# jwliao1209/DiffMusic

Measured on AMD Instinct MI355X. Metric: denoising steps/sec (10 s clip, 200-step DPS), higher is better.
Workload: dtype f16; 1 GPU; MusicLDM + DPS music_inpainting, 10 s @16 kHz, 200-step schedule, batch 8 per GPU (BASELINE.json configs[1]); global_batch=8, clips_per_gpu=8, lanes=1, parallelism=clip-sharded x1 (RCCL world size 1, no per-step collective), finite=True, nan_steps=0, settle_steps=10, cached_reference_transform=True, launched_by=single process

## Files before the change

### diffmusic_amd/_ctypes_ops.py

```python
import ctypes as C

import torch

from . import _lib


def _stream():
    return C.c_void_p(torch.cuda.current_stream().cuda_stream)


def _p(t):
    return C.c_void_p(t.data_ptr()) if t is not None else C.c_void_p(0)


def abi_version():
    return _lib.lib().dmx_abi_version()


def sched_pred_x0(x, eps, alpha_t, *, ptype=0, clip_r=0.0):
    x0 = torch.empty_like(x)
    if ptype == 0 and clip_r == 0.0:
        _lib.check(_lib.lib().dmx_sched_pred_x0(_p(x), _p(eps), _p(x0), x.numel(), alpha_t, _stream()), "pred_x0")
    else:
        _lib.check(_lib.lib().dmx_sched_pred_x0_ex(_p(x), _p(eps), _p(x0), x.numel(), alpha_t, ptype, clip_r, _stream()), "pred_x0_ex")
# ... 244 lines not shown


def vae_dec_fwd(model, z, z_scale, keep_state, want_f32, scale_factor, ws):
    B, _, h, w = z.shape
    s = scale_factor
    mel = torch.empty(B, h * s, w * s, dtype=_lib.act_dtype(), device=z.device)
    mel32 = torch.empty(B, h * s, w * s, dtype=torch.float32, device=z.device) if want_f32 else None
    _lib.check(_lib.lib().dmx_vae_decode_fwd(model, _p(z), z_scale, _p(mel), _p(mel32), B, h, w, int(keep_state), _p(ws), ws.numel(),
                                             _stream()), "vae_decode_fwd")
    return mel, mel32


def vae_dec_bwd(model, dmel, z_scale, latent_channels, scale_factor):
    B, H, W = dmel.shape
    dz = torch.empty(B, latent_channels, H // scale_factor, W // scale_factor, dtype=torch.float32, device=dmel.device)
    _lib.check(_lib.lib().dmx_vae_decode_bwd(model, _p(dmel), z_scale, _p(dz), _stream()), "vae_decode_bwd")
    return dz


def vae_enc_fwd(model, mel, log_floor, latent_channels, scale_factor, ws):
    B, T, F = mel.shape
    s = scale_factor
    mom = torch.empty(B, (T // s) * (F // s), 2 * latent_channels, dtype=torch.float32, device=mel.device)
    _lib.check(_lib.lib().dmx_vae_encode_fwd(model, _p(mel), log_floor, _p(mom), B, T, F, _p(ws), ws.numel(), _stream()), "vae_encode_fwd")
    return mom


def latent_init(moments, h, w, eps, noise, sqrt_abar, scaling_factor, sqrt_1m_abar, want_x):
    B, P, L2 = moments.shape
    assert P == h * w and L2 % 2 == 0, (moments.shape, h, w)
    L = L2 // 2
    mean = torch.empty(B, L, h, w, dtype=torch.float32, device=moments.device)
    logvar = torch.empty_like(mean)
    x = torch.empty_like(mean) if want_x else None
    _lib.check(_lib.lib().dmx_latent_init(_p(moments), _p(mean), _p(logvar), _p(x), _p(eps), _p(noise), B, L, P, sqrt_abar,
                                          scaling_factor, sqrt_1m_abar, _stream()), "latent_init")
    return mean, logvar, x


def grad_normalize_(dwav, target):
    inv_scale = torch.empty(dwav.shape[0], dtype=torch.float32, device=dwav.device)
    _lib.check(_lib.lib().dmx_grad_normalize(_p(dwav), _p(inv_scale), dwav.shape[0], dwav.shape[1], target, _stream()), "grad_normalize")
    return inv_scale


def hifigan_fwd(model, mel, ws):
    lib = _lib.lib()
    B, T, _ = mel.shape
    wav = torch.empty(B, lib.dmx_hifigan_out_len(model, T), dtype=torch.float32, device=mel.device)
    _lib.check(lib.dmx_hifigan_fwd(model, _p(mel), _p(wav), B, T, _p(ws), ws.numel(), _stream()), "hifigan_fwd")
    return wav


def hifigan_bwd(model, dwav, frames, model_in_dim):
    dmel = torch.empty(dwav.shape[0], frames, model_in_dim, dtype=_lib.act_dtype(), device=dwav.device)
    _lib.check(_lib.lib().dmx_hifigan_bwd(model, _p(dwav), _p(dmel), _stream()), "hifigan_bwd")
    return dmel


def htsat_fwd(model, mel, keep_state, ws):
    lib = _lib.lib()
    B, frames, _ = mel.shape
    tokens, channels = C.c_int(), C.c_int()
    _lib.check(lib.dmx_htsat_feature_dims(model, C.byref(tokens), C.byref(channels)), "htsat dims")
    feat = torch.empty(B, tokens.value, channels.value, dtype=torch.float32, device=mel.device)
    _lib.check(lib.dmx_htsat_fwd(model, _p(mel), B, frames, _p(feat), int(keep_state), _p(ws), ws.numel(), _stream()), "htsat_fwd")
    return feat


def htsat_bwd(model, dfeat, scale, frames, bins):
    dmel = torch.empty(dfeat.shape[0], frames, bins, dtype=torch.float32, device=dfeat.device)
    _lib.check(_lib.lib().dmx_htsat_bwd(model, _p(dfeat), _p(scale), _p(dmel), _stream()), "htsat_bwd")
    return dmel


def gram_fwd(feat):
    B, T, Cc = feat.shape
    g = torch.empty(B, Cc, Cc, dtype=torch.float32, device=feat.device)
    _lib.check(_lib.lib().dmx_gram_fwd(_p(feat), _p(g), B, T, Cc, _stream()), "gram_fwd")
    return g


def gram_bwd(feat, dgram):
    B, T, Cc = feat.shape
    d = torch.empty_like(feat)
    _lib.check(_lib.lib().dmx_gram_bwd(_p(feat), _p(dgram), _p(d), B, T, Cc, _stream()), "gram_bwd")
    return d
```

### diffmusic_amd/_lib.py

```python
import ctypes as C
import os

_HERE = os.path.dirname(os.path.abspath(__file__))
LIB_PATH = os.environ.get("DMX_LIB_PATH") or os.path.join(_HERE, "lib", "libdiffmusic_hip.so")
MAX_STAGES = 8


class HifiGanConfig(C.Structure):
    _fields_ = [("model_in_dim", C.c_int), ("upsample_initial_channel", C.c_int), ("num_upsamples", C.c_int),
                ("upsample_rates", C.c_int * MAX_STAGES), ("upsample_kernel_sizes", C.c_int * MAX_STAGES),
                ("num_kernels", C.c_int), ("resblock_kernel_sizes", C.c_int * MAX_STAGES),
                ("num_dilations", C.c_int), ("resblock_dilation_sizes", C.c_int * (MAX_STAGES * MAX_STAGES)),
                ("leaky_relu_slope", C.c_float)]


class VaeConfig(C.Structure):
    _fields_ = [("latent_channels", C.c_int), ("out_channels", C.c_int), ("num_blocks", C.c_int),
                ("block_out_channels", C.c_int * MAX_STAGES), ("layers_per_block", C.c_int),
                ("norm_num_groups", C.c_int), ("eps", C.c_float)]


class UNetConfig(C.Structure):
    _fields_ = [("in_channels", C.c_int), ("out_channels", C.c_int), ("num_blocks", C.c_int),
                ("block_out_channels", C.c_int * MAX_STAGES), ("layers_per_block", C.c_int),
# ... 2 lines not shown
                ("class_embed_dim", C.c_int), ("num_attn_per_layer", C.c_int), ("attn_cross_dims", C.c_int * 4)]


class HtsatConfig(C.Structure):
    _fields_ = [("spec_size", C.c_int), ("num_mel_bins", C.c_int), ("patch_size", C.c_int), ("embed_dim", C.c_int), ("window_size", C.c_int),
                ("num_stages", C.c_int), ("depths", C.c_int * 4), ("num_heads", C.c_int * 4), ("ln_eps", C.c_float), ("bn_eps", C.c_float)]


class GemmDesc(C.Structure):
    _fields_ = [("A", C.c_void_p), ("W", C.c_void_p), ("C", C.c_void_p), ("C2", C.c_void_p),
                ("bias", C.c_void_p), ("rowbias", C.c_void_p), ("R", C.c_void_p), ("X", C.c_void_p),
                ("M", C.c_int), ("N", C.c_int), ("K", C.c_int), ("ldw", C.c_int),
                ("Hi", C.c_int), ("Wi", C.c_int), ("Ci", C.c_int), ("lda", C.c_int),
                ("Hq", C.c_int), ("Wq", C.c_int), ("sy", C.c_int), ("sx", C.c_int),
                ("ntaps", C.c_int),
                ("Ho", C.c_int), ("Wo", C.c_int), ("ldc", C.c_int), ("osy", C.c_int), ("ooy", C.c_int),
                ("osx", C.c_int), ("oox", C.c_int),
                ("ldr", C.c_int), ("ldx", C.c_int), ("ldc2", C.c_int),
                ("Z", C.c_int), ("Zi", C.c_int),
                ("sAo", C.c_longlong), ("sAi", C.c_longlong), ("sWo", C.c_longlong), ("sWi", C.c_longlong),
                ("sCo", C.c_longlong), ("sCi", C.c_longlong),
                ("alpha", C.c_float), ("act_slope", C.c_float), ("mask_slope", C.c_float),
                ("flags", C.c_int),
                ("tdy", C.c_byte * 16), ("tdx", C.c_byte * 16), ("resid_inv_slope", C.c_float), ("tile_cfg", C.c_int), ("ldrb", C.c_int), ("ksplit", C.c_int),
                ("XB", C.c_void_p), ("B2", C.c_void_p), ("ldxb", C.c_int), ("ldb2", C.c_int),
                ("colsum", C.c_void_p), ("ln_eps", C.c_float), ("rowstats_in", C.c_void_p), ("rowstats_out", C.c_void_p), ("nslots", C.c_int),
                ("gn_part", C.c_void_p), ("gnb_x", C.c_void_p), ("gnb_scale", C.c_void_p), ("gnb_shift", C.c_void_p),
                ("gnb_ldx", C.c_int), ("gnb_silu", C.c_int), ("gnb_stats", C.c_void_p), ("gnb_cpg", C.c_int)]


EPI_BIAS, EPI_ROWBIAS, EPI_RESID, EPI_ACCUM, EPI_MASK, EPI_LRELU2, EPI_TANH, EPI_F32OUT, EPI_NO_C, EPI_RESID_INV, EPI_MASKBITS, EPI_BITS2, EPI_SOFTBWD = \
    1, 2, 4, 8, 16, 32, 64, 128, 256, 512, 1024, 2048, 4096
EPI_GEGLU, EPI_LNFOLD, EPI_ROWSTATS, EPI_GNSTATS, EPI_GNBWD = 8192, 16384, 32768, 65536, 131072

_SIGS = {
    "dmx_abi_version": (C.c_int, []),
    "dmx_act_dtype": (C.c_int, []),
    "dmx_last_error": (C.c_char_p, []),
    "dmx_hifigan_create": (C.c_void_p, [C.POINTER(HifiGanConfig)]),
    "dmx_vae_decoder_create": (C.c_void_p, [C.POINTER(VaeConfig)]),
    "dmx_unet_create": (C.c_void_p, [C.POINTER(UNetConfig)]),
    "dmx_model_destroy": (None, [C.c_void_p]),
    "dmx_model_num_params": (C.c_int, [C.c_void_p]),
    "dmx_model_param_name": (C.c_char_p, [C.c_void_p, C.c_int]),
    "dmx_model_param_numel": (C.c_size_t, [C.c_void_p, C.c_int]),
    "dmx_model_param_ndim": (C.c_int, [C.c_void_p, C.c_int]),
    "dmx_model_param_dim": (C.c_int, [C.c_void_p, C.c_int, C.c_int]),
    "dmx_model_load_param": (C.c_int, [C.c_void_p, C.c_char_p, C.c_void_p, C.c_size_t]),
    "dmx_model_finalize": (C.c_int, [C.c_void_p, C.c_void_p]),
    "dmx_hifigan_out_len": (C.c_int, [C.c_void_p, C.c_int]),
    "dmx_hifigan_workspace_bytes": (C.c_size_t, [C.c_void_p, C.c_int, C.c_int]),
    "dmx_hifigan_fwd": (C.c_int, [C.c_void_p, C.c_void_p, C.c_void_p, C.c_int, C.c_int, C.c_void_p, C.c_size_t, C.c_void_p]),
    "dmx_hifigan_bwd": (C.c_int, [C.c_void_p, C.c_void_p, C.c_void_p, C.c_void_p]),
    "dmx_vae_workspace_bytes": (C.c_size_t, [C.c_void_p, C.c_int, C.c_int, C.c_int]),
    "dmx_vae_decode_fwd": (C.c_int, [C.c_void_p, C.c_void_p, C.c_float, C.c_void_p, C.c_void_p, C.c_int, C.c_int, C.c_int,
                                     C.c_int, C.c_void_p, C.c_size_t, C.c_void_p]),
    "dmx_vae_decode_bwd": (C.c_int, [C.c_void_p, C.c_void_p, C.c_float, C.c_void_p, C.c_void_p]),
    "dmx_vae_encoder_create": (C.c_void_p, [C.POINTER(VaeConfig)]),
    "dmx_vae_encoder_workspace_bytes": (C.c_size_t, [C.c_void_p, C.c_int, C.c_int, C.c_int]),
    "dmx_vae_encode_fwd": (C.c_int, [C.c_void_p, C.c_void_p, C.c_float, C.c_void_p, C.c_int, C.c_int, C.c_int, C.c_void_p, C.c_size_t,
                                     C.c_void_p]),
    "dmx_latent_init": (C.c_int, [C.c_void_p] * 6 + [C.c_int] * 3 + [C.c_float] * 3 + [C.c_void_p]),
    "dmx_conv2d_raw": (C.c_int, [C.c_void_p] * 4 + [C.c_int] * 9 + [C.c_void_p]),
    "dmx_unet_workspace_bytes": (C.c_size_t, [C.c_void_p, C.c_int, C.c_int, C.c_int]),
    "dmx_unet_fwd": (C.c_int, [C.c_void_p, C.c_void_p, C.c_void_p, C.c_void_p, C.c_void_p, C.c_int, C.c_int, C.c_int,
                               C.c_void_p, C.c_size_t, C.c_void_p]),
    "dmx_unet_fwd_ctx": (C.c_int, [C.c_void_p] * 5 + [C.c_int, C.c_void_p, C.c_int, C.c_void_p, C.c_void_p, C.c_int, C.c_int, C.c_int,
                                   C.c_void_p, C.c_size_t, C.c_void_p]),
    "dmx_unet_workspace_bytes_ctx": (C.c_size_t, [C.c_void_p, C.c_int, C.c_int, C.c_int, C.c_int, C.c_int]),
    "dmx_htsat_create": (C.c_void_p, [C.POINTER(HtsatConfig)]),
    "dmx_htsat_feature_dims": (C.c_int, [C.c_void_p, C.POINTER(C.c_int), C.POINTER(C.c_int)]),
    "dmx_htsat_workspace_bytes": (C.c_size_t, [C.c_void_p, C.c_int, C.c_int]),
    "dmx_htsat_fwd": (C.c_int, [C.c_void_p, C.c_void_p, C.c_int, C.c_int, C.c_void_p, C.c_int, C.c_void_p, C.c_size_t, C.c_void_p]),
    "dmx_htsat_bwd": (C.c_int, [C.c_void_p, C.c_void_p, C.c_void_p, C.c_void_p, C.c_void_p]),
    "dmx_htsat_tape_raw": (C.c_size_t, [C.c_void_p, C.c_int, C.c_int, C.c_int, C.c_void_p, C.c_size_t, C.c_void_p]),
    "dmx_gram_fwd": (C.c_int, [C.c_void_p, C.c_void_p, C.c_int, C.c_int, C.c_int, C.c_void_p]),
    "dmx_gram_bwd": (C.c_int, [C.c_void_p, C.c_void_p, C.c_void_p, C.c_int, C.c_int, C.c_int, C.c_void_p]),
    "dmx_gemm_raw": (C.c_int, [C.c_void_p, C.c_size_t, C.c_void_p]),
    "dmx_prof_begin": (None, []),
    "dmx_prof_end": (C.c_int, [C.POINTER(C.c_double), C.POINTER(C.c_double)]),
    "dmx_flash_attn_raw": (C.c_int, [C.c_void_p, C.c_void_p, C.c_void_p, C.c_void_p, C.c_void_p] + [C.c_int] * 6 + [C.c_float, C.c_void_p]),
    "dmx_gemm_splitk_workspace": (C.c_int, [C.c_void_p, C.c_size_t]),
    "dmx_conv_pair_raw": (C.c_int, [C.c_void_p, C.c_void_p, C.c_size_t, C.c_void_p]),
    "dmx_conv_pair_group_raw": (C.c_int, [C.c_int, C.c_void_p, C.c_void_p, C.c_size_t, C.c_void_p]),
    "dmx_groupnorm_scratch_floats": (C.c_size_t, [C.c_int, C.c_int, C.c_int]),
    "dmx_groupnorm_raw": (C.c_int, [C.c_void_p] * 8 + [C.c_int] * 4 + [C.c_float, C.c_int, C.c_void_p]),
    "dmx_groupnorm_part_floats": (C.c_size_t, [C.c_int, C.c_int, C.c_int]),
    "dmx_groupnorm_parts_raw": (C.c_int, [C.c_void_p] * 7 + [C.c_int] * 4 + [C.c_float, C.c_int, C.c_int, C.c_void_p, C.c_void_p, C.c_void_p]),
    "dmx_gemm_last_tile_rows_raw": (C.c_int, []),
    "dmx_groupnorm_bwd_raw": (C.c_int, [C.c_void_p] * 10 + [C.c_int] * 6 + [C.c_void_p, C.c_void_p, C.c_void_p]),
    "dmx_prof_dominant": (C.c_int, [C.POINTER(C.c_double)] * 3),
    "dmx_audio_create": (C.c_void_p, [C.c_int, C.c_int, C.c_int, C.c_int, C.c_void_p]),
    "dmx_audio_destroy": (None, [C.c_void_p]),
    "dmx_audio_num_frames": (C.c_int, [C.c_void_p, C.c_int]),
    "dmx_audio_num_bins": (C.c_int, [C.c_void_p]),
    "dmx_audio_state_bytes": (C.c_size_t, [C.c_void_p, C.c_int, C.c_int]),
    "dmx_audio_transform_fwd": (C.c_int, [C.c_void_p, C.c_void_p, C.c_longlong, C.c_void_p, C.c_void_p, C.c_int, C.c_int, C.c_int,
                                          C.c_int, C.c_float, C.c_float, C.c_void_p]),
    "dmx_audio_transform_bwd": (C.c_int, [C.c_void_p, C.c_void_p, C.c_void_p, C.c_longlong, C.c_void_p, C.c_int, C.c_int, C.c_int,
                                          C.c_int, C.c_float, C.c_float, C.c_int, C.c_void_p]),
    "dmx_audio_is_fused": (C.c_int, [C.c_void_p, C.c_int]),
    "dmx_audio_guidance_fwd": (C.c_int, [C.c_void_p, C.c_void_p, C.c_longlong, C.c_void_p, C.c_void_p, C.c_longlong, C.c_void_p, C.c_void_p,
                                         C.c_int, C.c_int, C.c_int, C.c_int, C.c_float, C.c_float, C.c_void_p]),
    "dmx_audio_guidance_bwd": (C.c_int, [C.c_void_p, C.c_void_p, C.c_longlong, C.c_void_p, C.c_void_p, C.c_longlong, C.c_float, C.c_void_p,
                                         C.c_void_p, C.c_longlong, C.c_int, C.c_void_p, C.c_int, C.c_int, C.c_int, C.c_int, C.c_float, C.c_float,
                                         C.c_void_p]),
    "dmx_audio_guidance_fwd_ex": (C.c_int, [C.c_void_p, C.c_void_p, C.c_longlong, C.c_void_p, C.c_void_p, C.c_longlong, C.c_void_p, C.c_void_p,
                                            C.c_int, C.c_int, C.c_int, C.c_int, C.c_float, C.c_float, C.c_void_p, C.c_longlong, C.c_void_p,
                                            C.c_float, C.c_void_p]),
    "dmx_audio_guidance_bwd_ex": (C.c_int, [C.c_void_p, C.c_void_p, C.c_longlong, C.c_void_p, C.c_void_p, C.c_longlong, C.c_float, C.c_void_p,
                                            C.c_void_p, C.c_longlong, C.c_int, C.c_void_p, C.c_int, C.c_int, C.c_int, C.c_int, C.c_float, C.c_float,
                                            C.c_void_p, C.c_longlong, C.c_void_p, C.c_float, C.c_void_p]),
    "dmx_audio_guidance_fwd_shaped": (C.c_int, [C.c_void_p, C.c_void_p, C.c_longlong, C.c_void_p, C.c_void_p, C.c_longlong, C.c_void_p, C.c_void_p,
                                                C.c_int, C.c_int, C.c_int, C.c_int, C.c_float, C.c_float, C.c_void_p, C.c_longlong, C.c_void_p,
                                                C.c_float, C.c_void_p, C.c_void_p]),
    "dmx_audio_guidance_bwd_shaped": (C.c_int, [C.c_void_p, C.c_void_p, C.c_longlong, C.c_void_p, C.c_void_p, C.c_longlong, C.c_float, C.c_void_p,
                                                C.c_void_p, C.c_longlong, C.c_int, C.c_void_p, C.c_int, C.c_int, C.c_int, C.c_int, C.c_float, C.c_float,
                                                C.c_void_p, C.c_longlong, C.c_void_p, C.c_float, C.c_void_p, C.c_void_p]),
    "dmx_clip_fwd": (C.c_int, [C.c_void_p, C.c_longlong, C.c_void_p, C.c_void_p, C.c_longlong, C.c_int, C.c_int, C.c_void_p]),
    "dmx_clip_bwd": (C.c_int, [C.c_void_p, C.c_longlong, C.c_void_p, C.c_longlong, C.c_void_p, C.c_void_p, C.c_longlong, C.c_int, C.c_int, C.c_int,
                               C.c_void_p]),
    "dmx_declip_project": (C.c_int, [C.c_void_p, C.c_longlong, C.c_void_p, C.c_longlong, C.c_void_p, C.c_void_p, C.c_longlong, C.c_int, C.c_int,
                                     C.c_void_p]),
    "dmx_noise_add": (C.c_int, [C.c_void_p, C.c_void_p, C.c_void_p, C.c_longlong, C.c_float, C.c_void_p]),
    "dmx_audio_stft_mag": (C.c_int, [C.c_void_p, C.c_void_p, C.c_longlong, C.c_void_p, C.c_void_p, C.c_int, C.c_int, C.c_void_p]),
    "dmx_audio_stft_mag_bwd": (C.c_int, [C.c_void_p, C.c_void_p, C.c_void_p, C.c_longlong, C.c_void_p, C.c_int, C.c_int, C.c_int, C.c_void_p]),
    "dmx_audio_melscale": (C.c_int, [C.c_void_p, C.c_void_p, C.c_void_p, C.c_int, C.c_int, C.c_float, C.c_float, C.c_void_p]),
    "dmx_mask_apply": (C.c_int, [C.c_void_p, C.c_longlong, C.c_void_p, C.c_void_p, C.c_longlong, C.c_int, C.c_int, C.c_int, C.c_void_p]),
    "dmx_l2_loss": (C.c_int, [C.c_void_p, C.c_longlong, C.c_void_p, C.c_void_p, C.c_void_p, C.c_int, C.c_longlong, C.c_float, C.c_void_p]),
    "dmx_track_stitch_fwd": (C.c_int, [C.c_void_p, C.c_longlong, C.c_void_p, C.POINTER(C.c_int)] + [C.c_int] * 4 + [C.c_void_p]),
    "dmx_track_stitch_bwd": (C.c_int, [C.c_void_p, C.c_void_p, C.c_longlong, C.POINTER(C.c_int)] + [C.c_int] * 5 + [C.c_void_p]),
    "dmx_grad_normalize": (C.c_int, [C.c_void_p, C.c_void_p, C.c_int, C.c_longlong, C.c_float, C.c_void_p]),
    "dmx_fir_fwd": (C.c_int, [C.c_void_p, C.c_longlong, C.c_void_p, C.c_void_p, C.c_longlong] + [C.c_int] * 7 + [C.c_void_p]),
    "dmx_fir_bwd": (C.c_int, [C.c_void_p, C.c_longlong, C.c_void_p, C.c_void_p, C.c_void_p, C.c_longlong] + [C.c_int] * 7 + [C.c_void_p]),
    "dmx_sched_pred_x0": (C.c_int, [C.c_void_p, C.c_void_p, C.c_void_p, C.c_longlong, C.c_float, C.c_void_p]),
    "dmx_sched_pred_x0_ex": (C.c_int, [C.c_void_p, C.c_void_p, C.c_void_p, C.c_longlong, C.c_float, C.c_int, C.c_float, C.c_void_p]),
    "dmx_sched_step_ex": (C.c_int, [C.c_int] + [C.c_void_p] * 9 + [C.c_int, C.c_int] + [C.c_float] * 5 + [C.c_int, C.c_int, C.c_float, C.c_void_p]),
    "dmx_sched_cfg_combine": (C.c_int, [C.c_void_p, C.c_void_p, C.c_longlong, C.c_float, C.c_void_p]),
    "dmx_randn_philox": (C.c_int, [C.c_void_p, C.c_int, C.c_longlong, C.POINTER(C.c_ulonglong), C.c_ulonglong, C.c_void_p]),
    "dmx_sched_step": (C.c_int, [C.c_int] + [C.c_void_p] * 9 + [C.c_int, C.c_int] + [C.c_float] * 5 + [C.c_int, C.c_void_p]),
}

ADDED_IN_V4 = ("dmx_vae_encoder_create", "dmx_vae_encoder_workspace_bytes", "dmx_vae_encode_fwd", "dmx_latent_init",
               "dmx_track_stitch_fwd", "dmx_track_stitch_bwd", "dmx_audio_guidance_fwd_shaped", "dmx_audio_guidance_bwd_shaped",
               "dmx_clip_fwd", "dmx_clip_bwd", "dmx_declip_project")

_lib = None


def check_symbols(h, path=LIB_PATH):
    for name in ADDED_IN_V4:
        if not hasattr(h, name):
            raise RuntimeError(f"{path} reports ABI version {ABI_VERSION} but does not export `{name}` (a build from before the VAE "
                               "encoder / track-mode / declipping entry points): rebuild it (python -m diffmusic_amd.build --force)")


def lib():
    global _lib
    if _lib is None:
        if not os.path.exists(LIB_PATH):
            raise RuntimeError(f"{LIB_PATH} is missing: build it with `python -m diffmusic_amd.build` "
                               "(the diffmusic_amd hot path has no CPU fallback)")
        h = C.CDLL(LIB_PATH)
        for name, (res, args) in _SIGS.items():
            if not hasattr(h, name):
                continue
            fn = getattr(h, name)
            fn.restype, fn.argtypes = res, args
        if h.dmx_abi_version() != ABI_VERSION:
            raise RuntimeError(f"libdiffmusic_hip.so ABI version {h.dmx_abi_version()} != {ABI_VERSION} expected by this package: rebuild it "
                               "(python -m diffmusic_amd.build --force)")
        check_symbols(h)
        _lib = h
    return _lib


ABI_VERSION = 4


def act_dtype():
    import torch
    return torch.float16 if lib().dmx_act_dtype() == 1 else torch.bfloat16


class DmxError(RuntimeError):
    pass


def check(rc, what=""):
    if rc != 0:
        msg = lib().dmx_last_error()
        raise DmxError(f"{what} failed with code {rc}: {msg.decode() if msg else ''}")
```

### diffmusic_amd/csrc/capi.hip

```cpp
#include "conv_pair.h"
#include "models.h"

#define M_IMPL(m) ((m) ? (m)->impl : nullptr)
#define ST(s) ((hipStream_t)(s))

extern "C" {

int dmx_abi_version(void) { return DMX_ABI_VERSION; }
int dmx_act_dtype(void) { return DMX_ACT_DTYPE; }

dmx_model* dmx_hifigan_create(const dmx_hifigan_config* cfg) {
  if (!cfg || cfg->num_upsamples > DMX_MAX_STAGES || cfg->num_kernels > DMX_MAX_STAGES || cfg->num_dilations > DMX_MAX_STAGES) {
    dmx_set_error("bad hifigan config");
    return nullptr;
  }
  return new dmx_model{dmx_make_hifigan(cfg)};
}
dmx_model* dmx_vae_decoder_create(const dmx_vae_config* cfg) {
  if (!cfg || cfg->num_blocks > DMX_MAX_STAGES) { dmx_set_error("bad vae config"); return nullptr; }
  Model* m = dmx_make_vae(cfg);
  return m ? new dmx_model{m} : nullptr;
}
dmx_model* dmx_unet_create(const dmx_unet_config* cfg) {
  if (!cfg || cfg->num_blocks > DMX_MAX_STAGES) { dmx_set_error("bad unet config"); return nullptr; }
  Model* m = dmx_make_unet(cfg);
  return m ? new dmx_model{m} : nullptr;
}
void dmx_model_destroy(dmx_model* m) {
  if (!m) return;
  delete m->impl;
  delete m;
}
int dmx_model_num_params(const dmx_model* m) { return (int)m->impl->ps.params.size(); }
const char* dmx_model_param_name(const dmx_model* m, int i) { return m->impl->ps.params[i].name.c_str(); }
size_t dmx_model_param_numel(const dmx_model* m, int i) { return m->impl->ps.params[i].numel; }
int dmx_model_param_ndim(const dmx_model* m, int i) { return (int)m->impl->ps.params[i].shape.size(); }
int dmx_model_param_dim(const dmx_model* m, int i, int d) { return m->impl->ps.params[i].shape[d]; }
int dmx_model_load_param(dmx_model* m, const char* name, const float* data_host, size_t numel) {
  if (m->impl->finalized) { dmx_set_error("model already finalized"); return DMX_ERR_STATE; }
  return m->impl->ps.load(name, data_host, numel);
}
int dmx_model_finalize(dmx_model* m, void* stream) {
  std::string missing;
  if (!m->impl->ps.all_loaded(&missing)) { dmx_set_error("parameter '%s' was never loaded", missing.c_str()); return DMX_ERR_PARAM; }
  const int rc = m->impl->finalize(ST(stream));
  if (rc == DMX_OK) m->impl->finalized = true;
  return rc;
}

static int check(dmx_model* m, int kind) {
  if (!m || !m->impl || m->impl->kind != kind) { dmx_set_error("wrong model handle"); return DMX_ERR_STATE; }
  if (!m->impl->finalized) { dmx_set_error("model not finalized"); return DMX_ERR_STATE; }
  return DMX_OK;
}

int dmx_hifigan_out_len(const dmx_model* m, int frames) { return dmx_hifigan_out_len_impl(m->impl, frames); }
size_t dmx_hifigan_workspace_bytes(dmx_model* m, int batch, int frames) { return dmx_hifigan_ws_impl(m->impl, batch, frames); }
int dmx_hifigan_fwd(dmx_model* m, const uint16_t* mel, float* wav, int batch, int frames, void* ws, size_t ws_bytes, void* stream) {
  int rc = check(m, DMX_MODEL_HIFIGAN);
  if (rc) return rc;
  if (!ws) { dmx_set_error("null workspace"); return DMX_ERR_WORKSPACE; }
  return dmx_hifigan_fwd_impl(m->impl, mel, wav, batch, frames, ws, ws_bytes, ST(stream));
}
int dmx_hifigan_bwd(dmx_model* m, const float* dwav, uint16_t* dmel, void* stream) {
  int rc = check(m, DMX_MODEL_HIFIGAN);
  if (rc) return rc;
  return dmx_hifigan_bwd_impl(m->impl, dwav, dmel, ST(stream));
}

size_t dmx_vae_workspace_bytes(dmx_model* m, int batch, int h, int w) { return dmx_vae_ws_impl(m->impl, batch, h, w); }
int dmx_vae_decode_fwd(dmx_model* m, const float* z, float z_scale, uint16_t* mel, float* mel_f32, int batch, int h, int w,
                       int keep_state, void* ws, size_t ws_bytes, void* stream) {
  int rc = check(m, DMX_MODEL_VAE);
  if (rc) return rc;
  if (!ws) { dmx_set_error("null workspace"); return DMX_ERR_WORKSPACE; }
  return dmx_vae_fwd_impl(m->impl, z, z_scale, mel, mel_f32, batch, h, w, keep_state, ws, ws_bytes, ST(stream));
}
int dmx_vae_decode_bwd(dmx_model* m, const uint16_t* dmel, float z_scale, float* dz, void* stream) {
  int rc = check(m, DMX_MODEL_VAE);
  if (rc) return rc;
  return dmx_vae_bwd_impl(m->impl, dmel, z_scale, dz, ST(stream));
}

dmx_model* dmx_vae_encoder_create(const dmx_vae_config* cfg) {
  if (!cfg || cfg->num_blocks > DMX_MAX_STAGES) { dmx_set_error("bad vae config"); return nullptr; }
  Model* m = dmx_make_vae_encoder(cfg);
  return m ? new dmx_model{m} : nullptr;
}
size_t dmx_vae_encoder_workspace_bytes(dmx_model* m, int batch, int frames, int bins) {
  if (!m || !m->impl || m->impl->kind != DMX_MODEL_VAE_ENC) return 0;
  return dmx_vae_enc_ws_impl(m->impl, batch, frames, bins);
}
int dmx_vae_encode_fwd(dmx_model* m, const float* mel, float log_floor, float* moments, int batch, int frames, int bins, void* ws,
                       size_t ws_bytes, void* stream) {
  int rc = check(m, DMX_MODEL_VAE_ENC);
  if (rc) return rc;
  if (!ws) { dmx_set_error("null workspace"); return DMX_ERR_WORKSPACE; }
  return dmx_vae_enc_fwd_impl(m->impl, mel, log_floor, moments, batch, frames, bins, ws, ws_bytes, ST(stream));
}
int dmx_latent_init(const float* moments, float* mean, float* logvar, float* x, const float* eps, const float* noise, int batch,
                    int latent_channels, int hw, float sqrt_abar, float scaling_factor, float sqrt_1m_abar, void* stream) {
  return dmx_latent_init_impl(moments, mean, logvar, x, eps, noise, batch, latent_channels, hw, sqrt_abar, scaling_factor, sqrt_1m_abar, ST(stream));
}
int dmx_conv2d_raw(const float* w_host, const float* b_host, const void* x, void* y, int B, int Hi, int Wi, int Ci, int Co, int k, int stride,
                   int pad_lo, int pad_hi, void* stream) {
  return dmx_conv2d_raw_impl(w_host, b_host, (const act_t*)x, (act_t*)y, B, Hi, Wi, Ci, Co, k, stride, pad_lo, pad_hi, ST(stream));
}

dmx_model* dmx_htsat_create(const dmx_htsat_config* cfg) {
  Model* impl = dmx_make_htsat(cfg);
  if (!impl) return nullptr;
  return new dmx_model{impl};
}
int dmx_htsat_feature_dims(dmx_model* m, int* tokens, int* channels) {
  if (!m || !m->impl || m->impl->kind != DMX_MODEL_HTSAT) { dmx_set_error("wrong model handle"); return DMX_ERR_STATE; }
// ... 140 lines not shown
```

### diffmusic_amd/csrc/conv_pair.h

```cpp
#pragma once
#include <cstdlib>
#include <cstring>
#include "dmx_common.h"

bool dmx_conv_pair_eligible(const GemmDesc* a, const GemmDesc& b);
int dmx_conv_pair_launch(const GemmDesc* a, const GemmDesc& b, hipStream_t st);
int dmx_conv_pair_group_launch(int n, const GemmDesc* const* a, const GemmDesc* const* b, hipStream_t st);

int dmx_prof_open(hipStream_t st);
void dmx_prof_close(int rec, hipStream_t st, double flops, double bytes, int M, int N, int K, int taps, int flags, int cfg);
```

### diffmusic_amd/csrc/conv_pair.hip

```cpp
#include "gemm_epilogue.h"
#include "conv_pair.h"

namespace {

constexpr int PAIR_HALO = 50;
constexpr int PAIR_ROWS = 256;
constexpr unsigned PAIR_OOB = 0x80000000u;

struct PairParams {
  GemmDesc a, b;
  int T, nb, BMo;
  int loA, hiA, loB, hiB;
  int off0A, dA, off0B, dB;
  int single;
  int r_from_slab;
  int a_tape_bits_only;
};

#ifdef DMX_PAIR_STAMPS
__device__ unsigned long long g_pair_stamps[4096 * 8];
#define DMX_STAMP(i) do { stamp_v[i] = wall_clock64(); } while (0)
#else
#define DMX_STAMP(i) do { } while (0)
#endif

template <int C>
struct PairCfg {
  static constexpr int PITCH = 2 * C + 32;
  static constexpr int CPR = C / 8;
  static constexpr int WN = C > 64 ? C / 64 : 1;
  static constexpr int NW = 4 * WN;
  static constexpr int NT = NW * 64;
  static constexpr int FN = C / 16 / WN;
  static constexpr int SLAB_ROWS = PAIR_ROWS + PAIR_HALO;
  static constexpr int SLAB_BYTES = SLAB_ROWS * PITCH;
  static constexpr int TILE = C * 128;
  static constexpr int NS = C == 128 ? 4 : 3;
  static constexpr int PER = TILE / 1024 / NW;
  static constexpr int SLAB_IT = (SLAB_ROWS * CPR + NT - 1) / NT;
  static constexpr int BITS_IT = PAIR_ROWS * CPR / NT;
  static constexpr int BITS_BYTES = PAIR_ROWS * CPR;
  static constexpr int BIAS_BYTES = 2 * C * 4;
  static constexpr int LDS_BYTES = SLAB_BYTES + NS * TILE + BITS_BYTES + BIAS_BYTES;
  static constexpr int MIN_WAVES = C == 32 ? 3 : 2;
  static_assert(PER >= 1 && PAIR_ROWS * CPR % NT == 0, "tile / thread-count mismatch");
};

template <int FN>
struct PairFrags { frag8_t x[2][4]; frag8_t w[2][FN]; };

#define DMX_PAIR_DSR(dst, addr, off) asm volatile("ds_read_b128 %0, %1 offset:%2" : "=v"(dst) : "v"(addr), "n"(off))

#define DMX_LDS_ADDR(p) ((unsigned)(size_t)(__attribute__((address_space(3))) const char*)(p))
typedef unsigned u32x2_t __attribute__((ext_vector_type(2)));
typedef unsigned u32x4_t __attribute__((ext_vector_type(4)));
__device__ __forceinline__ void pair_lds_w64(const void* p, uint2 v) {
  const u32x2_t w = {v.x, v.y};
  asm volatile("ds_write_b64 %0, %1" ::"v"(DMX_LDS_ADDR(p)), "v"(w) : "memory");
}
#define DMX_PAIR_DSR64(dst, p) asm volatile("ds_read_b64 %0, %1" : "=v"(dst) : "v"(DMX_LDS_ADDR(p)))
#define DMX_PAIR_DSRU8(dst, p) asm volatile("ds_read_u8 %0, %1" : "=v"(dst) : "v"(DMX_LDS_ADDR(p)))
__device__ __forceinline__ void pair_lds_wait() { asm volatile("s_waitcnt lgkmcnt(0)" ::: "memory"); }
template <typename T>
__device__ __forceinline__ void pair_tie8(T (&r)[8]) {
  asm volatile("s_waitcnt lgkmcnt(0)" : "+v"(r[0]), "+v"(r[1]), "+v"(r[2]), "+v"(r[3]), "+v"(r[4]), "+v"(r[5]), "+v"(r[6]), "+v"(r[7]) : : "memory");
}
template <typename T>
__device__ __forceinline__ void pair_tie16(T (&r)[16]) {
  asm volatile("s_waitcnt lgkmcnt(0)"
               : "+v"(r[0]), "+v"(r[1]), "+v"(r[2]), "+v"(r[3]), "+v"(r[4]), "+v"(r[5]), "+v"(r[6]), "+v"(r[7]), "+v"(r[8]), "+v"(r[9]), "+v"(r[10]),
                 "+v"(r[11]), "+v"(r[12]), "+v"(r[13]), "+v"(r[14]), "+v"(r[15])
               :
               : "memory");
}
template <typename T, int N>
__device__ __forceinline__ void pair_tie(T (&r)[N]) {
  static_assert(N == 8 || N == 16, "4 row fragments x 2 or 4 column fragments");
  if constexpr (N == 8) pair_tie8(r); else pair_tie16(r);
}

__device__ __forceinline__ void pair_settle(PairFrags<4>& f) {
  asm volatile("s_waitcnt lgkmcnt(0)"
               : "+v"(f.x[0][0]), "+v"(f.x[0][1]), "+v"(f.x[0][2]), "+v"(f.x[0][3]), "+v"(f.x[1][0]), "+v"(f.x[1][1]), "+v"(f.x[1][2]),
                 "+v"(f.x[1][3]), "+v"(f.w[0][0]), "+v"(f.w[0][1]), "+v"(f.w[0][2]), "+v"(f.w[0][3]), "+v"(f.w[1][0]), "+v"(f.w[1][1]),
                 "+v"(f.w[1][2]), "+v"(f.w[1][3])
               :
               : "memory");
}
__device__ __forceinline__ void pair_settle(PairFrags<2>& f) {
  asm volatile("s_waitcnt lgkmcnt(0)"
               : "+v"(f.x[0][0]), "+v"(f.x[0][1]), "+v"(f.x[0][2]), "+v"(f.x[0][3]), "+v"(f.x[1][0]), "+v"(f.x[1][1]), "+v"(f.x[1][2]),
                 "+v"(f.x[1][3]), "+v"(f.w[0][0]), "+v"(f.w[0][1]), "+v"(f.w[1][0]), "+v"(f.w[1][1])
               :
               : "memory");
}

template <int C>
__device__ __forceinline__ void pair_body(const PairParams& P, char* smem, int bid, const int nwg) {
  using K = PairCfg<C>;
  constexpr int PITCH = K::PITCH, CPR = K::CPR, FN = K::FN, NS = K::NS, PER = K::PER, TILE = K::TILE, NT = K::NT, NW = K::NW, WN = K::WN;
  char* ring = smem;
  char* slab = smem + NS * TILE;
  unsigned char* s_bits = reinterpret_cast<unsigned char*>(slab + K::SLAB_BYTES);
  float* s_bias = reinterpret_cast<float*>(slab + K::SLAB_BYTES + K::BITS_BYTES);

  const int tid = threadIdx.x, lane = tid & 63, lr = lane & 15, lq = lane >> 4;
  const int wave = __builtin_amdgcn_readfirstlane(tid >> 6);
  const int rg = wave / WN, cg = wave - rg * WN;
#ifdef DMX_PAIR_STAMPS
  const int stamp_id = bid;
  unsigned long long stamp_v[8] = {0, 0, 0, 0, 0, 0, 0, 0};
#endif
  DMX_STAMP(0);
  {
    const int q = nwg >> 3, r = nwg & 7, xcd = bid & 7, loc = bid >> 3;
    bid = (xcd < r ? xcd * (q + 1) : r * (q + 1) + (xcd - r) * q) + loc;
  }
  const int T = P.T;
  const int b = bid / P.nb, tq = bid - b * P.nb;
  const int t0 = tq * P.BMo;
  const bool single = P.single != 0;
  const int kA = single ? 0 : P.a.ntaps, kB = P.b.ntaps;
  const int stepsA = (kA * C + 63) / 64, stepsB = (kB * C + 63) / 64, total = stepsA + stepsB;

  const __amdgpu_buffer_rsrc_t rsA = __builtin_amdgcn_make_buffer_rsrc(const_cast<act_t*>(single ? P.b.W : P.a.W), 0, PAIR_OOB, 0x00020000);
  const __amdgpu_buffer_rsrc_t rsB = __builtin_amdgcn_make_buffer_rsrc(const_cast<act_t*>(P.b.W), 0, PAIR_OOB, 0x00020000);
  const int lrow = lane >> 3, cc = (lane & 7) ^ lrow;
  auto issue_dma = [&](int g) {
    const bool inA = g < stepsA;
    const int sidx = inA ? g : g - stepsA;
    const int Kel = inA ? P.a.K : P.b.K;
    const unsigned ldw2 = (unsigned)(inA ? P.a.ldw : P.b.ldw) * 2u;
    const int kel = sidx * 64 + cc * 8;
    const bool ok = g < total && kel < Kel;
    char* dst = ring + (g % NS) * TILE;
#pragma unroll
    for (int i = 0; i < PER; ++i) {
      const int j = i * NW + wave;
      const unsigned voff = ok ? (unsigned)(j * 8 + lrow) * ldw2 + (unsigned)kel * 2u : PAIR_OOB;
      if (inA) __builtin_amdgcn_raw_ptr_buffer_load_lds(rsA, (__attribute__((address_space(3))) void*)(dst + j * 1024), 16, voff, 0, 0, 0);
      else __builtin_amdgcn_raw_ptr_buffer_load_lds(rsB, (__attribute__((address_space(3))) void*)(dst + j * 1024), 16, voff, 0, 0, 0);
    }
  };
  issue_dma(0);
  issue_dma(1);
  issue_dma(2);

  {
    const act_t* src = single ? P.b.A : P.a.A;
    const int nrows = PAIR_ROWS + (single ? P.loB + P.hiB : P.loA + P.hiA);
    const int tfirst = t0 - P.loB - (single ? 0 : P.loA);
    uint4 sv[K::SLAB_IT];
#pragma unroll
    for (int it = 0; it < K::SLAB_IT; ++it) {
      const int c = tid + it * NT, row = c / CPR, piece = c % CPR, t = tfirst + row;
      sv[it] = make_uint4(0, 0, 0, 0);
      if (row < nrows && t >= 0 && t < T) sv[it] = *reinterpret_cast<const uint4*>(src + ((long long)b * T + t) * C + piece * 8);
    }
    const bool masked = !single && (P.a.flags & EPI_MASK);
    const bool maskbits = !single && (P.a.flags & EPI_MASKBITS);
    constexpr int BPT = K::BITS_BYTES / NT;
    static_assert(BPT == 4 || BPT == 8, "bit-mask copy granularity");
    static_assert(CPR % BPT == 0, "a thread's mask bytes must stay inside one row");
    uint32_t mb[2] = {0u, 0u};
    if (maskbits) {
      const int c = tid * BPT, row = c / CPR, piece = c % CPR, t = t0 - P.loB + row;
      if (t >= 0 && t < T) {
        const unsigned char* src = P.a.XB + ((long long)b * T + t) * P.a.ldxb + piece;
        mb[0] = *reinterpret_cast<const uint32_t*>(src);
        if (BPT == 8) mb[1] = *reinterpret_cast<const uint32_t*>(src + 4);
      }
    }
#pragma unroll
    for (int it = 0; it < K::SLAB_IT; ++it) {
      const int c = tid + it * NT, row = c / CPR, piece = c % CPR;
      if (row < K::SLAB_ROWS) *reinterpret_cast<uint4*>(slab + row * PITCH + piece * 16) = sv[it];
    }
    if (masked) {
#pragma unroll 1
      for (int it = 0; it < K::BITS_IT; ++it) {
        const int c = tid + it * NT, row = c / CPR, piece = c % CPR, t = t0 - P.loB + row;
        uint4 m = make_uint4(0, 0, 0, 0);
        if (t >= 0 && t < T) m = *reinterpret_cast<const uint4*>(P.a.X + ((long long)b * T + t) * C + piece * 8);
        s_bits[c] = (unsigned char)dmx_pos8(m);
      }
    }
    if (maskbits) {
      uint32_t* d = reinterpret_cast<uint32_t*>(s_bits + tid * BPT);
      d[0] = mb[0];
      if (BPT == 8) d[1] = mb[1];
    }
  }
  if (tid < 2 * C) {
    const GemmDesc& d = tid < C ? P.a : P.b;
    const int ch = tid < C ? tid : tid - C;
    s_bias[tid] = (!(single && tid < C) && d.bias && (d.flags & (EPI_BIAS | EPI_BIASINIT))) ? d.bias[ch] : 0.f;
  }
  asm volatile("s_waitcnt vmcnt(0)" ::: "memory");
  __syncthreads();
  DMX_STAMP(1);

  f32x4 acc[4][FN];
  auto zero_acc = [&]() {
#pragma unroll
    for (int i = 0; i < 4; ++i)
#pragma unroll
      for (int n = 0; n < FN; ++n) acc[i][n] = f32x4{0.f, 0.f, 0.f, 0.f};
  };
  auto init_acc = [&](const GemmDesc& d) {
    if (C < 128 && (d.flags & EPI_BIASINIT)) {
// ... 256 lines not shown
  Halo h{0, 0, true, d.ntaps > 1 ? d.tdx[1] - d.tdx[0] : 0};
  for (int j = 0; j < d.ntaps; ++j) {
    if (d.tdx[j] != d.tdx[0] + j * h.d) h.ok = false;
    if (d.tdy[j] != 0) h.ok = false;
    if (-d.tdx[j] > h.lo) h.lo = -d.tdx[j];
    if (d.tdx[j] > h.hi) h.hi = d.tdx[j];
  }
  if (h.lo + h.hi > PAIR_HALO) h.ok = false;
  return h;
}

bool stage_ok(const GemmDesc& d, int C, int T, int allowed_flags) {
  if (d.N != C || d.Ci != C || d.lda != C || d.K != d.ntaps * C || d.ldw < d.K) return false;
  if (d.ntaps < 1 || d.ntaps > 16 || d.Z != 1 || d.Hq != 1 || d.Hi != 1 || d.Ho != 1) return false;
  if (d.Wq != T || d.Wi != T || d.Wo != T || d.sx != 1 || d.osx != 1 || d.oox != 0 || d.ooy != 0) return false;
  if (d.flags & ~allowed_flags) return false;
  if (d.M % T != 0) return false;
  return true;
}

bool g_pair_enabled = getenv("DMX_NO_PAIR") == nullptr;

}

bool dmx_conv_pair_eligible(const GemmDesc* a, const GemmDesc& b) {
  if (!g_pair_enabled) return false;
  const int C = b.N, T = b.Wq;
  static const bool c128 = getenv("DMX_NO_PAIR128") == nullptr;
  if (C != 32 && C != 64 && !(C == 128 && c128)) return false;
  if (T < 1) return false;
  const int bflags = EPI_BIAS | EPI_RESID | EPI_RESID_INV | EPI_ACCUM | EPI_MASK | EPI_LRELU2 | EPI_NO_C | EPI_MASKBITS | EPI_BITS2;
  if (!stage_ok(b, C, T, bflags) || !halo_of(b).ok) return false;
  if ((b.flags & EPI_LRELU2) && !(b.act_slope >= 0.f && b.act_slope <= 1.f)) return false;
  if ((b.flags & EPI_RESID_INV) && !(b.resid_inv_slope >= 1.f)) return false;
  if (b.ldc != C || ((b.flags & EPI_RESID) && b.ldr != C) || ((b.flags & EPI_MASK) && b.ldx != C) || ((b.flags & EPI_LRELU2) && b.ldc2 != C))
    return false;
  if ((b.flags & EPI_MASKBITS) && (!b.XB || b.ldxb * 8 < C)) return false;
  if ((b.flags & EPI_BITS2) && (!b.B2 || b.ldb2 * 8 < C)) return false;
  if (a) {
    if (!stage_ok(*a, C, T, EPI_BIAS | EPI_LRELU2 | EPI_NO_C | EPI_MASK | EPI_MASKBITS | EPI_BITS2) || !halo_of(*a).ok) return false;
    if (a->M != b.M || a->alpha != 1.f) return false;
    if ((a->flags & EPI_LRELU2) && !(a->flags & EPI_BITS2) && (a->ldc2 != C || !a->C2)) return false;
    if ((a->flags & EPI_LRELU2) && a->C2 && a->ldc2 != C) return false;
    if ((a->flags & EPI_BITS2) && (!(a->flags & EPI_LRELU2) || !a->B2 || a->ldb2 * 8 < C)) return false;
    if ((a->flags & EPI_MASK) && (a->ldx != C || !a->X)) return false;
    if ((a->flags & EPI_MASKBITS) && (!a->XB || a->ldxb * 8 < C || (a->flags & EPI_MASK))) return false;
    const Halo hb = halo_of(b);
    if (PAIR_ROWS - hb.lo - hb.hi < 128) return false;
  }
  return true;
}

namespace {
long long pair_params(const GemmDesc* a, const GemmDesc& b, PairParams& P, double& fl, double& by) {
  memset(&P, 0, sizeof(P));
  P.b = b;
  P.single = a ? 0 : 1;
  if (a) P.a = *a;
  const Halo hb = halo_of(b);
  P.loB = hb.lo; P.hiB = hb.hi;
  P.off0B = b.tdx[0] + hb.lo; P.dB = hb.d;
  if (a) { const Halo ha = halo_of(*a); P.loA = ha.lo; P.hiA = ha.hi; P.off0A = a->tdx[0] + ha.lo; P.dA = ha.d; }
  P.T = b.Wq;
  P.BMo = a ? PAIR_ROWS - hb.lo - hb.hi : PAIR_ROWS;
  P.nb = cdiv(P.T, P.BMo);
  static const bool bias_init = getenv("DMX_NO_BIAS_INIT") == nullptr;
  if (bias_init && b.N < 128) {
    if ((P.b.flags & EPI_BIAS) && P.b.bias && !(P.b.flags & (EPI_MASK | EPI_MASKBITS))) P.b.flags = (P.b.flags & ~EPI_BIAS) | EPI_BIASINIT;
    if (a && (P.a.flags & EPI_BIAS) && P.a.bias && !(P.a.flags & (EPI_MASK | EPI_MASKBITS))) P.a.flags = (P.a.flags & ~EPI_BIAS) | EPI_BIASINIT;
  }
  P.r_from_slab = (a && (b.flags & EPI_RESID) && b.R == a->A && b.ldr == b.N) ? 1 : 0;
  P.a_tape_bits_only = (a && (a->flags & EPI_BITS2) && !a->C2) ? 1 : 0;
  const int nclips = b.M / P.T;
  const int C = b.N;
  fl = 2.0 * b.M * (double)b.N * b.K;
  by = 2.0 * b.M * (double)C * 2.0;
  const double bits_by = b.M * (double)C / 8.0;
  if (a) {
    fl += 2.0 * a->M * (double)a->N * a->K;
    if ((a->flags & EPI_LRELU2) && !P.a_tape_bits_only) by += 2.0 * b.M * (double)C;
    if (a->flags & EPI_BITS2) by += bits_by;
    if (a->flags & EPI_MASK) by += 2.0 * b.M * (double)C;
    if (a->flags & EPI_MASKBITS) by += bits_by;
  }
  if ((b.flags & EPI_RESID) && !P.r_from_slab) by += 2.0 * b.M * (double)C;
  if (b.flags & EPI_MASK) by += 2.0 * b.M * (double)C;
  if (b.flags & EPI_MASKBITS) by += bits_by;
  if (b.flags & EPI_BITS2) by += bits_by;
  if (b.flags & EPI_ACCUM) by += 2.0 * b.M * (double)C;
  if ((b.flags & EPI_LRELU2) && !(b.flags & EPI_NO_C)) by += 2.0 * b.M * (double)C;
  return (long long)nclips * P.nb;
}
}

static int pair_extra_lds() { static const int v = [] { const char* e = getenv("DMX_PAIR_EXTRA_LDS"); return e ? atoi(e) : 0; }(); return v; }
int dmx_conv_pair_launch(const GemmDesc* a, const GemmDesc& b, hipStream_t st) {
  if (!dmx_conv_pair_eligible(a, b)) return DMX_ERR_SHAPE;
  PairParams P;
  double fl, by;
  const long long grid = pair_params(a, b, P, fl, by);
  if (grid > 0x7fffffffLL) return DMX_ERR_SHAPE;
  const int C = b.N;
  const int rec = dmx_prof_open(st);
  auto launch = [&](auto tag) {
    constexpr int CC = decltype(tag)::value;
    static bool attr = false;
    if (!attr) { (void)hipFuncSetAttribute((const void*)conv_pair_kernel<CC>, hipFuncAttributeMaxDynamicSharedMemorySize, PairCfg<CC>::LDS_BYTES + (CC < 128 ? pair_extra_lds() : 0)); attr = true; }
    hipLaunchKernelGGL(conv_pair_kernel<CC>, dim3((unsigned)grid), dim3(PairCfg<CC>::NT), PairCfg<CC>::LDS_BYTES + (CC < 128 ? pair_extra_lds() : 0), st, P);
  };
  if (C == 32) launch(std::integral_constant<int, 32>{});
  else if (C == 64) launch(std::integral_constant<int, 64>{});
  else launch(std::integral_constant<int, 128>{});
  dmx_prof_close(rec, st, fl, by, b.M, b.N, (a ? a->K : 0) + b.K, b.ntaps, b.flags, a ? 21 : 20);
  return hipGetLastError() == hipSuccess ? DMX_OK : DMX_ERR_LAUNCH;
}

int dmx_conv_pair_group_launch(int n, const GemmDesc* const* a, const GemmDesc* const* b, hipStream_t st) {
  if (n < 1 || n > DMX_PAIR_GROUP) return DMX_ERR_SHAPE;
  static const bool off = getenv("DMX_NO_PAIR_GROUP") != nullptr;
  bool same = !off && n > 1;
  for (int j = 0; j < n; ++j) {
    if (!a[j] || !b[j] || !dmx_conv_pair_eligible(a[j], *b[j])) return DMX_ERR_SHAPE;
    if (b[j]->N != b[0]->N) same = false;
    for (int i = 0; i < j; ++i)
      if (b[j]->C == b[i]->C || (b[j]->C2 && b[j]->C2 == b[i]->C2)) same = false;
  }
  if (!same) {
    for (int j = 0; j < n; ++j) { const int rc = dmx_conv_pair_launch(a[j], *b[j], st); if (rc != DMX_OK) return rc; }
    return DMX_OK;
  }
  int order[DMX_PAIR_GROUP] = {0, 1, 2};
  auto work = [&](int j) { return a[j]->K + b[j]->K; };
  for (int i = 0; i < n; ++i)
    for (int k = i + 1; k < n; ++k)
      if (work(order[k]) > work(order[i])) { const int t = order[i]; order[i] = order[k]; order[k] = t; }
  PairGroup G;
  memset(&G, 0, sizeof(G));
  double fl = 0.0, by = 0.0;
  long long gmax = 0;
  int Ksum = 0;
  for (int i = 0; i < n; ++i) {
    const int j = order[i];
    double f1, b1;
    const long long g = pair_params(a[j], *b[j], G.p[i], f1, b1);
    if (g > 0x7ffffff0LL) return DMX_ERR_SHAPE;
    G.n[i] = (int)g;
    if (g > gmax) gmax = g;
    fl += f1; by += b1; Ksum += a[j]->K + b[j]->K;
  }
  const unsigned gx = (unsigned)((gmax + 7) & ~7ll);
  const int C = b[0]->N;
  const int rec = dmx_prof_open(st);
  auto launch = [&](auto tag) {
    constexpr int CC = decltype(tag)::value;
    static bool attr = false;
    if (!attr) { (void)hipFuncSetAttribute((const void*)conv_pair_group_kernel<CC>, hipFuncAttributeMaxDynamicSharedMemorySize, PairCfg<CC>::LDS_BYTES); attr = true; }
    hipLaunchKernelGGL(conv_pair_group_kernel<CC>, dim3(gx, (unsigned)n), dim3(PairCfg<CC>::NT), PairCfg<CC>::LDS_BYTES, st, G);
  };
  if (C == 32) launch(std::integral_constant<int, 32>{});
  else if (C == 64) launch(std::integral_constant<int, 64>{});
  else launch(std::integral_constant<int, 128>{});
  dmx_prof_close(rec, st, fl, by, b[0]->M, C, Ksum, b[0]->ntaps, b[0]->flags, 22);
  return hipGetLastError() == hipSuccess ? DMX_OK : DMX_ERR_LAUNCH;
}

#ifdef DMX_PAIR_STAMPS
extern "C" int dmx_pair_stamps_read(unsigned long long* host) {
  return hipMemcpyFromSymbol(host, HIP_SYMBOL(g_pair_stamps), sizeof(unsigned long long) * 4096 * 8) == hipSuccess ? 0 : -1;
}
#endif
```

### diffmusic_amd/csrc/elementwise.hip

```cpp
#include "dmx_common.h"
#include <cstdlib>
#include "kernels.h"

namespace {

__device__ __forceinline__ void unpack8(const uint4& u, float* f) {
  f[0] = alo(u.x); f[1] = ahi(u.x); f[2] = alo(u.y); f[3] = ahi(u.y);
  f[4] = alo(u.z); f[5] = ahi(u.z); f[6] = alo(u.w); f[7] = ahi(u.w);
}
__device__ __forceinline__ uint4 pack8(const float* f) {
  return make_uint4(pack2a(f[0], f[1]), pack2a(f[2], f[3]), pack2a(f[4], f[5]), pack2a(f[6], f[7]));
}
__device__ __forceinline__ float silu_f(float z) { return z / (1.f + __expf(-z)); }
__device__ __forceinline__ float dsilu_f(float z) {
  const float s = 1.f / (1.f + __expf(-z));
  return s * (1.f + z * (1.f - s));
}

template <int MODE>
__global__ void gn_partial_kernel(const act_t* __restrict__ x, const act_t* __restrict__ dy,
                                  const float* __restrict__ scale, const float* __restrict__ shift,
                                  const float* __restrict__ stats, float* __restrict__ partial,
                                  int P, int C, int G, int rpb, int ppb, int silu) {
  extern __shared__ float sh[];
// ... 928 lines not shown
}

__global__ void nchw_f32_to_nhwc_bf16_kernel(const float* __restrict__ x, act_t* __restrict__ y, int B, int C, int HW,
                                             int Cp, float scale) {
  const long long idx = (long long)blockIdx.x * blockDim.x + threadIdx.x;
  if (idx >= (long long)B * HW * Cp) return;
  const int c = (int)(idx % Cp);
  const long long pix = idx / Cp;
  const int b = (int)(pix / HW), p = (int)(pix - (long long)b * HW);
  y[idx] = c < C ? f2a(x[((long long)b * C + c) * HW + p] * scale) : (act_t)0;
}
__global__ void nhwc_bf16_to_nchw_f32_kernel(const act_t* __restrict__ x, float* __restrict__ y, int B, int C, int HW,
                                             int Cp, float scale) {
  const long long idx = (long long)blockIdx.x * blockDim.x + threadIdx.x;
  if (idx >= (long long)B * C * HW) return;
  const int p = (int)(idx % HW);
  const long long bc = idx / HW;
  const int b = (int)(bc / C), c = (int)(bc - (long long)b * C);
  y[idx] = a2f(x[((long long)b * HW + p) * Cp + c]) * scale;
}
__global__ void f32_to_bf16_kernel(const float* __restrict__ x, act_t* __restrict__ y, long long n, float scale) {
  const long long idx = (long long)blockIdx.x * blockDim.x + threadIdx.x;
  if (idx < n) y[idx] = f2a(x[idx] * scale);
}
__global__ void bf16_to_f32_kernel(const act_t* __restrict__ x, float* __restrict__ y, long long n, float scale) {
  const long long idx = (long long)blockIdx.x * blockDim.x + threadIdx.x;
  if (idx < n) y[idx] = a2f(x[idx]) * scale;
}
__global__ void extract_col_kernel(const act_t* __restrict__ x, float* __restrict__ y, long long rows, int ld, int col) {
  const long long idx = (long long)blockIdx.x * blockDim.x + threadIdx.x;
  if (idx < rows) y[idx] = a2f(x[idx * ld + col]);
}
__global__ void timestep_embed_kernel(const float* __restrict__ t, act_t* __restrict__ y, int B, int dim) {
  const int idx = blockIdx.x * blockDim.x + threadIdx.x;
  if (idx >= B * dim) return;
  const int b = idx / dim, j = idx - b * dim, half = dim >> 1;
  const int k = j < half ? j : j - half;
  const float e = t[b] * __expf(-9.210340371976184f * (float)k / (float)half);
  y[idx] = f2a(j < half ? cosf(e) : sinf(e));
}

__global__ void gather_col_f32_kernel(const float* __restrict__ x, float* __restrict__ y, long long rows, int ld, int col) {
  const long long idx = (long long)blockIdx.x * blockDim.x + threadIdx.x;
  if (idx < rows) y[idx] = x[idx * ld + col];
}
__global__ void tanh_bwd_pad8_kernel(const float* __restrict__ dwav, const float* __restrict__ wav8, act_t* __restrict__ gz,
                                     long long rows) {
  const long long idx = (long long)blockIdx.x * blockDim.x + threadIdx.x;
  if (idx >= rows) return;
  const float w = wav8[idx * 8];
  const float g = dwav[idx] * (1.f - w * w);
  reinterpret_cast<uint4*>(gz)[idx] = make_uint4((uint32_t)f2a(g), 0u, 0u, 0u);
}
__global__ void scatter_col_pad8_kernel(const float* __restrict__ v, act_t* __restrict__ y, long long rows, float scale) {
  const long long idx = (long long)blockIdx.x * blockDim.x + threadIdx.x;
  if (idx >= rows) return;
  reinterpret_cast<uint4*>(y)[idx] = make_uint4((uint32_t)f2a(v[idx] * scale), 0u, 0u, 0u);
}

__global__ void gather_col_f32_to_act_kernel(const float* __restrict__ x, act_t* __restrict__ y, long long rows, int ld, int col) {
  const long long idx = (long long)blockIdx.x * blockDim.x + threadIdx.x;
  if (idx < rows) y[idx] = f2a(x[idx * ld + col]);
}
__global__ void pad_col8_act_kernel(const act_t* __restrict__ v, act_t* __restrict__ y, long long rows) {
  const long long idx = (long long)blockIdx.x * blockDim.x + threadIdx.x;
  if (idx >= rows) return;
  reinterpret_cast<uint4*>(y)[idx] = make_uint4((uint32_t)v[idx], 0u, 0u, 0u);
}

constexpr int GN_SMALL_MAXU = 16;
__global__ __launch_bounds__(256) void gn_small_kernel(const act_t* __restrict__ x, act_t* __restrict__ y,
                                                       const float* __restrict__ gamma, const float* __restrict__ beta,
                                                       float* __restrict__ stats, float* __restrict__ scale, float* __restrict__ shift,
                                                       int P, int C, int G, float eps, int silu) {
  __shared__ float sh[16];
  const int g = blockIdx.x, b = blockIdx.y, cpg = C / G, U = cpg >> 2, c0 = g * cpg;
  const int units = P * U;
  const act_t* xb = x + (long long)b * P * C + c0;
  uint2 v[GN_SMALL_MAXU];
  float sum = 0.f;
#pragma unroll
  for (int i = 0; i < GN_SMALL_MAXU; ++i) {
    const int u = threadIdx.x + i * 256;
    v[i] = make_uint2(0, 0);
    if (u < units) {
      const int px = u / U, cu = u - px * U;
      v[i] = *reinterpret_cast<const uint2*>(xb + (long long)px * C + cu * 4);
      sum += alo(v[i].x) + ahi(v[i].x) + alo(v[i].y) + ahi(v[i].y);
    }
  }
  const float n = (float)units * 4.f;
  const float mean = block_sum(sum, sh) / n;
  float m2 = 0.f;
#pragma unroll
  for (int i = 0; i < GN_SMALL_MAXU; ++i) {
    if (threadIdx.x + i * 256 < units) {
      const float d0 = alo(v[i].x) - mean, d1 = ahi(v[i].x) - mean, d2 = alo(v[i].y) - mean, d3 = ahi(v[i].y) - mean;
      m2 += d0 * d0 + d1 * d1 + d2 * d2 + d3 * d3;
    }
  }
  const float rstd = rsqrtf(block_sum(m2, sh) / n + eps);
  if (threadIdx.x == 0) {
    stats[((long long)b * G + g) * 2] = mean;
    stats[((long long)b * G + g) * 2 + 1] = rstd;
  }
  if (threadIdx.x < cpg) {
// ... 199 lines not shown
  return CHECK_LAUNCH();
}
int dmx_concat2(const act_t* a, const act_t* b, act_t* dst, long long rows, int Ca, int Cb, hipStream_t st) {
  if ((Ca & 7) || (Cb & 7)) return DMX_ERR_SHAPE;
  const long long n = rows * ((Ca + Cb) >> 3);
  hipLaunchKernelGGL(concat2_kernel, dim3((unsigned)((n + 255) / 256)), dim3(256), 0, st, a, b, dst, rows, Ca, Cb);
  return CHECK_LAUNCH();
}
int dmx_axpby(const act_t* x, const act_t* y0, act_t* y, float a, float b, long long n, hipStream_t st) {
  if (n & 7) return DMX_ERR_SHAPE;
  hipLaunchKernelGGL(axpby_kernel, dim3((unsigned)((n / 8 + 255) / 256)), dim3(256), 0, st, x, y0, y, a, b, n / 8);
  return CHECK_LAUNCH();
}
int dmx_nchw_f32_to_nhwc_bf16(const float* x, act_t* y, int B, int C, int HW, int Cp, float scale, hipStream_t st) {
  const long long n = (long long)B * HW * Cp;
  hipLaunchKernelGGL(nchw_f32_to_nhwc_bf16_kernel, dim3((unsigned)((n + 255) / 256)), dim3(256), 0, st, x, y, B, C, HW, Cp, scale);
  return CHECK_LAUNCH();
}
int dmx_nhwc_bf16_to_nchw_f32(const act_t* x, float* y, int B, int C, int HW, int Cp, float scale, hipStream_t st) {
  const long long n = (long long)B * C * HW;
  hipLaunchKernelGGL(nhwc_bf16_to_nchw_f32_kernel, dim3((unsigned)((n + 255) / 256)), dim3(256), 0, st, x, y, B, C, HW, Cp, scale);
  return CHECK_LAUNCH();
}
int dmx_f32_to_bf16(const float* x, act_t* y, long long n, float scale, hipStream_t st) {
  hipLaunchKernelGGL(f32_to_bf16_kernel, dim3((unsigned)((n + 255) / 256)), dim3(256), 0, st, x, y, n, scale);
  return CHECK_LAUNCH();
}
int dmx_bf16_to_f32(const act_t* x, float* y, long long n, float scale, hipStream_t st) {
  hipLaunchKernelGGL(bf16_to_f32_kernel, dim3((unsigned)((n + 255) / 256)), dim3(256), 0, st, x, y, n, scale);
  return CHECK_LAUNCH();
}
int dmx_extract_col(const act_t* x, float* y, long long rows, int ld, int col, hipStream_t st) {
  hipLaunchKernelGGL(extract_col_kernel, dim3((unsigned)((rows + 255) / 256)), dim3(256), 0, st, x, y, rows, ld, col);
  return CHECK_LAUNCH();
}
int dmx_timestep_embed(const float* t, act_t* y, int B, int dim, hipStream_t st) {
  hipLaunchKernelGGL(timestep_embed_kernel, dim3(cdiv(B * dim, 256)), dim3(256), 0, st, t, y, B, dim);
  return CHECK_LAUNCH();
}

int dmx_gather_col_f32(const float* x, float* y, long long rows, int ld, int col, hipStream_t st) {
  hipLaunchKernelGGL(gather_col_f32_kernel, dim3((unsigned)((rows + 255) / 256)), dim3(256), 0, st, x, y, rows, ld, col);
  return CHECK_LAUNCH();
}
int dmx_tanh_bwd_pad8(const float* dwav, const float* wav8, act_t* gz, long long rows, hipStream_t st) {
  hipLaunchKernelGGL(tanh_bwd_pad8_kernel, dim3((unsigned)((rows + 255) / 256)), dim3(256), 0, st, dwav, wav8, gz, rows);
  return CHECK_LAUNCH();
}
int dmx_scatter_col_pad8(const float* v, act_t* y, long long rows, float scale, hipStream_t st) {
  hipLaunchKernelGGL(scatter_col_pad8_kernel, dim3((unsigned)((rows + 255) / 256)), dim3(256), 0, st, v, y, rows, scale);
  return CHECK_LAUNCH();
}

int dmx_gather_col_f32_to_act(const float* x, act_t* y, long long rows, int ld, int col, hipStream_t st) {
  hipLaunchKernelGGL(gather_col_f32_to_act_kernel, dim3((unsigned)((rows + 255) / 256)), dim3(256), 0, st, x, y, rows, ld, col);
  return CHECK_LAUNCH();
}
int dmx_pad_col8_act(const act_t* v, act_t* y, long long rows, hipStream_t st) {
  hipLaunchKernelGGL(pad_col8_act_kernel, dim3((unsigned)((rows + 255) / 256)), dim3(256), 0, st, v, y, rows);
  return CHECK_LAUNCH();
}
```

### diffmusic_amd/csrc/hifigan.hip

```cpp
#include "models.h"
#include "conv_pair.h"
#include <cstdlib>

struct SplitKScope {
  explicit SplitKScope(float* ws, size_t bytes, bool on) : on_(on && ws) { if (on_) dmx_gemm_set_splitk_workspace(ws, bytes); }
  ~SplitKScope() { if (on_) dmx_gemm_set_splitk_workspace(nullptr, 0); }
  bool on_;
};

struct HifiGan : Model {
  dmx_hifigan_config cfg;
  static constexpr size_t kSplitKBytes = 32u << 20;
  float* splitk_ws = nullptr;
  ConvLayer conv_pre, conv_post;
  std::vector<ConvLayer> ups;
  std::vector<ConvLayer> c1, c2;
  int nk = 0, nd = 0, ns = 0;
  int B = 0, T = 0;
  std::vector<int> Ts;
  act_t* act_pre = nullptr;
  std::vector<act_t*> xs_a;
  std::vector<act_t*> ha, xa;
  std::vector<act_t*> act_out;
  std::vector<unsigned char*> hb, xb;
  std::vector<char> fused;
  float* wav8 = nullptr;
  bool have_tape = false;
  hipStream_t bstream[DMX_MAX_STAGES] = {};
  std::vector<hipEvent_t> events;
  size_t ev_next = 0;
  bool want_multi = true;
  hipEvent_t next_event() { hipEvent_t e = events[ev_next]; ev_next = (ev_next + 1) % events.size(); return e; }
  bool multi() const { return want_multi && !dry && !dmx_prof_is_active() && nk > 1; }
  bool multi_wanted() const { return want_multi && nk > 1; }

  int idx(int s, int k, int d) const { return (s * nk + k) * nd + d; }

  explicit HifiGan(const dmx_hifigan_config& c) : cfg(c) {
    kind = DMX_MODEL_HIFIGAN;
    ns = c.num_upsamples; nk = c.num_kernels; nd = c.num_dilations;
    const int C0 = c.upsample_initial_channel;
    conv_pre = make_conv1d(ps, "conv_pre", c.model_in_dim, C0, 7, 1, 3, true);
    for (int i = 0; i < ns; ++i) {
      const int s = c.upsample_rates[i], k = c.upsample_kernel_sizes[i];
      ups.push_back(make_convT1d(ps, "upsampler." + std::to_string(i), C0 >> i, C0 >> (i + 1), k, s, (k - s) / 2, true));
    }
    int ch = C0;
    for (int i = 0; i < ns; ++i) {
      ch = C0 >> (i + 1);
      for (int j = 0; j < nk; ++j) {
        const int k = c.resblock_kernel_sizes[j];
        const std::string pre = "resblocks." + std::to_string(i * nk + j);
        for (int d = 0; d < nd; ++d) {
          const int dil = c.resblock_dilation_sizes[j * nd + d];
          c1.push_back(make_conv1d(ps, pre + ".convs1." + std::to_string(d), ch, ch, k, dil, (k * dil - dil) / 2, true));
          c2.push_back(make_conv1d(ps, pre + ".convs2." + std::to_string(d), ch, ch, k, 1, (k - 1) / 2, true));
        }
      }
    }
    conv_post = make_conv1d(ps, "conv_post", ch, 1, 7, 1, 3, true);
    want_multi = getenv("DMX_MULTI_STREAM") != nullptr && getenv("DMX_SINGLE_STREAM") == nullptr;
    for (int k = 1; k < nk; ++k) (void)hipStreamCreateWithFlags(&bstream[k], hipStreamNonBlocking);
    events.resize(256);
    for (auto& e : events) (void)hipEventCreateWithFlags(&e, hipEventDisableTiming);
    splitk_ws = (float*)ps.dalloc(kSplitKBytes);
  }
  ~HifiGan() override {
    dmx_gemm_release_splitk_workspace(splitk_ws);
    for (int k = 1; k < nk; ++k) if (bstream[k]) (void)hipStreamDestroy(bstream[k]);
    for (auto& e : events) (void)hipEventDestroy(e);
  }

  int finalize(hipStream_t st) override {
    int rc = pack_layer(ps, conv_pre, st);
    for (auto& l : ups) if (rc == DMX_OK) rc = pack_layer(ps, l, st);
    for (auto& l : c1) if (rc == DMX_OK) rc = pack_layer(ps, l, st);
    for (auto& l : c2) if (rc == DMX_OK) rc = pack_layer(ps, l, st);
    if (rc == DMX_OK) rc = pack_layer(ps, conv_post, st);
    return rc;
  }

  bool step_is_fused(int id, int To) const {
    GemmDesc da, db;
    act_t* dummy = reinterpret_cast<act_t*>(size_t(256));
    unsigned char* dummyb = reinterpret_cast<unsigned char*>(size_t(256));
    Epi ea; ea.flags = EPI_LRELU2 | EPI_NO_C | EPI_BITS2; ea.act_slope = cfg.leaky_relu_slope; ea.B2 = dummyb;
    if (conv_fwd_1d_desc(c1[id], dummy, nullptr, B, To, ea, da) != DMX_OK) return false;
    Epi eb; eb.flags = EPI_RESID | EPI_RESID_INV | EPI_LRELU2 | EPI_NO_C | EPI_ACCUM; eb.R = dummy; eb.C2 = dummy;
    eb.resid_inv_slope = 1.f / cfg.leaky_relu_slope; eb.act_slope = cfg.leaky_relu_slope;
    if (conv_fwd_1d_desc(c2[id], nullptr, dummy, B, To, eb, db) != DMX_OK) return false;
    return dmx_conv_pair_eligible(&da, db);
  }

  int out_len(int T_) const {
    int t = T_;
    for (int i = 0; i < ns; ++i) t = conv_out_len(ups[i], t);
    return t;
  }

  int forward(const act_t* mel, float* wav, int B_, int T_, void* ws, size_t ws_bytes, hipStream_t st) {
    if (cfg.model_in_dim & 7) return DMX_ERR_SHAPE;
    dry = (ws == nullptr);
    SplitKScope sk_scope(splitk_ws, kSplitKBytes, !dry && !multi_wanted());
    arena.reset(ws, dry ? (size_t)-1 : ws_bytes);
    B = B_; T = T_;
    Ts.assign(ns, 0);
    xs_a.assign(ns, nullptr); act_out.assign(ns, nullptr);
    ha.assign(ns * nk * nd, nullptr); xa.assign(ns * nk * nd, nullptr);
    hb.assign(ns * nk * nd, nullptr); xb.assign(ns * nk * nd, nullptr);
    fused.assign(ns * nk * nd, 0);
    const float slope = cfg.leaky_relu_slope;
    auto bits = [&](size_t rows, int C) { return (unsigned char*)arena.raw(rows * (size_t)(C >> 3)); };
    act_pre = arena.bf((size_t)B * T * conv_pre.Cop);
    {
      Epi e; e.flags = EPI_LRELU2 | EPI_NO_C; e.act_slope = slope; e.C2 = act_pre;
      RUN(conv_fwd_1d(conv_pre, mel, act_pre, B, T, e, st));
    }
    const act_t* cur_act = act_pre;
    int Tin = T;
    for (int s = 0; s < ns; ++s) {
      const ConvLayer& up = ups[s];
      const int To = conv_out_len(up, Tin), C = up.Cop;
      const size_t n = (size_t)B * To * C;
      Ts[s] = To;
      xs_a[s] = arena.bf(n);
      act_out[s] = arena.bf(n);
      unsigned char* xs_b = nullptr;
      for (int k = 0; k < nk; ++k)
        for (int d = 0; d < nd; ++d) {
          const int id = idx(s, k, d);
          fused[id] = step_is_fused(id, To) ? 1 : 0;
          xa[id] = d == 0 ? xs_a[s] : arena.bf(n);
          if (fused[id]) {
            hb[id] = bits((size_t)B * To, C);
            if (d == 0) { if (!xs_b) xs_b = bits((size_t)B * To, C); xb[id] = xs_b; }
            else xb[id] = bits((size_t)B * To, C);
          } else {
            ha[id] = arena.bf(n);
          }
        }
      const size_t mk = arena.mark();
      act_t* sum = arena.bf(n);
      {
        Epi e; e.flags = EPI_LRELU2 | EPI_NO_C; e.act_slope = slope; e.C2 = xs_a[s];
        if (xs_b) { e.flags |= EPI_BITS2; e.B2 = xs_b; }
        RUN(conv_fwd_1d(up, cur_act, xs_a[s], B, Tin, e, st));
      }
      const float next_slope = (s == ns - 1) ? 0.01f : slope;
      const bool mt = multi();
      bool all_fused = nk <= 3;
      for (int k = 0; k < nk; ++k) for (int d = 0; d < nd; ++d) all_fused = all_fused && fused[idx(s, k, d)] != 0;
      if (all_fused && !mt) {
        for (int d = 0; d < nd; ++d) {
          GemmDesc da[DMX_MAX_STAGES], db[DMX_MAX_STAGES];
          const GemmDesc* pa[DMX_MAX_STAGES]; const GemmDesc* pb[DMX_MAX_STAGES];
          for (int k = 0; k < nk; ++k) {
            const int id = idx(s, k, d);
            {
              Epi e; e.flags = EPI_LRELU2 | EPI_NO_C | EPI_BITS2; e.act_slope = slope; e.B2 = hb[id];
              RUN(conv_fwd_1d_desc(c1[id], xa[id], ha[id], B, To, e, da[k]));
            }
            if (d < nd - 1) {
              const int idn = idx(s, k, d + 1);
              act_t* xn = xa[idn];
              Epi e; e.flags = EPI_RESID | EPI_RESID_INV | EPI_LRELU2 | EPI_NO_C | EPI_BITS2; e.R = xa[id]; e.resid_inv_slope = 1.f / slope;
              e.act_slope = slope; e.C2 = xn; e.B2 = xb[idn];
              RUN(conv_fwd_1d_desc(c2[id], ha[id], xn, B, To, e, db[k]));
            } else {
              Epi e; e.flags = EPI_RESID | EPI_RESID_INV; e.R = xa[id]; e.resid_inv_slope = 1.f / slope; e.alpha = 1.f / nk;
              if (k > 0) e.flags |= EPI_ACCUM;
              if (k == nk - 1) { e.flags |= EPI_LRELU2 | EPI_NO_C; e.act_slope = next_slope; e.C2 = act_out[s]; }
              RUN(conv_fwd_1d_desc(c2[id], ha[id], sum, B, To, e, db[k]));
            }
            pa[k] = &da[k]; pb[k] = &db[k];
          }
          if (dry) continue;
          for (int k = 0; k < nk; ++k)
            if (!dmx_conv_pair_eligible(&da[k], db[k])) {
              dmx_set_error("hifigan: resblock step %d was planned as fused but the pair kernel refuses it", idx(s, k, d));
              return DMX_ERR_STATE;
            }
          if (d < nd - 1) RUN(dmx_conv_pair_group_launch(nk, pa, pb, st));
          else for (int k = 0; k < nk; ++k) RUN(conv_pair_run(da[k], db[k], st));
        }
        arena.release(mk);
        cur_act = act_out[s];
        Tin = To;
        continue;
      }
      hipEvent_t fin_prev = nullptr;
      if (mt) {
        hipEvent_t e0 = next_event();
        (void)hipEventRecord(e0, st);
        for (int k = 1; k < nk; ++k) (void)hipStreamWaitEvent(bstream[k], e0, 0);
      }
      for (int k = 0; k < nk; ++k) {
        hipStream_t sk = (mt && k > 0) ? bstream[k] : st;
        for (int d = 0; d < nd; ++d) {
          const int id = idx(s, k, d);
          const bool fz = fused[id] != 0;
          GemmDesc da, db;
          {
            Epi e; e.flags = EPI_LRELU2 | EPI_NO_C; e.act_slope = slope;
            if (fz) { e.flags |= EPI_BITS2; e.B2 = hb[id]; } else e.C2 = ha[id];
            RUN(conv_fwd_1d_desc(c1[id], xa[id], ha[id], B, To, e, da));
          }
          if (d < nd - 1) {
            const int idn = idx(s, k, d + 1);
            act_t* xn = xa[idn];
            Epi e; e.flags = EPI_RESID | EPI_RESID_INV | EPI_LRELU2 | EPI_NO_C; e.R = xa[id]; e.resid_inv_slope = 1.f / slope;
            e.act_slope = slope; e.C2 = xn;
            if (fused[idn]) { e.flags |= EPI_BITS2; e.B2 = xb[idn]; }
            RUN(conv_fwd_1d_desc(c2[id], ha[id], xn, B, To, e, db));
          } else {
            Epi e; e.flags = EPI_RESID | EPI_RESID_INV; e.R = xa[id]; e.resid_inv_slope = 1.f / slope; e.alpha = 1.f / nk;
            if (k > 0) e.flags |= EPI_ACCUM;
            if (k == nk - 1) { e.flags |= EPI_LRELU2 | EPI_NO_C; e.act_slope = next_slope; e.C2 = act_out[s]; }
            RUN(conv_fwd_1d_desc(c2[id], ha[id], sum, B, To, e, db));
          }
          if (!dry && fz && !dmx_conv_pair_eligible(&da, db)) {
            dmx_set_error("hifigan: resblock step %d was planned as fused but the pair kernel refuses it", id);
            return DMX_ERR_STATE;
          }
          if (d == nd - 1 && mt && fin_prev) (void)hipStreamWaitEvent(sk, fin_prev, 0);
          RUN(conv_pair_run(da, db, sk));
          if (d == nd - 1 && mt) { fin_prev = next_event(); (void)hipEventRecord(fin_prev, sk); }
        }
      }
      if (mt && fin_prev) (void)hipStreamWaitEvent(st, fin_prev, 0);
      arena.release(mk);
      cur_act = act_out[s];
      Tin = To;
    }
    const int Tout = Tin;
    wav8 = arena.f32((size_t)B * Tout * 8);
    CHECK_WS("hifigan");
    {
      Epi e; e.flags = EPI_F32OUT | EPI_TANH;
      RUN(conv_fwd_1d(conv_post, cur_act, wav8, B, Tout, e, st));
    }
    RUN(dmx_gather_col_f32(wav8, wav, (long long)B * Tout, 8, 0, st));
    have_tape = true;
    return DMX_OK;
  }

  int backward(const float* dwav, act_t* dmel, hipStream_t st) {
    if (!have_tape && !dry) { dmx_set_error("hifigan backward without forward"); return DMX_ERR_STATE; }
    SplitKScope sk_scope(splitk_ws, kSplitKBytes, !dry && !multi_wanted());
    const float slope = cfg.leaky_relu_slope;
    const int Tout = Ts[ns - 1];
    const size_t mk0 = arena.mark();
    act_t* gz = arena.bf((size_t)B * Tout * 8);
    const int Clast = ups[ns - 1].Cop;
    act_t* g = arena.bf((size_t)B * Tout * Clast);
    CHECK_WS("hifigan");
    RUN(dmx_tanh_bwd_pad8(dwav, wav8, gz, (long long)B * Tout, st));
    {
      Epi e; e.flags = EPI_MASK; e.X = act_out[ns - 1]; e.mask_slope = 0.01f; e.alpha = 1.f / nk;
      RUN(conv_bwd_1d(conv_post, gz, g, B, Tout, e, st));
    }
    for (int s = ns - 1; s >= 0; --s) {
      const int To = Ts[s], Tin = s == 0 ? T : Ts[s - 1], C = ups[s].Cop;
      const size_t n = (size_t)B * To * C;
      act_t* gxs = arena.bf(n);
      act_t* ghk[DMX_MAX_STAGES];
      act_t* gAB[DMX_MAX_STAGES][2];
      for (int k = 0; k < nk; ++k) { ghk[k] = arena.bf(n); gAB[k][0] = arena.bf(n); gAB[k][1] = arena.bf(n); }
      const int Cin = ups[s].Cip;
      act_t* gprev = arena.bf((size_t)B * Tin * Cin);
      CHECK_WS("hifigan");
      const bool mt = multi();
      hipEvent_t fin_prev = nullptr;
      bool all_fused = nk <= 3;
      for (int k = 0; k < nk; ++k) for (int d = 0; d < nd; ++d) all_fused = all_fused && fused[idx(s, k, d)] != 0;
      if (all_fused && !mt) {
        const act_t* gcs[DMX_MAX_STAGES];
        for (int k = 0; k < nk; ++k) gcs[k] = g;
        for (int d = nd - 1; d >= 0; --d) {
          GemmDesc da[DMX_MAX_STAGES], db[DMX_MAX_STAGES];
          const GemmDesc* pa[DMX_MAX_STAGES]; const GemmDesc* pb[DMX_MAX_STAGES];
          act_t* dsts[DMX_MAX_STAGES];
          for (int k = 0; k < nk; ++k) {
            const int id = idx(s, k, d);
            {
              Epi e; e.mask_slope = slope; e.flags = EPI_MASKBITS; e.XB = hb[id];
              RUN(conv_bwd_1d_desc(c2[id], gcs[k], ghk[k], B, To, e, da[k]));
            }
            Epi e; e.flags = EPI_RESID | EPI_MASKBITS; e.mask_slope = slope; e.R = gcs[k]; e.XB = xb[id];
            if (d == 0) { dsts[k] = gxs; if (k > 0) e.flags |= EPI_ACCUM; }
            else dsts[k] = (gcs[k] == gAB[k][0]) ? gAB[k][1] : gAB[k][0];
            RUN(conv_bwd_1d_desc(c1[id], ghk[k], dsts[k], B, To, e, db[k]));
            pa[k] = &da[k]; pb[k] = &db[k];
          }
          if (!dry) {
            if (d > 0) RUN(dmx_conv_pair_group_launch(nk, pa, pb, st));
            else for (int k = 0; k < nk; ++k) RUN(conv_pair_run(da[k], db[k], st));
          }
          for (int k = 0; k < nk; ++k) gcs[k] = dsts[k];
        }
      } else {
      if (mt) {
        hipEvent_t e0 = next_event();
        (void)hipEventRecord(e0, st);
        for (int k = 1; k < nk; ++k) (void)hipStreamWaitEvent(bstream[k], e0, 0);
      }
      for (int k = 0; k < nk; ++k) {
        hipStream_t sk = (mt && k > 0) ? bstream[k] : st;
        const act_t* gc = g;
        for (int d = nd - 1; d >= 0; --d) {
          const int id = idx(s, k, d);
          GemmDesc da, db;
          {
            Epi e; e.mask_slope = slope;
            if (fused[id]) { e.flags = EPI_MASKBITS; e.XB = hb[id]; } else { e.flags = EPI_MASK; e.X = ha[id]; }
            RUN(conv_bwd_1d_desc(c2[id], gc, ghk[k], B, To, e, da));
          }
          Epi e; e.flags = EPI_RESID; e.mask_slope = slope; e.R = gc;
          if (fused[id]) { e.flags |= EPI_MASKBITS; e.XB = xb[id]; } else { e.flags |= EPI_MASK; e.X = xa[id]; }
          act_t* dst;
          if (d == 0) {
            dst = gxs;
            if (k > 0) e.flags |= EPI_ACCUM;
            if (mt && fin_prev) (void)hipStreamWaitEvent(sk, fin_prev, 0);
          } else {
            dst = (gc == gAB[k][0]) ? gAB[k][1] : gAB[k][0];
          }
          RUN(conv_bwd_1d_desc(c1[id], ghk[k], dst, B, To, e, db));
          RUN(conv_pair_run(da, db, sk));
          if (d == 0 && mt) { fin_prev = next_event(); (void)hipEventRecord(fin_prev, sk); }
          gc = dst;
        }
      }
      }
      if (mt && fin_prev) (void)hipStreamWaitEvent(st, fin_prev, 0);
      {
        Epi e; e.flags = EPI_MASK; e.mask_slope = slope;
        if (s > 0) { e.X = act_out[s - 1]; e.alpha = 1.f / nk; } else { e.X = act_pre; }
        RUN(conv_bwd_1d(ups[s], gxs, gprev, B, Tin, e, st));
      }
      g = gprev;
    }
    {
      Epi e;
      RUN(conv_bwd_1d(conv_pre, g, dmel, B, T, e, st));
    }
    arena.release(mk0);
    return DMX_OK;
  }
};

Model* dmx_make_hifigan(const dmx_hifigan_config* c) { return new HifiGan(*c); }
int dmx_hifigan_out_len_impl(Model* m, int T) { return static_cast<HifiGan*>(m)->out_len(T); }
int dmx_hifigan_fwd_impl(Model* m, const act_t* mel, float* wav, int B, int T, void* ws, size_t wsb, hipStream_t st) {
  return static_cast<HifiGan*>(m)->forward(mel, wav, B, T, ws, wsb, st);
}
int dmx_hifigan_bwd_impl(Model* m, const float* dwav, act_t* dmel, hipStream_t st) {
  return static_cast<HifiGan*>(m)->backward(dwav, dmel, st);
}
size_t dmx_hifigan_ws_impl(Model* m, int B, int T) {
  HifiGan* h = static_cast<HifiGan*>(m);
  h->arena.peak = 0;
  h->forward(nullptr, nullptr, B, T, nullptr, 0, nullptr);
  h->backward(nullptr, nullptr, nullptr);
  h->have_tape = false;
  h->dry = false;
  return h->arena.peak + 256;
}
```

### diffmusic_amd/csrc/kernels.h

```cpp
#pragma once
#include "dmx_common.h"

#define DMX_GN_MAX_CHUNKS 512

size_t dmx_gn_scratch_floats(int B, int C, int G);
struct GnRegion {
  float* part = nullptr;
  int tm = 0, P = 0, nq = 0;
  int qoff = 0, cq = 0;
};
struct GnParts { int n = 0; GnRegion r[8]; };
size_t dmx_gn_part_floats(int B, int P, int N);
int dmx_groupnorm_fwd(const act_t* x, act_t* y, const float* gamma, const float* beta, float* stats, float* scale,
                      float* shift, float* partial, int B, int P, int C, int G, float eps, int silu, hipStream_t st,
                      const GnParts* parts = nullptr);
int dmx_groupnorm_bwd(const act_t* x, const act_t* dy, const act_t* add, act_t* dx, const float* stats,
                      const float* scale, const float* shift, float* k0, float* k1, float* partial, int B, int P, int C,
                      int G, int silu, hipStream_t st, const GnParts* parts = nullptr);
int dmx_layernorm_fwd(const act_t* x, act_t* y, const float* gamma, const float* beta, int rows, int C, float eps,
                      hipStream_t st);
int dmx_softmax_fwd(const float* S, act_t* P, const float* colbias, long long rows, int N, long long lds, long long ldp,
                    int rows_per_bias, hipStream_t st);
int dmx_softmax_act(const act_t* S, act_t* P, const float* colbias, long long rows, int N, long long ldp, int rows_per_bias,
                    hipStream_t st);
int dmx_rowdot(const act_t* a, const act_t* b, float* out, long long rows, int C, long long lda, long long ldb, hipStream_t st);
int dmx_geglu(const act_t* x, act_t* y, long long rows, int I, hipStream_t st);
int dmx_silu(const act_t* x, act_t* y, long long n, hipStream_t st);
int dmx_upsample_nearest(const act_t* x, act_t* y, int B, int Hi, int Wi, int Ho, int Wo, int C, hipStream_t st);
int dmx_upsample2x_bwd(const act_t* dy, act_t* dx, int B, int Hi, int Wi, int C, hipStream_t st);
int dmx_transpose(const act_t* in, act_t* out, int R, int C, long long ldi, long long ldo, int Z, int Zi, long long sIo,
                  long long sIi, long long sOo, long long sOi, hipStream_t st);
int dmx_concat2(const act_t* a, const act_t* b, act_t* dst, long long rows, int Ca, int Cb, hipStream_t st);
int dmx_copy_channels(const act_t* src, act_t* dst, long long rows, int C, int lds, int ldd, int soff, int doff,
                      hipStream_t st);
int dmx_axpby(const act_t* x, const act_t* y0, act_t* y, float a, float b, long long n, hipStream_t st);
int dmx_nchw_f32_to_nhwc_bf16(const float* x, act_t* y, int B, int C, int HW, int Cp, float scale, hipStream_t st);
int dmx_nhwc_bf16_to_nchw_f32(const act_t* x, float* y, int B, int C, int HW, int Cp, float scale, hipStream_t st);
int dmx_f32_to_bf16(const float* x, act_t* y, long long n, float scale, hipStream_t st);
int dmx_bf16_to_f32(const act_t* x, float* y, long long n, float scale, hipStream_t st);
int dmx_extract_col(const act_t* x, float* y, long long rows, int ld, int col, hipStream_t st);
int dmx_gather_col_f32(const float* x, float* y, long long rows, int ld, int col, hipStream_t st);
int dmx_tanh_bwd_pad8(const float* dwav, const float* wav8, act_t* gz, long long rows, hipStream_t st);
int dmx_scatter_col_pad8(const float* v, act_t* y, long long rows, float scale, hipStream_t st);
int dmx_gather_col_f32_to_act(const float* x, act_t* y, long long rows, int ld, int col, hipStream_t st);
int dmx_pad_col8_act(const act_t* v, act_t* y, long long rows, hipStream_t st);
int dmx_timestep_embed(const float* t, act_t* y, int B, int dim, hipStream_t st);

bool dmx_flash_attn_ok(int dh, int C);
int dmx_flash_attn_fwd(const act_t* q, const act_t* k, const act_t* v, act_t* o, const float* colbias, int B, int Nq, int Nk,
                       int C, int heads, float scale, hipStream_t st, int ldq = 0, int ldk = 0, int ldv = 0);

int dmx_stft_tables(float* table, float* tableT, int n_fft, int bins, int Npad, int Kpad, int hann, hipStream_t st);
int dmx_stft_fwd(const float* wav, long long wav_stride, const float* table, float* X, int B, int L, int T, int n_fft, int hop, int Npad,
                 hipStream_t st);
int dmx_stft_bwd_frames(const float* Y, const float* tableT, float* dframe, int M, int n_fft, int Kpad, hipStream_t st);
int dmx_mel_fwd(const float* X, const float* fb, float* mel_lin, float* mel_out, int rows, int ldx, int bins, int n_mels, int power2,
                int to_db, float lo, float hi, hipStream_t st);
int dmx_mel_bwd(const float* X, const float* fb, const float* mel_lin, const float* dmel, float* Y, int rows, int ldx, int ldy, int bins,
                int n_mels, int power2, int to_db, float lo, float hi, hipStream_t st);
int dmx_stft_mag(const float* X, float* mag, int B, int T, int bins, int ldx, hipStream_t st);
int dmx_stft_mag_bwd(const float* X, const float* dmag, float* Y, int B, int T, int bins, int ldx, int ldy, hipStream_t st);
int dmx_overlap_add(const float* dframe, float* dwav, long long out_stride, int B, int T, int L, int n_fft, int hop, int accumulate,
                    hipStream_t st);
int dmx_l2_loss_grad(const float* ref, const float* pred, float* loss, float* dpred, int B, long long n, long long ref_stride, float gscale,
                     hipStream_t st);
int dmx_mask_mul(const float* x, long long xs, const float* mask, float* y, long long ys, int B, int L, int Ly, hipStream_t st);
int dmx_melscale(const float* mag, const float* fb, float* mel, int B, int T, int bins, int n_mels, float lo, float hi, hipStream_t st);
int dmx_absmax_normalize(float* x, float* inv_scale, int B, long long n, float target, hipStream_t st);

struct DmxStftMelTables {
  const float2* tw;
  const float* win;
  const int *klo, *klen; const float* fbc; int kmax;
  const int *mlo, *mlen; const float* fbr; int mmax;
};
int dmx_stft_mel_parts(int L, int hop);
int dmx_stft_mel_fwd(const DmxStftMelTables& t, const float* wav, long long wav_stride, const float* mask, const float* ref, long long ref_stride,
                     float* mel_out, float* partial, int B, int L, int hop, int power2, int to_db, float lo, float hi, hipStream_t st,
                     const float* add = nullptr, long long add_stride = 0, const float* addmag = nullptr, float nscale = 0.f,
                     const float* thr = nullptr);
int dmx_stft_mel_bwd(const DmxStftMelTables& t, const float* wav, long long wav_stride, const float* mask, const float* ref, long long ref_stride,
                     const float* dmel, const float* partial, float gscale, float* loss, float* dwav, long long dwav_stride, int Lfull,
                     int accumulate, int B, int L, int hop, int power2, int to_db, float lo, float hi, hipStream_t st,
                     const float* add = nullptr, long long add_stride = 0, const float* addmag = nullptr, float nscale = 0.f,
                     const float* thr = nullptr);


int dmx_pred_x0(const float* x, const float* eps, float* x0, long long n, float sqrt_a, float sqrt_1ma, hipStream_t st);
int dmx_pred_x0_ex(const float* x, const float* m, float* x0, long long n, float sqrt_a, float sqrt_1ma, int ptype, float clip_r, hipStream_t st);
int dmx_cfg_combine(const float* eps2, float* out, long long n, float scale, hipStream_t st);
int dmx_sched_update(int mode, const float* x, const float* eps, const float* x0, const float* g0, const float* inv_scale,
                     const float* noise, float* prev, float* x0_out, float* grad_out, int B, int n, float alpha_t, float alpha_prev,
                     float sigma, float rate, float eps_small, int global_norm, hipStream_t st, int ptype = 0, float clip_r = 0.f);
```

### diffmusic_amd/csrc/layers.h

```cpp
#pragma once
#include <string>
#include <vector>
#include <map>
#include <cstdio>
#include <cstring>
#include "dmx_common.h"
#include "kernels.h"

void dmx_set_error(const char* fmt, ...);

inline int pad8(int c) { return (c + 7) & ~7; }

struct Arena {
  char* base = nullptr;
  size_t cap = 0, off = 0, peak = 0;
  bool overflow = false;
  void reset(void* b, size_t c) { base = (char*)b; cap = c; off = 0; overflow = false; }
  void* raw(size_t bytes) {
    bytes = align_up(bytes, 256);
    if (off + bytes > cap) { overflow = true; off += bytes; if (off > peak) peak = off; return base; }
    void* p = base + off;
    off += bytes;
    if (off > peak) peak = off;
    return p;
// ... 28 lines not shown
  int Ci = 0, Co = 0, Cip = 0, Cop = 0;
  int kh = 1, kw = 1, stride = 1, dil = 1, pad_h = 0, pad_w = 0;
  int pad_h_hi = 0, pad_w_hi = 0;
  bool transposed = false;
  bool has_bias = true, need_bwd = false;
  bool geglu = false;
  int w_id = -1, b_id = -1;
  int ln_g_id = -1, ln_b_id = -1;
  float ln_eps = 1e-5f;
  float* colsum = nullptr;
  std::vector<act_t*> wf;
  std::vector<std::vector<int>> wf_taps;
  act_t* wb = nullptr;
  float* bias = nullptr;
  std::vector<act_t*> wup;
  act_t* wup_b = nullptr;
  int ntaps() const { return kh * kw; }
};

struct Epi {
  int flags = 0;
  float alpha = 1.f, act_slope = 0.f, mask_slope = 0.f, resid_inv_slope = 1.f;
  const act_t* R = nullptr;
  const act_t* X = nullptr;
  act_t* C2 = nullptr;
  const float* rowbias = nullptr;
  int ldrb = 0;
  const unsigned char* XB = nullptr;
  unsigned char* B2 = nullptr;
  float* rowstats_out = nullptr;
  const float* rowstats_in = nullptr;
  int nslots = 0;
  float* gn_part = nullptr;
  const act_t* gnb_x = nullptr;
  const float* gnb_scale = nullptr;
  const float* gnb_shift = nullptr;
  int gnb_silu = 0, gnb_cpg = 0;
  const float* gnb_stats = nullptr;
};

ConvLayer make_conv1d(ParamStore& ps, const std::string& prefix, int Ci, int Co, int k, int dil, int pad, bool need_bwd);
ConvLayer make_convT1d(ParamStore& ps, const std::string& prefix, int Ci, int Co, int k, int stride, int pad, bool need_bwd);
ConvLayer make_conv2d(ParamStore& ps, const std::string& prefix, int Ci, int Co, int k, int stride, int pad, bool need_bwd);
ConvLayer make_conv2d_asym(ParamStore& ps, const std::string& prefix, int Ci, int Co, int k, int stride, int pad_lo, int pad_hi);
ConvLayer make_linear(ParamStore& ps, const std::string& prefix, int Ci, int Co, bool bias, bool need_bwd);
int pack_layer(ParamStore& ps, ConvLayer& L, hipStream_t st);
int pack_linear_stack(ParamStore& ps, ConvLayer& dst, const ConvLayer* const* src, int n, hipStream_t st);

int conv_out_len(const ConvLayer& L, int Ti);
int conv_fwd_1d(const ConvLayer& L, const act_t* in, void* out, int B, int Ti, const Epi& e, hipStream_t st);
int conv_bwd_1d(const ConvLayer& L, const act_t* dout, void* din, int B, int Ti, const Epi& e, hipStream_t st);
int conv_fwd_1d_desc(const ConvLayer& L, const act_t* in, void* out, int B, int Ti, const Epi& e, GemmDesc& d);
int conv_bwd_1d_desc(const ConvLayer& L, const act_t* dout, void* din, int B, int Ti, const Epi& e, GemmDesc& d);
int conv_pair_run(const GemmDesc& a, const GemmDesc& b, hipStream_t st);
int conv_fwd_2d(const ConvLayer& L, const act_t* in, void* out, int B, int Hi, int Wi, const Epi& e, hipStream_t st, int* gn_rows = nullptr);
int pack_layer_up2x(ParamStore& ps, ConvLayer& L, hipStream_t st);
int conv_up2x_fwd(const ConvLayer& L, const act_t* in, void* out, int B, int Hi, int Wi, const Epi& e, hipStream_t st,
                  float* const* gn_buf = nullptr, int* gn_rows = nullptr);
int conv_up2x_bwd(const ConvLayer& L, const act_t* dout, void* din, int B, int Hi, int Wi, const Epi& e, hipStream_t st);
int conv_bwd_2d(const ConvLayer& L, const act_t* dout, void* din, int B, int Hi, int Wi, const Epi& e, hipStream_t st, int* gn_rows = nullptr);
struct GemmBatch { int Z = 1, Zi = 1; long long sAo = 0, sAi = 0, sBo = 0, sBi = 0, sCo = 0, sCi = 0; };
int gemm_nt(const act_t* A, int lda, const act_t* Bm, int ldb, void* C, int ldc, int M, int N, int K, const Epi& e,
            const GemmBatch& gb, hipStream_t st);
int linear_fwd(const ConvLayer& L, const act_t* in, int lda, void* out, int ldc, long long rows, const Epi& e, hipStream_t st);
int linear_bwd(const ConvLayer& L, const act_t* dout, int lda, void* din, int ldc, long long rows, const Epi& e, hipStream_t st);

struct GroupNormLayer {
  int C = 0, G = 32, g_id = -1, b_id = -1;
  float eps = 1e-5f;
};
GroupNormLayer make_gn(ParamStore& ps, const std::string& prefix, int C, int G, float eps);
struct GnSave { float* stats = nullptr; float* scale = nullptr; float* shift = nullptr; };
```

### diffmusic_amd/csrc/layers.hip

```cpp
#include "layers.h"
#include "conv_pair.h"
#include <cstdarg>

static thread_local char g_err[512] = "";
void dmx_set_error(const char* fmt, ...) {
  va_list ap;
  va_start(ap, fmt);
  vsnprintf(g_err, sizeof(g_err), fmt, ap);
  va_end(ap);
}
extern "C" const char* dmx_last_error() { return g_err; }

int ParamStore::add(const std::string& name, std::vector<int> shape) {
  Param p;
  p.name = name;
  p.shape = shape;
  p.numel = 1;
  for (int s : shape) p.numel *= (size_t)s;
  p.dev = (float*)dalloc(p.numel * sizeof(float));
  index[name] = (int)params.size();
  params.push_back(p);
  return (int)params.size() - 1;
}
void* ParamStore::dalloc(size_t bytes) {
// ... 315 lines not shown
  d.Hq = 1; d.Wq = To; d.sx = L.stride; d.M = B * To;
  for (int t = 0; t < L.kw; ++t) { d.tdy[t] = 0; d.tdx[t] = (signed char)(t * L.dil - L.pad_w); }
  return DMX_OK;
}

int conv_fwd_1d(const ConvLayer& L, const act_t* in, void* out, int B, int Ti, const Epi& e, hipStream_t st) {
  const int To = conv_out_len(L, Ti);
  GemmDesc d;
  if (!L.transposed) {
    const int rc = conv_fwd_1d_desc(L, in, out, B, Ti, e, d);
    return rc != DMX_OK ? rc : dmx_gemm_launch(d, st);
  }
  fwd_1d_common(d, L, in, out, Ti, To, e);
  const int s = L.stride, p = L.pad_w;
  for (int r = 0; r < s; ++r) {
    GemmDesc q = d;
    const int nt = (int)L.wf_taps[r].size();
    const int base = (r + p) / s;
    q.W = L.wf[r]; q.ntaps = nt; q.K = nt * L.Cip; q.ldw = q.K;
    q.Hq = 1; q.Wq = cdiv(To - r, s); q.M = B * q.Wq;
    q.osx = s; q.oox = r;
    for (int i = 0; i < nt; ++i) { q.tdy[i] = 0; q.tdx[i] = (signed char)(base - i); }
    if (q.Wq <= 0) continue;
    const int rc = dmx_gemm_launch(q, st);
    if (rc != DMX_OK) return rc;
  }
  return DMX_OK;
}

int conv_bwd_1d_desc(const ConvLayer& L, const act_t* dout, void* din, int B, int Ti, const Epi& e, GemmDesc& d) {
  if (!L.wb) { dmx_set_error("layer has no dgrad weights"); return DMX_ERR_STATE; }
  const int To = conv_out_len(L, Ti);
  init_desc(d, e);
  d.A = dout; d.Hi = 1; d.Wi = To; d.Ci = L.Cop; d.lda = L.Cop;
  d.W = L.wb; d.ntaps = L.kw; d.K = L.kw * L.Cop; d.ldw = d.K;
  d.N = L.Cip;
  d.Hq = 1; d.Wq = Ti; d.M = B * Ti;
  set_out(d, din, 1, Ti, L.Cip);
  if (!L.transposed) {
    if (L.stride != 1) return DMX_ERR_SHAPE;
    for (int t = 0; t < L.kw; ++t) { d.tdy[t] = 0; d.tdx[t] = (signed char)(L.pad_w - t * L.dil); }
  } else {
    d.sx = L.stride;
    for (int t = 0; t < L.kw; ++t) { d.tdy[t] = 0; d.tdx[t] = (signed char)(t - L.pad_w); }
  }
  return DMX_OK;
}
int conv_bwd_1d(const ConvLayer& L, const act_t* dout, void* din, int B, int Ti, const Epi& e, hipStream_t st) {
  GemmDesc d;
  const int rc = conv_bwd_1d_desc(L, dout, din, B, Ti, e, d);
  return rc != DMX_OK ? rc : dmx_gemm_launch(d, st);
}

int conv_pair_run(const GemmDesc& a, const GemmDesc& b, hipStream_t st) {
  if (dmx_conv_pair_eligible(&a, b)) return dmx_conv_pair_launch(&a, b, st);
  const int rc = dmx_gemm_launch(a, st);
  return rc != DMX_OK ? rc : dmx_gemm_launch(b, st);
}

int conv_fwd_2d(const ConvLayer& L, const act_t* in, void* out, int B, int Hi, int Wi, const Epi& e, hipStream_t st, int* gn_rows) {
  const int Ho = (Hi + L.pad_h + L.pad_h_hi - L.kh) / L.stride + 1, Wo = (Wi + L.pad_w + L.pad_w_hi - L.kw) / L.stride + 1;
  GemmDesc d;
  init_desc(d, e);
  if (L.has_bias) { d.bias = L.bias; d.flags |= EPI_BIAS; }
  d.A = in; d.Hi = Hi; d.Wi = Wi; d.Ci = L.Cip; d.lda = L.Cip;
  d.W = L.wf[0]; d.ntaps = L.kh * L.kw; d.K = d.ntaps * L.Cip; d.ldw = d.K;
  d.N = L.Cop; d.Hq = Ho; d.Wq = Wo; d.sy = d.sx = L.stride; d.M = B * Ho * Wo;
  set_out(d, out, Ho, Wo, L.Cop);
  for (int ky = 0; ky < L.kh; ++ky)
    for (int kx = 0; kx < L.kw; ++kx) {
      d.tdy[ky * L.kw + kx] = (signed char)(ky - L.pad_h);
      d.tdx[ky * L.kw + kx] = (signed char)(kx - L.pad_w);
    }
  return dmx_gemm_launch(d, st, gn_rows);
}

int conv_up2x_fwd(const ConvLayer& L, const act_t* in, void* out, int B, int Hi, int Wi, const Epi& e, hipStream_t st,
                  float* const* gn_buf, int* gn_rows) {
  if (L.wup.size() != 4) { dmx_set_error("layer has no upsample-folded weights"); return DMX_ERR_STATE; }
  for (int py = 0; py < 2; ++py)
    for (int px = 0; px < 2; ++px) {
      GemmDesc d;
      Epi ep = e;
      if (gn_buf) ep.gn_part = gn_buf[py * 2 + px];
      init_desc(d, ep);
      if (L.has_bias) { d.bias = L.bias; d.flags |= EPI_BIAS; }
      d.A = in; d.Hi = Hi; d.Wi = Wi; d.Ci = L.Cip; d.lda = L.Cip;
      d.W = L.wup[py * 2 + px]; d.ntaps = 4; d.K = 4 * L.Cip; d.ldw = d.K;
      d.N = L.Cop; d.Hq = Hi; d.Wq = Wi; d.M = B * Hi * Wi;
      set_out(d, out, 2 * Hi, 2 * Wi, L.Cop);
      d.osy = d.osx = 2; d.ooy = py; d.oox = px;
      for (int ty = 0; ty < 2; ++ty)
        for (int tx = 0; tx < 2; ++tx) {
          d.tdy[ty * 2 + tx] = (signed char)up2x_delta(py, ty);
          d.tdx[ty * 2 + tx] = (signed char)up2x_delta(px, tx);
        }
      const int rc = dmx_gemm_launch(d, st, gn_rows ? gn_rows + py * 2 + px : nullptr);
      if (rc != DMX_OK) return rc;
    }
  return DMX_OK;
}

int conv_up2x_bwd(const ConvLayer& L, const act_t* dout, void* din, int B, int Hi, int Wi, const Epi& e, hipStream_t st) {
  if (!L.wup_b) { dmx_set_error("layer has no upsample-folded dgrad weights"); return DMX_ERR_STATE; }
  GemmDesc d;
  init_desc(d, e);
  d.A = dout; d.Hi = 2 * Hi; d.Wi = 2 * Wi; d.Ci = L.Cop; d.lda = L.Cop;
  d.W = L.wup_b; d.ntaps = 16; d.K = 16 * L.Cop; d.ldw = d.K;
// ... 71 lines not shown
```

### diffmusic_amd/csrc/models.h

```cpp
#pragma once
#include "layers.h"
#include "../../include/diffmusic_hip.h"

enum { DMX_MODEL_HIFIGAN = 1, DMX_MODEL_VAE = 2, DMX_MODEL_UNET = 3, DMX_MODEL_HTSAT = 4, DMX_MODEL_VAE_ENC = 5 };

struct Model {
  int kind = 0;
  ParamStore ps;
  Arena arena;
  bool finalized = false;
  bool dry = false;
  virtual ~Model() { ps.free_all(); }
  virtual int finalize(hipStream_t st) = 0;
};
struct dmx_model { Model* impl; };

#define RUN(expr) do { if (!dry) { int rc_ = (expr); if (rc_ != DMX_OK) return rc_; } } while (0)
#define CHECK_WS(name) do { if (arena.overflow) { dmx_set_error(name " workspace too small: need %zu bytes", arena.peak); return DMX_ERR_WORKSPACE; } } while (0)

Model* dmx_make_hifigan(const dmx_hifigan_config* c);
int dmx_hifigan_out_len_impl(Model* m, int T);
int dmx_hifigan_fwd_impl(Model* m, const act_t* mel, float* wav, int B, int T, void* ws, size_t wsb, hipStream_t st);
int dmx_hifigan_bwd_impl(Model* m, const float* dwav, act_t* dmel, hipStream_t st);
size_t dmx_hifigan_ws_impl(Model* m, int B, int T);

Model* dmx_make_vae(const dmx_vae_config* c);
size_t dmx_vae_ws_impl(Model* m, int B, int h, int w);
int dmx_vae_fwd_impl(Model* m, const float* z, float zs, act_t* mel, float* mel32, int B, int h, int w, int keep, void* ws, size_t wsb,
                     hipStream_t st);
int dmx_vae_bwd_impl(Model* m, const act_t* dmel, float zs, float* dz, hipStream_t st);
Model* dmx_make_vae_encoder(const dmx_vae_config* c);
size_t dmx_vae_enc_ws_impl(Model* m, int B, int T, int F);
int dmx_vae_enc_fwd_impl(Model* m, const float* mel, float log_floor, float* moments, int B, int T, int F, void* ws, size_t wsb, hipStream_t st);
int dmx_latent_init_impl(const float* moments, float* mean, float* logvar, float* x, const float* eps, const float* noise, int B, int L, int P,
                         float sqrt_abar, float scaling_factor, float sqrt_1m_abar, hipStream_t st);
int dmx_conv2d_raw_impl(const float* w_host, const float* b_host, const act_t* x, act_t* y, int B, int Hi, int Wi, int Ci, int Co, int k,
                        int stride, int pad_lo, int pad_hi, hipStream_t st);
Model* dmx_make_unet(const dmx_unet_config* c);
size_t dmx_unet_ws_impl(Model* m, int B, int h, int w, int n0, int n1);
int dmx_unet_fwd_impl(Model* m, const float* x, const float* t, const float* cls, float* eps, int B, int h, int w, void* ws, size_t wsb,
                      hipStream_t st, const float* c0, int n0, const float* c1, int n1, const float* bias1);

Model* dmx_make_htsat(const dmx_htsat_config* c);
size_t dmx_htsat_ws_impl(Model* m, int B, int frames);
int dmx_htsat_fwd_impl(Model* m, const float* mel, int B, int frames, float* feat, int keep, void* ws, size_t wsb, hipStream_t st);
int dmx_htsat_bwd_impl(Model* m, const float* dfeat, const float* scale, float* dmel, hipStream_t st);
void dmx_htsat_dims_impl(Model* m, int* tokens, int* channels);
size_t dmx_htsat_tape_impl(Model* m, int stage, int block, int which, const act_t** p);
int dmx_gram_fwd_impl(const float* F, float* G, int B, int T, int C, hipStream_t st);
int dmx_gram_bwd_impl(const float* F, const float* dG, float* dF, int B, int T, int C, hipStream_t st);
```

### diffmusic_amd/csrc_torch/torch_ops.cpp

```cpp
#include <ATen/ATen.h>
#include <ATen/hip/impl/HIPGuardImplMasqueradingAsCUDA.h>
#include <ATen/hip/impl/HIPStreamMasqueradingAsCUDA.h>
#include <c10/hip/HIPStream.h>
#include <torch/library.h>

#include "../../include/diffmusic_hip.h"

#pragma weak dmx_vae_encoder_create
#pragma weak dmx_vae_encoder_workspace_bytes
#pragma weak dmx_vae_encode_fwd
#pragma weak dmx_latent_init
#pragma weak dmx_track_stitch_fwd
#pragma weak dmx_track_stitch_bwd
#pragma weak dmx_audio_guidance_fwd_shaped
#pragma weak dmx_audio_guidance_bwd_shaped
#pragma weak dmx_clip_fwd
#pragma weak dmx_clip_bwd
#pragma weak dmx_declip_project

namespace {

#define DMX_DEVICE_OF(t) const c10::hip::HIPGuardMasqueradingAsCUDA dmx_guard_((t).device())
inline void* cur_stream() { return (void*)c10::hip::getCurrentHIPStreamMasqueradingAsCUDA().stream(); }
inline void same_numel(const at::Tensor& a, const at::Tensor& b, const char* what) {
  TORCH_CHECK(a.numel() == b.numel() && a.device() == b.device(), what, ": size / device mismatch");
}

inline void ok(int rc, const char* what) {
  TORCH_CHECK(rc == 0, "diffmusic_hip::", what, " failed with code ", rc, ": ", dmx_last_error());
}
inline void f32_cuda(const at::Tensor& t, const char* name) {
  TORCH_CHECK(t.is_cuda(), name, " must be a GPU tensor (the diffmusic_hip ops have no CPU fallback)");
  TORCH_CHECK(t.scalar_type() == at::kFloat && t.is_contiguous(), name, " must be contiguous fp32");
}
inline void act_cuda(const at::Tensor& t, const char* name) {
  TORCH_CHECK(t.is_cuda() && t.is_contiguous(), name, " must be a contiguous GPU tensor");
  TORCH_CHECK(t.scalar_type() == (dmx_act_dtype() == 1 ? at::kHalf : at::kBFloat16), name, " must have the library's 16-bit activation dtype");
}
inline const float* fp(const std::optional<at::Tensor>& t) { return t.has_value() ? t->data_ptr<float>() : nullptr; }

at::Tensor sched_pred_x0(const at::Tensor& x, const at::Tensor& eps, double alpha_t) {
  f32_cuda(x, "x"); f32_cuda(eps, "eps");
  same_numel(x, eps, "sched_pred_x0(x, eps)");
  DMX_DEVICE_OF(x);
  at::Tensor x0 = at::empty_like(x);
  ok(dmx_sched_pred_x0(x.data_ptr<float>(), eps.data_ptr<float>(), x0.data_ptr<float>(), x.numel(), (float)alpha_t, cur_stream()), "sched_pred_x0");
  return x0;
}
at::Tensor cfg_combine(const at::Tensor& eps2, double scale) {
  f32_cuda(eps2, "eps2");
  TORCH_CHECK(eps2.dim() >= 1 && eps2.size(0) % 2 == 0, "eps2 must hold the [uncond | text] halves of the CFG batch");
  DMX_DEVICE_OF(eps2);
  auto sizes = eps2.sizes().vec();
  sizes[0] /= 2;
  at::Tensor out = at::empty(sizes, eps2.options());
  ok(dmx_sched_cfg_combine(eps2.data_ptr<float>(), out.data_ptr<float>(), out.numel(), (float)scale, cur_stream()), "cfg_combine");
  return out;
}
std::tuple<at::Tensor, std::optional<at::Tensor>> sched_update(int64_t mode, const at::Tensor& x, const at::Tensor& eps, const at::Tensor& x0,
                                                const std::optional<at::Tensor>& g0, const std::optional<at::Tensor>& inv_scale,
                                                const std::optional<at::Tensor>& noise, double alpha_t, double alpha_prev, double sigma,
                                                double rate, double eps_small, bool global_norm) {
  f32_cuda(x, "x"); f32_cuda(eps, "eps"); f32_cuda(x0, "x0");
  TORCH_CHECK(x.dim() >= 1 && x.size(0) >= 1, "x must have a batch dimension");
  same_numel(x, eps, "sched_update(x, eps)"); same_numel(x, x0, "sched_update(x, x0)");
  const int B = (int)x.size(0);
  const int n = (int)(x.numel() / B);
  if (g0) { f32_cuda(*g0, "g0"); same_numel(x, *g0, "sched_update(x, g0)"); }
  if (inv_scale) { f32_cuda(*inv_scale, "inv_scale"); TORCH_CHECK(inv_scale->numel() == B && inv_scale->device() == x.device(), "inv_scale must hold one value per clip"); }
  if (noise) { f32_cuda(*noise, "noise"); same_numel(x, *noise, "sched_update(x, noise)"); }
  TORCH_CHECK(mode == DMX_SCHED_DDIM || (g0 && inv_scale), "guided modes need g0 and inv_scale");
// ... 282 lines not shown
                        mel32 ? mel32->data_ptr<float>() : nullptr, B, h, w, keep_state, ws.data_ptr(), ws.nbytes(), cur_stream()), "vae_dec_fwd");
  return {mel, mel32};
}
at::Tensor vae_enc_fwd(int64_t model, const at::Tensor& mel, double log_floor, int64_t latent_channels, int64_t scale_factor, at::Tensor ws) {
  f32_cuda(mel, "mel");
  TORCH_CHECK(mel.dim() == 3 && scale_factor >= 1, "mel must be (B, frames, bins)");
  DMX_DEVICE_OF(mel);
  const int B = (int)mel.size(0), T = (int)mel.size(1), F = (int)mel.size(2);
  at::Tensor mom = at::empty({B, (T / scale_factor) * (F / scale_factor), 2 * latent_channels}, mel.options());
  ok(dmx_vae_encode_fwd(reinterpret_cast<dmx_model*>(model), mel.data_ptr<float>(), (float)log_floor, mom.data_ptr<float>(), B, T, F,
                        ws.data_ptr(), ws.nbytes(), cur_stream()), "vae_enc_fwd");
  return mom;
}
std::tuple<at::Tensor, at::Tensor, std::optional<at::Tensor>> latent_init(const at::Tensor& moments, int64_t h, int64_t w, const std::optional<at::Tensor>& eps,
                                                                          const std::optional<at::Tensor>& noise, double sqrt_abar, double scaling_factor,
                                                                          double sqrt_1m_abar, bool want_x) {
  f32_cuda(moments, "moments");
  TORCH_CHECK(moments.dim() == 3 && moments.size(1) == h * w && moments.size(2) % 2 == 0, "moments must be (B, h * w, 2 * latent_channels)");
  DMX_DEVICE_OF(moments);
  const int64_t B = moments.size(0), L = moments.size(2) / 2;
  at::Tensor mean = at::empty({B, L, h, w}, moments.options()), logvar = at::empty({B, L, h, w}, moments.options());
  if (eps) { f32_cuda(*eps, "eps"); same_numel(mean, *eps, "latent_init(eps)"); }
  if (noise) { f32_cuda(*noise, "noise"); same_numel(mean, *noise, "latent_init(noise)"); }
  std::optional<at::Tensor> x;
  if (want_x) x = at::empty({B, L, h, w}, moments.options());
  ok(dmx_latent_init(moments.data_ptr<float>(), mean.data_ptr<float>(), logvar.data_ptr<float>(), x ? x->data_ptr<float>() : nullptr, fp(eps), fp(noise),
                     (int)B, (int)L, (int)(h * w), (float)sqrt_abar, (float)scaling_factor, (float)sqrt_1m_abar, cur_stream()), "latent_init");
  return {mean, logvar, x};
}
at::Tensor grad_normalize_(at::Tensor dwav, double target) {
  f32_cuda(dwav, "dwav");
  TORCH_CHECK(dwav.dim() == 2, "dwav must be (B, samples)");
  DMX_DEVICE_OF(dwav);
  at::Tensor inv = at::empty({dwav.size(0)}, dwav.options());
  ok(dmx_grad_normalize(dwav.data_ptr<float>(), inv.data_ptr<float>(), (int)dwav.size(0), dwav.size(1), (float)target, cur_stream()), "grad_normalize");
  return inv;
}
at::Tensor vae_dec_bwd(int64_t model, const at::Tensor& dmel, double z_scale, int64_t latent_channels, int64_t scale_factor) {
  act_cuda(dmel, "dmel");
  DMX_DEVICE_OF(dmel);
  at::Tensor dz = at::empty({dmel.size(0), latent_channels, dmel.size(1) / scale_factor, dmel.size(2) / scale_factor}, dmel.options().dtype(at::kFloat));
  ok(dmx_vae_decode_bwd(reinterpret_cast<dmx_model*>(model), (const uint16_t*)dmel.data_ptr(), (float)z_scale, dz.data_ptr<float>(), cur_stream()), "vae_dec_bwd");
  return dz;
}
at::Tensor hifigan_fwd(int64_t model, const at::Tensor& mel, at::Tensor ws) {
  act_cuda(mel, "mel");
  DMX_DEVICE_OF(mel);
  dmx_model* m = reinterpret_cast<dmx_model*>(model);
  const int B = (int)mel.size(0), T = (int)mel.size(1);
  at::Tensor wav = at::empty({B, dmx_hifigan_out_len(m, T)}, mel.options().dtype(at::kFloat));
  ok(dmx_hifigan_fwd(m, (const uint16_t*)mel.data_ptr(), wav.data_ptr<float>(), B, T, ws.data_ptr(), ws.nbytes(), cur_stream()), "hifigan_fwd");
  return wav;
}
at::Tensor hifigan_bwd(int64_t model, const at::Tensor& dwav, int64_t frames, int64_t model_in_dim) {
  f32_cuda(dwav, "dwav");
  DMX_DEVICE_OF(dwav);
  at::Tensor dmel = at::empty({dwav.size(0), frames, model_in_dim}, dwav.options().dtype(dmx_act_dtype() == 1 ? at::kHalf : at::kBFloat16));
  ok(dmx_hifigan_bwd(reinterpret_cast<dmx_model*>(model), dwav.data_ptr<float>(), (uint16_t*)dmel.data_ptr(), cur_stream()), "hifigan_bwd");
  return dmel;
}

at::Tensor htsat_fwd(int64_t model, const at::Tensor& mel, bool keep_state, at::Tensor ws) {
  f32_cuda(mel, "mel");
  TORCH_CHECK(mel.dim() == 3, "mel must be (B, frames, mel bins)");
  DMX_DEVICE_OF(mel);
  dmx_model* m = reinterpret_cast<dmx_model*>(model);
  int tokens = 0, channels = 0;
  ok(dmx_htsat_feature_dims(m, &tokens, &channels), "htsat_feature_dims");
  at::Tensor feat = at::empty({mel.size(0), tokens, channels}, mel.options());
  ok(dmx_htsat_fwd(m, mel.data_ptr<float>(), (int)mel.size(0), (int)mel.size(1), feat.data_ptr<float>(), keep_state, ws.data_ptr(), ws.nbytes(),
                   cur_stream()), "htsat_fwd");
  return feat;
}
at::Tensor htsat_bwd(int64_t model, const at::Tensor& dfeat, const std::optional<at::Tensor>& scale, int64_t frames, int64_t bins) {
  f32_cuda(dfeat, "dfeat");
  DMX_DEVICE_OF(dfeat);
  if (scale) { f32_cuda(*scale, "scale"); TORCH_CHECK(scale->numel() == dfeat.size(0) && scale->device() == dfeat.device(), "scale must hold one value per clip"); }
  at::Tensor dmel = at::empty({dfeat.size(0), frames, bins}, dfeat.options());
  ok(dmx_htsat_bwd(reinterpret_cast<dmx_model*>(model), dfeat.data_ptr<float>(), fp(scale), dmel.data_ptr<float>(), cur_stream()), "htsat_bwd");
  return dmel;
}
at::Tensor gram_fwd(const at::Tensor& feat) {
  f32_cuda(feat, "feat");
  TORCH_CHECK(feat.dim() == 3, "feat must be (B, tokens, channels)");
  DMX_DEVICE_OF(feat);
  at::Tensor g = at::empty({feat.size(0), feat.size(2), feat.size(2)}, feat.options());
  ok(dmx_gram_fwd(feat.data_ptr<float>(), g.data_ptr<float>(), (int)feat.size(0), (int)feat.size(1), (int)feat.size(2), cur_stream()), "gram_fwd");
  return g;
}
at::Tensor gram_bwd(const at::Tensor& feat, const at::Tensor& dgram) {
  f32_cuda(feat, "feat"); f32_cuda(dgram, "dgram");
  TORCH_CHECK(feat.dim() == 3 && dgram.numel() == feat.size(0) * feat.size(2) * feat.size(2) && dgram.device() == feat.device(), "dgram must be (B, C, C)");
  DMX_DEVICE_OF(feat);
  at::Tensor d = at::empty_like(feat);
  ok(dmx_gram_bwd(feat.data_ptr<float>(), dgram.data_ptr<float>(), d.data_ptr<float>(), (int)feat.size(0), (int)feat.size(1), (int)feat.size(2), cur_stream()), "gram_bwd");
  return d;
}

}

int64_t abi_version() { return DMX_ABI_VERSION; }

TORCH_LIBRARY(diffmusic_hip, m) {
  TORCH_CHECK(dmx_abi_version() == DMX_ABI_VERSION, "libdiffmusic_torch_ops.so was built against C-ABI version ", DMX_ABI_VERSION,
              " but the loaded libdiffmusic_hip.so reports ", dmx_abi_version(), ": rebuild with `python -m diffmusic_amd.build`");
  {
    const std::pair<const char*, const void*> added[] = {{"dmx_vae_encoder_create", (const void*)&dmx_vae_encoder_create},
                                                         {"dmx_vae_encoder_workspace_bytes", (const void*)&dmx_vae_encoder_workspace_bytes},
                                                         {"dmx_vae_encode_fwd", (const void*)&dmx_vae_encode_fwd},
                                                         {"dmx_latent_init", (const void*)&dmx_latent_init},
                                                         {"dmx_track_stitch_fwd", (const void*)&dmx_track_stitch_fwd},
                                                         {"dmx_track_stitch_bwd", (const void*)&dmx_track_stitch_bwd},
                                                         {"dmx_audio_guidance_fwd_shaped", (const void*)&dmx_audio_guidance_fwd_shaped},
                                                         {"dmx_audio_guidance_bwd_shaped", (const void*)&dmx_audio_guidance_bwd_shaped},
                                                         {"dmx_clip_fwd", (const void*)&dmx_clip_fwd},
                                                         {"dmx_clip_bwd", (const void*)&dmx_clip_bwd},
                                                         {"dmx_declip_project", (const void*)&dmx_declip_project}};
    for (const auto& s : added)
      TORCH_CHECK(s.second != nullptr, "the loaded libdiffmusic_hip.so reports C-ABI version ", DMX_ABI_VERSION, " but does not export `", s.first,
                  "` (a build from before the VAE encoder / track-mode / declipping entry points): rebuild with `python -m diffmusic_amd.build --force`");
  }
  m.def("abi_version() -> int", &abi_version);
  m.def("sched_pred_x0(Tensor x, Tensor eps, float alpha_t) -> Tensor", &sched_pred_x0);
  m.def("cfg_combine(Tensor eps2, float scale) -> Tensor", &cfg_combine);
  m.def("sched_update(int mode, Tensor x, Tensor eps, Tensor x0, Tensor? g0, Tensor? inv_scale, Tensor? noise, float alpha_t, float alpha_prev, "
        "float sigma, float rate, float eps_small, bool global_norm) -> (Tensor, Tensor?)", &sched_update);
  m.def("randn_philox(int[] shape, int[] seeds, int offset, Device device) -> Tensor", &randn_philox);
  m.def("mask_mul(Tensor x, Tensor? mask, int L, int Ly) -> Tensor", &mask_mul);
  m.def("l2norm(Tensor ref, Tensor pred, float gscale) -> (Tensor, Tensor)", &l2norm);
  m.def("resample_fwd(Tensor x, Tensor h, int Lin, int Lout, int orig, int new_, int off) -> Tensor", &resample_fwd);
  m.def("resample_bwd(Tensor dy, Tensor h, Tensor? h_rev, int Lin, int Lfull, int orig, int new_, int off) -> Tensor", &resample_bwd);
  m.def("logmel_fwd(int audio, Tensor wav, Tensor(a!) state, int L, bool power2, bool to_db, float lo, float hi) -> Tensor", &logmel_fwd);
  m.def("logmel_bwd(int audio, Tensor dmel, Tensor state, int L, bool power2, bool to_db, float lo, float hi) -> Tensor", &logmel_bwd);
  m.def("mel_guidance(int audio, Tensor wav, Tensor? mask, Tensor ref, Tensor(a!) state, int L, int Lfull, bool power2, bool to_db, float lo, float hi, "
        "float gscale) -> (Tensor, Tensor)", &mel_guidance);
  m.def("mel_guidance_noisy(int audio, Tensor wav, Tensor? mask, Tensor ref, Tensor(a!) state, int L, int Lfull, bool power2, bool to_db, float lo, "
        "float hi, float gscale, Tensor? noise, Tensor? noise_mag, float sigma) -> (Tensor, Tensor)", &mel_guidance_noisy);
  m.def("mel_guidance_shaped(int audio, Tensor wav, Tensor? mask, Tensor ref, Tensor(a!) state, int L, int Lfull, bool power2, bool to_db, float lo, "
        "float hi, float gscale, Tensor? noise, Tensor? noise_mag, float sigma, Tensor? thr) -> (Tensor, Tensor)", &mel_guidance_shaped);
  m.def("clip_fwd(Tensor x, Tensor thr, int L) -> Tensor", &clip_fwd);
  m.def("clip_bwd(Tensor dy, Tensor wav, Tensor thr, int Lfull) -> Tensor", &clip_bwd);
  m.def("declip_project(Tensor wav, Tensor measurement, Tensor thr, int L) -> Tensor", &declip_project);
  m.def("noise_add(Tensor y, Tensor noise, float sigma) -> Tensor", &noise_add);
  m.def("track_stitch_fwd(Tensor wav, int[] starts, int L, int R, int T) -> Tensor", &track_stitch_fwd);
  m.def("track_stitch_bwd(Tensor dtrack, int[] starts, int L, int R, int Lfull) -> Tensor", &track_stitch_bwd);
  m.def("stft_mag_fwd(int audio, Tensor wav, Tensor(a!) state, int L) -> Tensor", &stft_mag_fwd);
  m.def("stft_mag_bwd(int audio, Tensor dmag, Tensor state, int L, int Lfull) -> Tensor", &stft_mag_bwd);
  m.def("melscale_fwd(int audio, Tensor mag, float lo, float hi) -> Tensor", &melscale_fwd);
  m.def("unet_fwd(int model, Tensor x, Tensor t, Tensor? class_labels, Tensor(a!) ws) -> Tensor", &unet_fwd);
  m.def("unet_fwd_ctx(int model, Tensor x, Tensor t, Tensor? class_labels, Tensor c0, Tensor c1, Tensor bias1, Tensor(a!) ws) -> Tensor", &unet_fwd_ctx);
  m.def("vae_dec_fwd(int model, Tensor z, float z_scale, bool keep_state, bool want_f32, int scale_factor, Tensor(a!) ws) -> (Tensor, Tensor?)", &vae_dec_fwd);
  m.def("vae_dec_bwd(int model, Tensor dmel, float z_scale, int latent_channels, int scale_factor) -> Tensor", &vae_dec_bwd);
  m.def("vae_enc_fwd(int model, Tensor mel, float log_floor, int latent_channels, int scale_factor, Tensor(a!) ws) -> Tensor", &vae_enc_fwd);
  m.def("latent_init(Tensor moments, int h, int w, Tensor? eps, Tensor? noise, float sqrt_abar, float scaling_factor, float sqrt_1m_abar, "
        "bool want_x) -> (Tensor, Tensor, Tensor?)", &latent_init);
  m.def("grad_normalize_(Tensor(a!) dwav, float target) -> Tensor", &grad_normalize_);
  m.def("hifigan_fwd(int model, Tensor mel, Tensor(a!) ws) -> Tensor", &hifigan_fwd);
  m.def("hifigan_bwd(int model, Tensor dwav, int frames, int model_in_dim) -> Tensor", &hifigan_bwd);
  m.def("htsat_fwd(int model, Tensor mel, bool keep_state, Tensor(a!) ws) -> Tensor", &htsat_fwd);
  m.def("htsat_bwd(int model, Tensor dfeat, Tensor? scale, int frames, int bins) -> Tensor", &htsat_bwd);
  m.def("gram_fwd(Tensor feat) -> Tensor", &gram_fwd);
  m.def("gram_bwd(Tensor feat, Tensor dgram) -> Tensor", &gram_bwd);
}
```

### diffmusic_amd/engine.py

```python
import ctypes as C
import torch
from . import _lib as L
from . import ops
from ._ctypes_ops import _stream
from .weights import synth_state_dict

HIFIGAN_DEFAULT = dict(model_in_dim=64, upsample_initial_channel=1024, upsample_rates=[5, 4, 2, 2, 2],
                       upsample_kernel_sizes=[16, 16, 8, 4, 4], resblock_kernel_sizes=[3, 7, 11],
                       resblock_dilation_sizes=[[1, 3, 5]] * 3, leaky_relu_slope=0.1, sampling_rate=16000)
VAE_DEFAULT = dict(latent_channels=8, out_channels=1, block_out_channels=[128, 256, 512], layers_per_block=2,
                   norm_num_groups=32, scaling_factor=0.9227914214134216, eps=1e-6)
UNET_MUSICLDM_DEFAULT = dict(in_channels=8, out_channels=8, block_out_channels=[128, 256, 384, 640],
                             layers_per_block=2, attention_heads=8, norm_num_groups=32,
                             down_attn=[0, 1, 1, 1], up_attn=[1, 1, 1, 0], class_embed_dim=512, attn_cross_dims=[0])
UNET_AUDIOLDM2_DEFAULT = dict(UNET_MUSICLDM_DEFAULT, class_embed_dim=0, attn_cross_dims=[0, 768, 1024])


def _fill(arr, vals):
    for i, v in enumerate(vals):
        arr[i] = int(v)


class _Engine:
    kind = "generic"

    def __init__(self, handle, config, device):
        if not handle:
            L.check(-1, "model create")
        self._h = C.c_void_p(handle)
        self.cfg = dict(config)
        self.device = torch.device(device)
        self._ws = {}
        self._finalized = False

    def __del__(self):
        try:
            if getattr(self, "_h", None):
                L.lib().dmx_model_destroy(self._h)
                self._h = None
        except Exception:
            pass

    def param_specs(self):
        lib = L.lib()
        out = []
        for i in range(lib.dmx_model_num_params(self._h)):
            nd = lib.dmx_model_param_ndim(self._h, i)
            out.append((lib.dmx_model_param_name(self._h, i).decode(),
                        tuple(lib.dmx_model_param_dim(self._h, i, d) for d in range(nd))))
        return out

    def _stride_of(self, name):
        return 1

    def synth_state_dict(self, seed=0):
        return synth_state_dict(self.param_specs(), seed, self.kind, self._stride_of)

    allow_unexpected = ()

    def load_state_dict(self, sd, strict=False):
        lib = L.lib()
        from .weights import check_manifest
        specs = self.param_specs()
        check_manifest(specs, sd if strict else {n: sd[n] for n, _ in specs if n in sd}, f"{self.kind} ({type(self).__name__})",
                       self.allow_unexpected)
        for name, shape in specs:
            t = sd[name].detach().to(torch.float32).contiguous().cpu()
            L.check(lib.dmx_model_load_param(self._h, name.encode(), C.c_void_p(t.data_ptr()), t.numel()), name)
        with torch.cuda.device(self.device):
            L.check(lib.dmx_model_finalize(self._h, _stream()), "finalize")
            torch.cuda.synchronize()
        self._finalized = True
        return self

    def _workspace(self, key, nbytes):
        ws = self._ws.get("buf")
        if ws is None or ws.numel() < nbytes:
            self._ws.clear()
            ws = torch.empty(int(nbytes), dtype=torch.uint8, device=self.device)
            self._ws["buf"] = ws
        return ws


class HifiGanEngine(_Engine):
    kind = "hifigan"
    allow_unexpected = ("mean", "scale")

    def __init__(self, config=None, device="cuda"):
        cfg = dict(HIFIGAN_DEFAULT)
        cfg.update(config or {})
        c = L.HifiGanConfig()
        c.model_in_dim, c.upsample_initial_channel = cfg["model_in_dim"], cfg["upsample_initial_channel"]
        c.num_upsamples = len(cfg["upsample_rates"])
        _fill(c.upsample_rates, cfg["upsample_rates"])
        _fill(c.upsample_kernel_sizes, cfg["upsample_kernel_sizes"])
        c.num_kernels = len(cfg["resblock_kernel_sizes"])
        _fill(c.resblock_kernel_sizes, cfg["resblock_kernel_sizes"])
        c.num_dilations = len(cfg["resblock_dilation_sizes"][0])
        _fill(c.resblock_dilation_sizes, [d for row in cfg["resblock_dilation_sizes"] for d in row])
        c.leaky_relu_slope = cfg["leaky_relu_slope"]
        super().__init__(L.lib().dmx_hifigan_create(C.byref(c)), cfg, device)

    def _stride_of(self, name):
        return self.cfg["upsample_rates"][int(name.split(".")[1])]

    @property
    def config(self):
        from types import SimpleNamespace
        return SimpleNamespace(**self.cfg)

    def out_len(self, frames):
        return L.lib().dmx_hifigan_out_len(self._h, frames)

    def __call__(self, mel):
        return self.forward(mel.to(device=self.device, dtype=L.act_dtype()).contiguous())

    def forward(self, mel):
        assert mel.dtype == L.act_dtype() and mel.is_cuda and mel.is_contiguous()
        B, T, _ = mel.shape
        lib = L.lib()
        ws = self._workspace(("h", B, T), lib.dmx_hifigan_workspace_bytes(self._h, B, T))
        self._shape = (B, T)
        return ops.hip.hifigan_fwd(self._h.value, mel, ws)

    def backward(self, dwav):
        _, T = self._shape
        assert dwav.dtype == torch.float32 and dwav.is_contiguous()
        return ops.hip.hifigan_bwd(self._h.value, dwav, T, self.cfg["model_in_dim"])


class VaeDecoderEngine(_Engine):
    kind = "vae"
    allow_unexpected = ("encoder.", "quant_conv.")

    def __init__(self, config=None, device="cuda"):
        cfg = dict(VAE_DEFAULT)
        cfg.update(config or {})
        c = L.VaeConfig()
        c.latent_channels, c.out_channels = cfg["latent_channels"], cfg["out_channels"]
        c.num_blocks = len(cfg["block_out_channels"])
        _fill(c.block_out_channels, cfg["block_out_channels"])
        c.layers_per_block, c.norm_num_groups, c.eps = cfg["layers_per_block"], cfg["norm_num_groups"], cfg["eps"]
        super().__init__(L.lib().dmx_vae_decoder_create(C.byref(c)), cfg, device)
        self.scale_factor = 2 ** (c.num_blocks - 1)
        self.scaling_factor = cfg["scaling_factor"]

    @property
    def config(self):
        from types import SimpleNamespace
        return SimpleNamespace(**self.cfg)

    def decode(self, z):
        from types import SimpleNamespace
        _, m32 = self.decode_hip(z.to(device=self.device, dtype=torch.float32).contiguous(), 1.0, keep_state=False, want_f32=True)
        return SimpleNamespace(sample=m32.unsqueeze(1))

    def decode_hip(self, z, z_scale=1.0, keep_state=True, want_f32=False):
        assert z.dtype == torch.float32 and z.is_cuda and z.is_contiguous()
        B, _, h, w = z.shape
        lib = L.lib()
        ws = self._workspace(("v", B, h, w), lib.dmx_vae_workspace_bytes(self._h, B, h, w))
        self._shape = (B, h, w)
        mel, mel32 = ops.hip.vae_dec_fwd(self._h.value, z, float(z_scale), bool(keep_state), bool(want_f32), self.scale_factor, ws)
        return (mel, mel32) if want_f32 else mel

    def backward(self, dmel, z_scale=1.0):
        assert dmel.dtype == L.act_dtype() and dmel.is_contiguous()
        return ops.hip.vae_dec_bwd(self._h.value, dmel, float(z_scale), self.cfg["latent_channels"], self.scale_factor)


class LatentDistribution:

    def __init__(self, moments, h, w):
        self.moments, self._hw = moments, (int(h), int(w))
        self.mean, self.logvar, _ = ops.hip.latent_init(moments, h, w, None, None, 1.0, 1.0, 0.0, False)

# ... 166 lines not shown
```

### diffmusic_amd/inverse_problem/operator.py

```python
import ctypes as C
import math
import numpy as np
import torch

from .. import _lib as L
from .. import ops
from . import dsp
from .noise import step_sigma

_NEG, _POS = -3.0e38, 3.0e38


class SpectralFrontend:

    def __init__(self, sample_rate=16000, n_fft=1024, hop_length=160, n_mels=64, window="hann", fb=None):
        self.n_fft, self.hop, self.n_mels, self.bins = n_fft, hop_length, n_mels, n_fft // 2 + 1
        if fb is None:
            fb = dsp.melscale_fbanks(self.bins, 0.0, float(sample_rate // 2), n_mels, sample_rate)
        fb = np.ascontiguousarray(np.asarray(fb, dtype=np.float32))
        assert fb.shape == (self.bins, n_mels), fb.shape
        self._h = C.c_void_p(L.lib().dmx_audio_create(n_fft, hop_length, n_mels, 1 if window == "hann" else 0,
                                                       fb.ctypes.data_as(C.c_void_p)))
        if not self._h:
            L.check(-1, "dmx_audio_create")
# ... 81 lines not shown

def l2_loss(ref, pred, want_grad=True, gscale=1.0):
    ref = ref.contiguous()
    assert ref[0].numel() == pred[0].numel(), (ref.shape, pred.shape)
    if pred.is_contiguous():
        loss, dpred = ops.hip.l2norm(ref, pred, float(gscale))
        return loss, (dpred if want_grad else None)
    return ops.ctypes_hip.l2norm(ref, pred, float(gscale), want_grad=want_grad)


def _as_f32_cuda(x):
    if not x.is_cuda:
        raise RuntimeError("diffmusic_amd operators run on the GPU only (HIP library); move the tensor to cuda")
    return x.to(torch.float32)


class BaseOperator:

    def transform(self, data, *args, **kwargs):
        raise NotImplementedError

    def inverse_transform(self, mel_spectrogram, vocoder):
        if mel_spectrogram.dim() == 4:
            mel_spectrogram = mel_spectrogram.squeeze(1)
        return vocoder(mel_spectrogram)

    def forward(self, data, **kwargs):
        raise NotImplementedError

    _ref_cache = None
    cache_reference = True

    def reset_cache(self):
        self._ref_cache = None
        reset = getattr(getattr(self, "noiser", None), "reset", None)
        if reset is not None:
            reset()

    def _ref(self, measurement, space, fn):
        if not self.cache_reference:
            return fn(_as_f32_cuda(measurement))
        cache = self._ref_cache
        if cache is None:
            cache = self._ref_cache = []
        for c in cache:
            if c[0] is measurement and c[1] == measurement._version and c[2] == space:
                return c[3]
        cache.insert(0, (measurement, measurement._version, space, fn(_as_f32_cuda(measurement))))
        del cache[4:]
        return cache[0][3]

    def guidance(self, wav, length, measurement, supervised_space, noise=None, step=None, generator=None):
        raise NotImplementedError

    def _step_noise(self, shape, device, noise, step, generator):
        noiser = getattr(self, "noiser", None)
        sigma = step_sigma(noiser)
        if sigma <= 0.0:
            return None, 0.0
        if noise is None:
            return noiser.draw(tuple(shape), device, step=step, generator=generator), sigma
        if tuple(noise.shape) != tuple(shape):
            raise ValueError(f"noise must be shaped like A(x) = {tuple(shape)}, got {tuple(noise.shape)}")
        return _as_f32_cuda(noise).contiguous(), sigma


class _MelOperator(BaseOperator):
    clamp = (-80.0, 80.0)

    def _init_mel(self, sample_rate=16000):
        self.frontend = SpectralFrontend(sample_rate, 1024, 160, 64, "hann")

    def _mel(self, audio, length=None):
        lo, hi = self.clamp if self.clamp else (_NEG, _POS)
        audio = _as_f32_cuda(audio)
        return self.frontend.transform_fwd(audio, length or audio.shape[-1], True, True, lo, hi)

    def transform(self, audio):
        return self._mel(audio).transpose(1, 2)

    def _a_fwd(self, wav, length):
        raise NotImplementedError

    def _a_bwd(self, dy, wav_full_len):
        raise NotImplementedError

    def _fused_mask_tensor(self, device, length):
        return None

    fused_mask = False

    def guidance(self, wav, length, measurement, supervised_space, noise=None, step=None, generator=None):
        if supervised_space == "mel_spectrogram" and self.fused_mask and self.frontend.fused(length):
            lo, hi = self.clamp if self.clamp else (_NEG, _POS)
            ref = self._ref(measurement, "mel_spectrogram", lambda m: self._mel(m.reshape(m.shape[0], -1)).clone())
            z, sigma = self._step_noise((wav.shape[0], length), wav.device, noise, step, generator)
            return self.frontend.guidance(wav, length, ref, self._fused_mask_tensor(wav.device, length), True, True, lo, hi, noise=z,
                                          sigma=sigma)
        y = self._a_fwd(wav, length)
        z, sigma = self._step_noise(y.shape, y.device, noise, step, generator)
        if z is not None:
            y = ops.hip.noise_add(y, z, sigma)
        if supervised_space == "mel_spectrogram" and self.frontend.fused(y.shape[1]):
            lo, hi = self.clamp if self.clamp else (_NEG, _POS)
            ref = self._ref(measurement, "mel_spectrogram", lambda m: self._mel(m.reshape(m.shape[0], -1)).clone())
            loss, dy = self.frontend.guidance(y, y.shape[1], ref, None, True, True, lo, hi)
            return loss, self._a_bwd(dy, wav.shape[1])
        if supervised_space == "wav_form":
            m32 = self._ref(measurement, "wav_form", lambda m: m.reshape(m.shape[0], -1).contiguous())
            loss, dy = l2_loss(m32, y)
        elif supervised_space == "mel_spectrogram":
            ref = self._ref(measurement, "mel_spectrogram", lambda m: self._mel(m.reshape(m.shape[0], -1)).clone())
            pred = self._mel(y)
            loss, dmel = l2_loss(ref, pred)
            dy = self.frontend.transform_bwd(dmel)
        else:
            raise ValueError("supervised_space should be either 'wav_form' or 'mel_spectrogram")
        return loss, self._a_bwd(dy, wav.shape[1])


class IdentityOperator(_MelOperator):
    fused_mask = True

    def __init__(self, sample_rate):
        self._init_mel(sample_rate)

    def forward(self, data, **kwargs):
        return data

    def _a_fwd(self, wav, length):
        return ops.ctypes_hip.mask_mul(wav, None, length, length)

    def _a_bwd(self, dy, full):
        return ops.ctypes_hip.mask_mul(dy, None, dy.shape[1], full)


class MusicInpaintingOperator(_MelOperator):
    clamp = None
    fused_mask = True

    def _fused_mask_tensor(self, device, length):
        if length != self.mask.shape[1]:
            raise ValueError(f"mask length {self.mask.shape[1]} != waveform length {length}")
        return self._mask_on(device)

    def __init__(self, audio_length_in_s, sample_rate, mask_type, start_inpainting_s, end_inpainting_s, mask_percentage,
                 mask_duration_s, interval_s, noiser=None):
        self.audio_length_in_s, self.sample_rate, self.mask_type = audio_length_in_s, sample_rate, mask_type
        self.start_inpainting_s, self.end_inpainting_s = start_inpainting_s, end_inpainting_s
        self.mask_percentage, self.interval_s, self.mask_duration_s = mask_percentage, interval_s, mask_duration_s
        self.mask = self.generate_mask()
        self._init_mel(sample_rate)
        self.noiser = noiser
        self._mask_dev = None

    def generate_mask(self):
        n = int(self.audio_length_in_s * self.sample_rate)
        mask = torch.ones([1, n])
        sr = self.sample_rate
        if self.mask_type == "box":
            if self.start_inpainting_s is not None and self.end_inpainting_s is not None:
                mask[:, int(self.start_inpainting_s * sr): int(self.end_inpainting_s * sr)] = 0.
        elif self.mask_type == "random":
            dur = int(self.mask_duration_s * sr)
            count = max(1, int(self.mask_percentage * n) // dur)
            for _ in range(count):
                start = int(torch.randint(0, mask.shape[1] - dur, (1,)))
                mask[:, start:start + dur] = 0.
        elif self.mask_type == "periodic":
            interval, dur = int(self.interval_s * sr), int(self.mask_duration_s * sr)
            for start in range(0, mask.shape[1], interval):
                mask[:, start:min(start + dur, mask.shape[1])] = 0.
        return mask

    def _mask_on(self, device):
        if self._mask_dev is None or self._mask_dev.device != device:
            self._mask_dev = self.mask.to(device=device, dtype=torch.float32).contiguous()
        return self._mask_dev

    def forward(self, data, **kwargs):
        data = _as_f32_cuda(data)
        n = data.shape[1]
        y = ops.ctypes_hip.mask_mul(data, self._mask_on(data.device), n, n)
        return self.noiser(y) if self.noiser is not None else y

    def _a_fwd(self, wav, length):
        if length != self.mask.shape[1]:
            raise ValueError(f"mask length {self.mask.shape[1]} != waveform length {length}")
        return ops.ctypes_hip.mask_mul(wav, self._mask_on(wav.device), length, length)

    def _a_bwd(self, dy, full):
        return ops.ctypes_hip.mask_mul(dy, self._mask_on(dy.device), dy.shape[1], full)


class DeclippingOperator(_MelOperator):

    def __init__(self, sample_rate, threshold, noiser=None):
        thr = torch.as_tensor(threshold, dtype=torch.float32).detach().cpu().reshape(-1)
        if thr.numel() < 1 or not bool(torch.isfinite(thr).all()) or not bool((thr > 0).all()):
            raise ValueError(f"threshold = {threshold!r}: positive finite value(s), one for all clips or one per clip")
        self.sample_rate, self.noiser = sample_rate, noiser
        self.per_clip = torch.as_tensor(threshold).dim() > 0
        self.threshold = thr.clone()
        self._thr_dev = None
        self._frontend = None
        self._wav = None

    @property
    def frontend(self):
        if self._frontend is None:
            self._frontend = SpectralFrontend(self.sample_rate, 1024, 160, 64, "hann")
        return self._frontend

    def _check_batch(self, batch):
        n = self.threshold.numel()
        if self.per_clip and n != batch:
            raise ValueError(f"DeclippingOperator holds {n} per-clip threshold(s), the batch has {batch} clip(s)")

    def thresholds(self, batch, device):
        self._check_batch(batch)
        t = self._thr_dev
        if t is None or t.device != device or t.numel() != batch:
            t = self._thr_dev = self.threshold.to(device).expand(batch).contiguous()
        return t

    def forward(self, data, **kwargs):
# ... 257 lines not shown
```

### diffmusic_amd/inverse_problem/track.py

```python
import torch

from .. import ops
from .noise import step_sigma
from .operator import StyleGuidanceOperator

MAX_WINDOWS = 64


def seconds_for_samples(samples, sample_rate):
    seconds = samples / sample_rate
    if int(seconds * sample_rate) != int(samples):
        seconds = (samples + 0.5) / sample_rate
    assert int(seconds * sample_rate) == int(samples), (samples, sample_rate)
    return seconds


class TrackLayout:

    def __init__(self, track_len, window_len, overlap):
        T, L, R = int(track_len), int(window_len), int(overlap)
        if L < 2:
            raise ValueError(f"window_len = {window_len!r}: at least 2 samples")
        if T < L:
            raise ValueError(f"a track of {T} samples is shorter than one window of {L}: tracks shorter than a window are not supported")
        if R <= 0 or R > L // 2:
            raise ValueError(f"overlap = {overlap!r} samples: need 0 < overlap <= window_len // 2 = {L // 2}")
        self.track_len, self.window_len, self.overlap = T, L, R
        W = 1 if T == L else 1 + -((T - L) // -(L - R))
        self.num_windows = W
        self.starts = [0] if W == 1 else [(w * (T - L)) // (W - 1) for w in range(W)]

    def __repr__(self):
        return f"TrackLayout(track_len={self.track_len}, window_len={self.window_len}, overlap={self.overlap}) [{self.num_windows} windows]"

    def cut(self, track):
        t = track.reshape(-1)
        if t.numel() != self.track_len:
            raise ValueError(f"track of {t.numel()} samples, layout of {self.track_len}")
        return torch.stack([t[s:s + self.window_len] for s in self.starts], dim=0)


class TrackOperator:

    def __init__(self, inner, layout):
        if isinstance(inner, TrackOperator):
            raise ValueError("TrackOperator around a TrackOperator: wrap the measurement operator itself")
        if isinstance(inner, StyleGuidanceOperator):
            raise ValueError("StyleGuidanceOperator cannot be the inner operator of a track: its CLAP tower is a 10-second model")
        if layout.num_windows > MAX_WINDOWS:
            raise ValueError(f"{layout.num_windows} windows: a track holds at most {MAX_WINDOWS}")
        self.inner, self.layout = inner, layout
        self.check_noise_stream()

    def check_noise_stream(self):
        noiser = self.noiser
        if step_sigma(noiser) > 0 and getattr(noiser, "stream", "global") == "clip":
            raise ValueError("track mode with measurement noise (sigma > 0) needs the global noise stream (GaussianNoise(sigma, "
                             "stream='global')): the per-clip stream keys one draw per clip, and a track is one sample made of all "
                             "its windows (teacher-forced `noise=` works too)")

    @property
    def noiser(self):
        return getattr(self.inner, "noiser", None)

    @property
    def cache_reference(self):
        return self.inner.cache_reference

    def forward(self, data, **kwargs):
        return self.inner.forward(data, **kwargs)

    def transform(self, *args, **kwargs):
        return self.inner.transform(*args, **kwargs)

    def inverse_transform(self, mel_spectrogram, vocoder):
        return self.inner.inverse_transform(mel_spectrogram, vocoder)

    def reset_cache(self):
        self.inner.reset_cache()

    def stitch(self, wav):
        lay = self.layout
        if wav.dim() != 2 or wav.shape[0] != lay.num_windows or wav.shape[1] < lay.window_len:
            raise ValueError(f"wav has shape {tuple(wav.shape)}, expected ({lay.num_windows}, >= {lay.window_len}) for {lay!r}")
        return ops.hip.track_stitch_fwd(wav, lay.starts, lay.window_len, lay.overlap, lay.track_len)

    def stitch_transpose(self, dtrack, full):
        lay = self.layout
        return ops.hip.track_stitch_bwd(dtrack.contiguous(), lay.starts, lay.window_len, lay.overlap, int(full))

    def guidance(self, wav, length, measurement, supervised_space, **kwargs):
        lay = self.layout
        if int(length) != lay.window_len:
            raise ValueError(f"original_waveform_length = {length}, but the track's windows hold {lay.window_len} samples")
        self.check_noise_stream()
        track = self.stitch(wav)
        loss, dtrack = self.inner.guidance(track, lay.track_len, measurement, supervised_space, **kwargs)
        return loss, self.stitch_transpose(dtrack, wav.shape[1])
```

### diffmusic_amd/schedulers/scheduling_guided.py

```python
from types import SimpleNamespace
import numpy as np
import torch

from .. import ops
from ..torch_utils import randn_tensor, randn_philox
from ..profiling import stage
from ..inverse_problem.noise import step_sigma
from ..inverse_problem.track import TrackOperator
from .utils import InverseProblemSchedulerOutput

_MODE = dict(ddim=0, dps=1, mpgd=2, dsg=3, diffmusic=4)
_PTYPE = dict(epsilon=0, sample=1, v_prediction=2)


def rescale_zero_terminal_snr(betas):
    alphas_bar_sqrt = torch.cumprod(1.0 - betas, dim=0).sqrt()
    a0, aT = alphas_bar_sqrt[0].clone(), alphas_bar_sqrt[-1].clone()
    alphas_bar_sqrt = (alphas_bar_sqrt - aT) * (a0 / (a0 - aT))
    alphas_bar = alphas_bar_sqrt ** 2
    alphas = torch.cat([alphas_bar[0:1], alphas_bar[1:] / alphas_bar[:-1]])
    return 1.0 - alphas


class GuidedDDIMScheduler:
# ... 69 lines not shown
        self._timesteps_host = [int(t) for t in ts]
        self._noise_offset = 0
        if self.operator is not None and hasattr(self.operator, "reset_cache"):
            self.operator.reset_cache()
        self.timesteps = torch.from_numpy(ts).to(device) if device is not None else torch.from_numpy(ts)

    def timesteps_for_strength(self, strength):
        n = self.num_inference_steps
        if n is None:
            raise ValueError("call set_timesteps(num_inference_steps) before timesteps_for_strength")
        if not 0.0 <= float(strength) <= 1.0:
            raise ValueError(f"strength = {strength!r}: a number in [0, 1]")
        n_run = min(int(n * float(strength)), n)
        if n_run == 0:
            raise ValueError(f"strength = {strength!r} leaves no step of num_inference_steps = {n} to run (int(N * strength) == 0)")
        return list(self._timesteps_host[n - n_run:])

    def add_noise_scalars(self, timestep):
        a = float(self._ac[int(timestep)])
        return a ** 0.5, (1.0 - a) ** 0.5

    def add_noise(self, original_samples, noise, timestep):
        if not original_samples.is_cuda:
            raise RuntimeError("diffmusic_amd schedulers run on the GPU only (no CPU fallback)")
        sa, s1 = self.add_noise_scalars(timestep)
        x0 = (original_samples.detach().to(torch.float32) * sa).contiguous()
        z = noise.detach().to(device=x0.device, dtype=torch.float32).contiguous()
        return ops.hip.noise_add(x0, z, float(s1)).to(original_samples.dtype)

    def _get_variance(self, timestep, prev_timestep):
        a_t = float(self._ac[timestep])
        a_p = float(self._ac[prev_timestep]) if prev_timestep >= 0 else float(self.final_alpha_cumprod)
        return (1 - a_p) / (1 - a_t) * (1 - a_t / a_p)

    def _scalars(self, timestep, eta):
        t = int(timestep)
        prev_t = t - self.config.num_train_timesteps // self.num_inference_steps
        a_t = float(self._ac[t])
        a_p = float(self._ac[prev_t]) if prev_t >= 0 else float(self.final_alpha_cumprod)
        sigma = eta * self._get_variance(t, prev_t) ** 0.5
        return t, a_t, a_p, sigma

    def _op_kwargs(self, op_kwargs, timestep, generator):
        if step_sigma(getattr(self.operator, "noiser", None)) <= 0 or "noise" in (op_kwargs or {}):
            return op_kwargs
        ts = getattr(self, "_timesteps_host", None) or []
        return dict(op_kwargs or {}, step=ts.index(timestep) if timestep in ts else None, generator=generator)

    def _guidance(self, x0, measurement, vae, vocoder, length, supervised_space, op_kwargs=None):
        zs = 1.0 / vae.config.scaling_factor
        with stage("vae_fwd"):
            mel = vae.decode_hip(x0, z_scale=zs, keep_state=True)
        with stage("hifigan_fwd"):
            wav = vocoder.forward(mel)
        with stage("operator_mel_loss_fwd_bwd"):
            loss, dwav = self.operator.guidance(wav, length, measurement, supervised_space, **(op_kwargs or {}))
            if not self.per_clip_norm and loss.numel() > 1:
                total = torch.linalg.vector_norm(loss)
                dwav.mul_((loss / total.clamp_min(1e-30))[:, None])
                loss = total.reshape(1)
            inv_scale = ops.hip.grad_normalize_(dwav, float(self.grad_target))
        with stage("hifigan_bwd"):
            dmel = vocoder.backward(dwav)
        with stage("vae_bwd"):
            g0 = vae.backward(dmel, z_scale=zs)
        return loss, g0, inv_scale

    def step(self, model_output, timestep, sample, eta=None, use_clipped_model_output=False, generator=None,
             variance_noise=None, return_dict=True, measurement=None, ip_guidance_rate=None, vae=None, vocoder=None,
             original_waveform_length=0, supervised_space="mel_spectrogram", eps=1e-8, *args, **kwargs):
        eta = self.default_eta if eta is None else eta
        rate = self.default_rate if ip_guidance_rate is None else ip_guidance_rate
        if supervised_space not in ("wav_form", "mel_spectrogram"):
            raise ValueError("supervised_space should be either 'wav_form' or 'mel_spectrogram")
        if variance_noise is not None and generator is not None and eta > 0:
            raise ValueError("Cannot pass both generator and variance_noise. Please make sure that either `generator` or"
                             " `variance_noise` stays `None`.")
        if self.per_clip_norm and self.mode != "ddim" and isinstance(self.operator, TrackOperator):
            raise ValueError("a TrackOperator makes the batch one sample (the windows of a track under one loss): construct the scheduler "
                             "with per_clip_norm=False")
        if not sample.is_cuda:
            raise RuntimeError("diffmusic_amd schedulers run on the GPU only (no CPU fallback)")
        if self._ptype == 1 and self.mode in ("dps", "dsg", "diffmusic"):
            raise RuntimeError("prediction_type='sample': pred_original_sample = model_output does not depend on the sample, so the gradient of "
                               "the loss w.r.t. the sample these schedulers take does not exist (the reference's torch.autograd.grad(rec_loss, "
                               "sample) raises for it, scheduling_dps.py:212)")
        t, a_t, a_p, sigma = self._scalars(timestep, eta)
        x = sample.detach().to(torch.float32).contiguous()
        e = model_output.detach().to(torch.float32).contiguous()
        plain = self._ptype == 0 and self._clip_r == 0.0
        if plain:
            x0 = ops.hip.sched_pred_x0(x, e, a_t)
        else:
            x0 = ops.ctypes_hip.sched_pred_x0(x, e, a_t, ptype=self._ptype, clip_r=self._clip_r)
        mode = _MODE[self.mode]
        noise = None
        if self.mode in ("dps", "mpgd") and eta > 0:
            if variance_noise is None:
                if self.passes_eta_to_parent:
                    randn_tensor(model_output.shape, generator=generator, device=model_output.device, dtype=model_output.dtype)
                variance_noise = randn_tensor(model_output.shape, generator=generator, device=model_output.device,
                                              dtype=model_output.dtype)
            noise = variance_noise.to(torch.float32).contiguous()
        loss = g0 = inv_scale = None
        if self.mode == "ddim":
            loss = torch.tensor([t])
        else:
# ... 65 lines not shown
```

### include/diffmusic_hip.h

```cpp
#ifndef DIFFMUSIC_HIP_H
#define DIFFMUSIC_HIP_H
#include <stddef.h>
#include <stdint.h>

#ifdef __cplusplus
extern "C" {
#endif

#define DMX_ABI_VERSION 4
#define DMX_MAX_STAGES 8

typedef struct dmx_model dmx_model;

typedef struct dmx_hifigan_config {
  int model_in_dim;
  int upsample_initial_channel;
  int num_upsamples;
  int upsample_rates[DMX_MAX_STAGES];
  int upsample_kernel_sizes[DMX_MAX_STAGES];
  int num_kernels;
  int resblock_kernel_sizes[DMX_MAX_STAGES];
  int num_dilations;
  int resblock_dilation_sizes[DMX_MAX_STAGES * DMX_MAX_STAGES];
  float leaky_relu_slope;
} dmx_hifigan_config;

typedef struct dmx_vae_config {
  int latent_channels;
  int out_channels;
  int num_blocks;
  int block_out_channels[DMX_MAX_STAGES];
  int layers_per_block;
  int norm_num_groups;
  float eps;
} dmx_vae_config;

typedef struct dmx_unet_config {
  int in_channels, out_channels;
  int num_blocks;
  int block_out_channels[DMX_MAX_STAGES];
  int layers_per_block;
  int attention_heads;
  int norm_num_groups;
  int down_attn[DMX_MAX_STAGES];
  int up_attn[DMX_MAX_STAGES];
  int class_embed_dim;
  int num_attn_per_layer;
  int attn_cross_dims[4];
} dmx_unet_config;

int dmx_abi_version(void);
int dmx_act_dtype(void);
const char* dmx_last_error(void);

dmx_model* dmx_hifigan_create(const dmx_hifigan_config* cfg);
dmx_model* dmx_vae_decoder_create(const dmx_vae_config* cfg);
dmx_model* dmx_unet_create(const dmx_unet_config* cfg);
void dmx_model_destroy(dmx_model* m);
int dmx_model_num_params(const dmx_model* m);
const char* dmx_model_param_name(const dmx_model* m, int i);
size_t dmx_model_param_numel(const dmx_model* m, int i);
int dmx_model_param_ndim(const dmx_model* m, int i);
int dmx_model_param_dim(const dmx_model* m, int i, int d);
int dmx_model_load_param(dmx_model* m, const char* name, const float* data_host, size_t numel);
int dmx_model_finalize(dmx_model* m, void* stream);

int dmx_hifigan_out_len(const dmx_model* m, int frames);
size_t dmx_hifigan_workspace_bytes(dmx_model* m, int batch, int frames);
int dmx_hifigan_fwd(dmx_model* m, const uint16_t* mel, float* wav, int batch, int frames, void* ws, size_t ws_bytes,
                    void* stream);
int dmx_hifigan_bwd(dmx_model* m, const float* dwav, uint16_t* dmel, void* stream);

size_t dmx_vae_workspace_bytes(dmx_model* m, int batch, int h, int w);
int dmx_vae_decode_fwd(dmx_model* m, const float* z, float z_scale, uint16_t* mel, float* mel_f32, int batch, int h, int w,
                       int keep_state, void* ws, size_t ws_bytes, void* stream);
int dmx_vae_decode_bwd(dmx_model* m, const uint16_t* dmel, float z_scale, float* dz, void* stream);

dmx_model* dmx_vae_encoder_create(const dmx_vae_config* cfg);
size_t dmx_vae_encoder_workspace_bytes(dmx_model* m, int batch, int frames, int bins);
int dmx_vae_encode_fwd(dmx_model* m, const float* mel, float log_floor, float* moments, int batch, int frames, int bins, void* ws,
                       size_t ws_bytes, void* stream);
int dmx_latent_init(const float* moments, float* mean, float* logvar, float* x, const float* eps, const float* noise, int batch,
                    int latent_channels, int hw, float sqrt_abar, float scaling_factor, float sqrt_1m_abar, void* stream);

size_t dmx_unet_workspace_bytes(dmx_model* m, int batch, int h, int w);
int dmx_unet_fwd(dmx_model* m, const float* x, const float* t, const float* class_labels, float* eps, int batch, int h,
                 int w, void* ws, size_t ws_bytes, void* stream);
int dmx_unet_fwd_ctx(dmx_model* m, const float* x, const float* t, const float* class_labels, const float* ctx0, int n0,
                     const float* ctx1, int n1, const float* bias1, float* eps, int batch, int h, int w, void* ws,
                     size_t ws_bytes, void* stream);
size_t dmx_unet_workspace_bytes_ctx(dmx_model* m, int batch, int h, int w, int n0, int n1);

typedef struct dmx_htsat_config {
  int spec_size;
  int num_mel_bins;
  int patch_size;
  int embed_dim;
  int window_size;
  int num_stages;
  int depths[4];
  int num_heads[4];
  float ln_eps;
  float bn_eps;
} dmx_htsat_config;
dmx_model* dmx_htsat_create(const dmx_htsat_config* cfg);
int dmx_htsat_feature_dims(dmx_model* m, int* tokens, int* channels);
size_t dmx_htsat_workspace_bytes(dmx_model* m, int batch, int frames);
int dmx_htsat_fwd(dmx_model* m, const float* mel, int batch, int frames, float* feat, int keep_state, void* ws, size_t ws_bytes, void* stream);
int dmx_htsat_bwd(dmx_model* m, const float* dfeat, const float* scale, float* dmel, void* stream);
size_t dmx_htsat_tape_raw(dmx_model* m, int stage, int block, int which, void* dst, size_t dst_elems, void* stream);
int dmx_gram_fwd(const float* F, float* G, int batch, int tokens, int channels, void* stream);
int dmx_gram_bwd(const float* F, const float* dG, float* dF, int batch, int tokens, int channels, void* stream);

typedef struct dmx_audio dmx_audio;
dmx_audio* dmx_audio_create(int n_fft, int hop, int n_mels, int window_hann, const float* fb_host);
void dmx_audio_destroy(dmx_audio* a);
int dmx_audio_num_frames(const dmx_audio* a, int L);
int dmx_audio_num_bins(const dmx_audio* a);
size_t dmx_audio_state_bytes(const dmx_audio* a, int batch, int L);
int dmx_audio_transform_fwd(dmx_audio* a, const float* wav, long long wav_stride, float* mel_out, void* state, int batch, int L,
                            int power2, int to_db, float lo, float hi, void* stream);
int dmx_audio_transform_bwd(dmx_audio* a, const float* dmel, float* dwav, long long dwav_stride, void* state, int batch, int L,
                            int power2, int to_db, float lo, float hi, int accumulate, void* stream);
int dmx_audio_is_fused(const dmx_audio* a, int L);
// ... 90 lines not shown
```

Baseline: 26.61 steps/s (weak scaling: one step advances a batch of 8 clips on one GPU; value = K / wall x 1 GPU(s)).

## Skip HiFi-GAN conv slabs whose outputs fall in the masked inpainting gap

For inpainting, the masked span of the waveform gets no gradient. The change maps that span back through every HiFi-GAN conv and transposed-conv layer to find the rows whose results can never reach the loss. The fused conv-pair kernels then skip the tiles covering those rows in both forward and backward, and zero the inputs there. The aim is to cut vocoder work in proportion to the gap length. The cost is extra planning code and boundary arithmetic that must stay exact, or gradients near the gap edges could be corrupted.

```diff
diff --git a/diffmusic_amd/_ctypes_ops.py b/diffmusic_amd/_ctypes_ops.py
--- a/diffmusic_amd/_ctypes_ops.py
+++ b/diffmusic_amd/_ctypes_ops.py
@@ -320,6 +320,22 @@
     return wav
 
 
+def hifigan_fwd_dead(model, mel, s0, s1, ws):
+    B, T, _ = mel.shape
+    lib = _lib.lib()
+    wav = torch.empty(B, lib.dmx_hifigan_out_len(model, T), dtype=torch.float32, device=mel.device)
+    _lib.check(lib.dmx_hifigan_fwd_dead(model, _p(mel), _p(wav), B, T, int(s0), int(s1), _p(ws), ws.numel(), _stream()), "hifigan_fwd_dead")
+    return wav
+
+
+def hifigan_dead_plan(model, stages):
+    n = int(stages)
+    arr = [(C.c_int * n)() for _ in range(4)]
+    if _lib.lib().dmx_hifigan_dead_plan(model, *arr, n) < 0:
+        _lib.check(-1, "hifigan_dead_plan")
+    return [int(a[s]) for s in range(n) for a in arr]
+
+
 def hifigan_bwd(model, dwav, frames, model_in_dim):
     dmel = torch.empty(dwav.shape[0], frames, model_in_dim, dtype=_lib.act_dtype(), device=dwav.device)
     _lib.check(_lib.lib().dmx_hifigan_bwd(model, _p(dwav), _p(dmel), _stream()), "hifigan_bwd")
diff --git a/diffmusic_amd/_lib.py b/diffmusic_amd/_lib.py
--- a/diffmusic_amd/_lib.py
+++ b/diffmusic_amd/_lib.py
@@ -78,6 +78,10 @@
     "dmx_hifigan_workspace_bytes": (C.c_size_t, [C.c_void_p, C.c_int, C.c_int]),
     "dmx_hifigan_fwd": (C.c_int, [C.c_void_p, C.c_void_p, C.c_void_p, C.c_int, C.c_int, C.c_void_p, C.c_size_t, C.c_void_p]),
     "dmx_hifigan_bwd": (C.c_int, [C.c_void_p, C.c_void_p, C.c_void_p, C.c_void_p]),
+    "dmx_hifigan_fwd_dead": (C.c_int, [C.c_void_p, C.c_void_p, C.c_void_p, C.c_int, C.c_int, C.c_int, C.c_int, C.c_void_p, C.c_size_t,
+                                       C.c_void_p]),
+    "dmx_hifigan_dead_plan": (C.c_int, [C.c_void_p, C.POINTER(C.c_int), C.POINTER(C.c_int), C.POINTER(C.c_int), C.POINTER(C.c_int), C.c_int]),
+    "dmx_conv_dead_rows": (C.c_int, [C.c_int] * 9 + [C.POINTER(C.c_int), C.POINTER(C.c_int)]),
     "dmx_vae_workspace_bytes": (C.c_size_t, [C.c_void_p, C.c_int, C.c_int, C.c_int]),
     "dmx_vae_decode_fwd": (C.c_int, [C.c_void_p, C.c_void_p, C.c_float, C.c_void_p, C.c_void_p, C.c_int, C.c_int, C.c_int,
                                      C.c_int, C.c_void_p, C.c_size_t, C.c_void_p]),
@@ -169,7 +173,7 @@
 
 ADDED_IN_V4 = ("dmx_vae_encoder_create", "dmx_vae_encoder_workspace_bytes", "dmx_vae_encode_fwd", "dmx_latent_init",
                "dmx_track_stitch_fwd", "dmx_track_stitch_bwd", "dmx_audio_guidance_fwd_shaped", "dmx_audio_guidance_bwd_shaped",
-               "dmx_clip_fwd", "dmx_clip_bwd", "dmx_declip_project")
+               "dmx_clip_fwd", "dmx_clip_bwd", "dmx_declip_project", "dmx_hifigan_fwd_dead", "dmx_hifigan_dead_plan", "dmx_conv_dead_rows")
 
 _lib = None
 
diff --git a/diffmusic_amd/csrc/capi.hip b/diffmusic_amd/csrc/capi.hip
--- a/diffmusic_amd/csrc/capi.hip
+++ b/diffmusic_amd/csrc/capi.hip
@@ -61,6 +61,21 @@
   if (rc) return rc;
   if (!ws) { dmx_set_error("null workspace"); return DMX_ERR_WORKSPACE; }
   return dmx_hifigan_fwd_impl(m->impl, mel, wav, batch, frames, ws, ws_bytes, ST(stream));
+}
+int dmx_hifigan_fwd_dead(dmx_model* m, const uint16_t* mel, float* wav, int batch, int frames, int s0, int s1, void* ws, size_t ws_bytes,
+                         void* stream) {
+  int rc = check(m, DMX_MODEL_HIFIGAN);
+  if (rc) return rc;
+  if (!ws || !mel || !wav) { dmx_set_error("hifigan_fwd_dead: null buffer"); return DMX_ERR_STATE; }
+  return dmx_hifigan_fwd_dead_impl(m->impl, mel, wav, batch, frames, s0, s1, ws, ws_bytes, ST(stream));
+}
+int dmx_hifigan_dead_plan(dmx_model* m, int* skipped, int* total, int* lo, int* hi, int n) {
+  if (!m || !m->impl || m->impl->kind != DMX_MODEL_HIFIGAN) { dmx_set_error("wrong model handle"); return -1; }
+  return dmx_hifigan_dead_plan_impl(m->impl, skipped, total, lo, hi, n);
+}
+int dmx_conv_dead_rows(int k, int dil, int pad, int stride, int transposed, int t_in, int t_out, int a, int b, int* lo, int* hi) {
+  if (!lo || !hi) return DMX_ERR_STATE;
+  return dmx_conv_dead_rows_impl(k, dil, pad, stride, transposed, t_in, t_out, a, b, lo, hi);
 }
 int dmx_hifigan_bwd(dmx_model* m, const float* dwav, uint16_t* dmel, void* stream) {
   int rc = check(m, DMX_MODEL_HIFIGAN);
diff --git a/diffmusic_amd/csrc/conv_pair.h b/diffmusic_amd/csrc/conv_pair.h
--- a/diffmusic_amd/csrc/conv_pair.h
+++ b/diffmusic_amd/csrc/conv_pair.h
@@ -3,9 +3,12 @@
 #include <cstring>
 #include "dmx_common.h"
 
+struct PairDead { int skip0 = 0, skip1 = 0, zero0 = 0, zero1 = 0; };
+
 bool dmx_conv_pair_eligible(const GemmDesc* a, const GemmDesc& b);
-int dmx_conv_pair_launch(const GemmDesc* a, const GemmDesc& b, hipStream_t st);
-int dmx_conv_pair_group_launch(int n, const GemmDesc* const* a, const GemmDesc* const* b, hipStream_t st);
+int dmx_conv_pair_launch(const GemmDesc* a, const GemmDesc& b, hipStream_t st, const PairDead* dead = nullptr);
+int dmx_conv_pair_group_launch(int n, const GemmDesc* const* a, const GemmDesc* const* b, hipStream_t st, const PairDead* dead = nullptr);
+void dmx_conv_pair_slabs(const GemmDesc* a, const GemmDesc& b, const PairDead* dead, int* skipped, int* total);
 
 int dmx_prof_open(hipStream_t st);
 void dmx_prof_close(int rec, hipStream_t st, double flops, double bytes, int M, int N, int K, int taps, int flags, int cfg);
diff --git a/diffmusic_amd/csrc/conv_pair.hip b/diffmusic_amd/csrc/conv_pair.hip
--- a/diffmusic_amd/csrc/conv_pair.hip
+++ b/diffmusic_amd/csrc/conv_pair.hip
@@ -15,6 +15,8 @@
   int single;
   int r_from_slab;
   int a_tape_bits_only;
+  int skip_q0, skip_n;
+  int z0, z1;
 };
 
 #ifdef DMX_PAIR_STAMPS
@@ -117,7 +119,9 @@
     bid = (xcd < r ? xcd * (q + 1) : r * (q + 1) + (xcd - r) * q) + loc;
   }
   const int T = P.T;
-  const int b = bid / P.nb, tq = bid - b * P.nb;
+  const int b = bid / P.nb;
+  int tq = bid - b * P.nb;
+  if (tq >= P.skip_q0) tq += P.skip_n;
   const int t0 = tq * P.BMo;
   const bool single = P.single != 0;
   const int kA = single ? 0 : P.a.ntaps, kB = P.b.ntaps;
@@ -155,7 +159,7 @@
     for (int it = 0; it < K::SLAB_IT; ++it) {
       const int c = tid + it * NT, row = c / CPR, piece = c % CPR, t = tfirst + row;
       sv[it] = make_uint4(0, 0, 0, 0);
-      if (row < nrows && t >= 0 && t < T) sv[it] = *reinterpret_cast<const uint4*>(src + ((long long)b * T + t) * C + piece * 8);
+      if (row < nrows && t >= 0 && t < T && !(t >= P.z0 && t < P.z1)) sv[it] = *reinterpret_cast<const uint4*>(src + ((long long)b * T + t) * C + piece * 8);
     }
     const bool masked = !single && (P.a.flags & EPI_MASK);
     const bool maskbits = !single && (P.a.flags & EPI_MASKBITS);
@@ -518,7 +522,15 @@
 }
 
 namespace {
-long long pair_params(const GemmDesc* a, const GemmDesc& b, PairParams& P, double& fl, double& by) {
+void pair_skip_slabs(const PairDead* dead, int T, int BMo, int& q0, int& q1) {
+  q0 = q1 = 0;
+  if (!dead || dead->skip1 <= dead->skip0) return;
+  const int nb = cdiv(T, BMo);
+  const int lo = cdiv(dead->skip0 > 0 ? dead->skip0 : 0, BMo), hi = dead->skip1 >= T ? nb : dead->skip1 / BMo;
+  if (hi > lo && hi - lo < nb) { q0 = lo; q1 = hi; }
+}
+
+long long pair_params(const GemmDesc* a, const GemmDesc& b, PairParams& P, double& fl, double& by, const PairDead* dead = nullptr) {
   memset(&P, 0, sizeof(P));
   P.b = b;
   P.single = a ? 0 : 1;
@@ -530,6 +542,14 @@
   P.T = b.Wq;
   P.BMo = a ? PAIR_ROWS - hb.lo - hb.hi : PAIR_ROWS;
   P.nb = cdiv(P.T, P.BMo);
+  const int nb_all = P.nb;
+  {
+    int q0, q1;
+    pair_skip_slabs(dead, P.T, P.BMo, q0, q1);
+    P.skip_q0 = q0; P.skip_n = q1 - q0;
+    P.nb -= P.skip_n;
+    if (dead && dead->zero1 > dead->zero0) { P.z0 = dead->zero0; P.z1 = dead->zero1; }
+  }
   static const bool bias_init = getenv("DMX_NO_BIAS_INIT") == nullptr;
   if (bias_init && b.N < 128) {
     if ((P.b.flags & EPI_BIAS) && P.b.bias && !(P.b.flags & (EPI_MASK | EPI_MASKBITS))) P.b.flags = (P.b.flags & ~EPI_BIAS) | EPI_BIASINIT;
@@ -555,17 +575,29 @@
   if (b.flags & EPI_BITS2) by += bits_by;
   if (b.flags & EPI_ACCUM) by += 2.0 * b.M * (double)C;
   if ((b.flags & EPI_LRELU2) && !(b.flags & EPI_NO_C)) by += 2.0 * b.M * (double)C;
+  fl *= (double)P.nb / nb_all; by *= (double)P.nb / nb_all;
   return (long long)nclips * P.nb;
 }
+bool pair_zero_ok(const PairParams& P) { return P.z1 <= P.z0 || !(P.b.flags & EPI_RESID) || P.r_from_slab; }
+}
+
+void dmx_conv_pair_slabs(const GemmDesc* a, const GemmDesc& b, const PairDead* dead, int* skipped, int* total) {
+  const Halo hb = halo_of(b);
+  const int T = b.Wq, BMo = a ? PAIR_ROWS - hb.lo - hb.hi : PAIR_ROWS;
+  int q0, q1;
+  pair_skip_slabs(dead, T, BMo, q0, q1);
+  *skipped = q1 - q0;
+  *total = cdiv(T, BMo);
 }
 
 static int pair_extra_lds() { static const int v = [] { const char* e = getenv("DMX_PAIR_EXTRA_LDS"); return e ? atoi(e) : 0; }(); return v; }
-int dmx_conv_pair_launch(const GemmDesc* a, const GemmDesc& b, hipStream_t st) {
+int dmx_conv_pair_launch(const GemmDesc* a, const GemmDesc& b, hipStream_t st, const PairDead* dead) {
   if (!dmx_conv_pair_eligible(a, b)) return DMX_ERR_SHAPE;
   PairParams P;
   double fl, by;
-  const long long grid = pair_params(a, b, P, fl, by);
+  const long long grid = pair_params(a, b, P, fl, by, dead);
   if (grid > 0x7fffffffLL) return DMX_ERR_SHAPE;
+  if (!pair_zero_ok(P)) return DMX_ERR_SHAPE;
   const int C = b.N;
   const int rec = dmx_prof_open(st);
   auto launch = [&](auto tag) {
@@ -581,7 +613,7 @@
   return hipGetLastError() == hipSuccess ? DMX_OK : DMX_ERR_LAUNCH;
 }
 
-int dmx_conv_pair_group_launch(int n, const GemmDesc* const* a, const GemmDesc* const* b, hipStream_t st) {
+int dmx_conv_pair_group_launch(int n, const GemmDesc* const* a, const GemmDesc* const* b, hipStream_t st, const PairDead* dead) {
   if (n < 1 || n > DMX_PAIR_GROUP) return DMX_ERR_SHAPE;
   static const bool off = getenv("DMX_NO_PAIR_GROUP") != nullptr;
   bool same = !off && n > 1;
@@ -592,7 +624,7 @@
       if (b[j]->C == b[i]->C || (b[j]->C2 && b[j]->C2 == b[i]->C2)) same = false;
   }
   if (!same) {
-    for (int j = 0; j < n; ++j) { const int rc = dmx_conv_pair_launch(a[j], *b[j], st); if (rc != DMX_OK) return rc; }
+    for (int j = 0; j < n; ++j) { const int rc = dmx_conv_pair_launch(a[j], *b[j], st, dead ? dead + j : nullptr); if (rc != DMX_OK) return rc; }
     return DMX_OK;
   }
   int order[DMX_PAIR_GROUP] = {0, 1, 2};
@@ -608,8 +640,8 @@
   for (int i = 0; i < n; ++i) {
     const int j = order[i];
     double f1, b1;
-    const long long g = pair_params(a[j], *b[j], G.p[i], f1, b1);
-    if (g > 0x7ffffff0LL) return DMX_ERR_SHAPE;
+    const long long g = pair_params(a[j], *b[j], G.p[i], f1, b1, dead ? dead + j : nullptr);
+    if (g > 0x7ffffff0LL || !pair_zero_ok(G.p[i])) return DMX_ERR_SHAPE;
     G.n[i] = (int)g;
     if (g > gmax) gmax = g;
     fl += f1; by += b1; Ksum += a[j]->K + b[j]->K;
diff --git a/diffmusic_amd/csrc/elementwise.hip b/diffmusic_amd/csrc/elementwise.hip
--- a/diffmusic_amd/csrc/elementwise.hip
+++ b/diffmusic_amd/csrc/elementwise.hip
@@ -1004,6 +1004,25 @@
   const float g = dwav[idx] * (1.f - w * w);
   reinterpret_cast<uint4*>(gz)[idx] = make_uint4((uint32_t)f2a(g), 0u, 0u, 0u);
 }
+__global__ void gather_col_f32_dead_kernel(const float* __restrict__ x, float* __restrict__ y, long long rows, int ld, int col, int T, int s0,
+                                           int s1) {
+  const long long idx = (long long)blockIdx.x * blockDim.x + threadIdx.x;
+  if (idx >= rows) return;
+  const int t = (int)(idx % T);
+  y[idx] = (t >= s0 && t < s1) ? 0.f : x[idx * ld + col];
+}
+__global__ void tanh_bwd_pad8_dead_kernel(const float* __restrict__ dwav, const float* __restrict__ wav8, act_t* __restrict__ gz,
+                                          long long rows, int T, int s0, int s1) {
+  const long long idx = (long long)blockIdx.x * blockDim.x + threadIdx.x;
+  if (idx >= rows) return;
+  const int t = (int)(idx % T);
+  float g = 0.f;
+  if (!(t >= s0 && t < s1)) {
+    const float w = wav8[idx * 8];
+    g = dwav[idx] * (1.f - w * w);
+  }
+  reinterpret_cast<uint4*>(gz)[idx] = make_uint4((uint32_t)f2a(g), 0u, 0u, 0u);
+}
 __global__ void scatter_col_pad8_kernel(const float* __restrict__ v, act_t* __restrict__ y, long long rows, float scale) {
   const long long idx = (long long)blockIdx.x * blockDim.x + threadIdx.x;
   if (idx >= rows) return;
@@ -1309,6 +1328,14 @@
   return CHECK_LAUNCH();
 }
 
+int dmx_gather_col_f32_dead(const float* x, float* y, long long rows, int ld, int col, int T, int s0, int s1, hipStream_t st) {
+  hipLaunchKernelGGL(gather_col_f32_dead_kernel, dim3((unsigned)((rows + 255) / 256)), dim3(256), 0, st, x, y, rows, ld, col, T, s0, s1);
+  return CHECK_LAUNCH();
+}
+int dmx_tanh_bwd_pad8_dead(const float* dwav, const float* wav8, act_t* gz, long long rows, int T, int s0, int s1, hipStream_t st) {
+  hipLaunchKernelGGL(tanh_bwd_pad8_dead_kernel, dim3((unsigned)((rows + 255) / 256)), dim3(256), 0, st, dwav, wav8, gz, rows, T, s0, s1);
+  return CHECK_LAUNCH();
+}
 int dmx_gather_col_f32_to_act(const float* x, act_t* y, long long rows, int ld, int col, hipStream_t st) {
   hipLaunchKernelGGL(gather_col_f32_to_act_kernel, dim3((unsigned)((rows + 255) / 256)), dim3(256), 0, st, x, y, rows, ld, col);
   return CHECK_LAUNCH();
diff --git a/diffmusic_amd/csrc/hifigan.hip b/diffmusic_amd/csrc/hifigan.hip
--- a/diffmusic_amd/csrc/hifigan.hip
+++ b/diffmusic_amd/csrc/hifigan.hip
@@ -8,8 +8,52 @@
   bool on_;
 };
 
+struct Span { int a = 0, b = 0; bool empty() const { return b <= a; } };
+static inline Span span_meet(Span x, Span y) { Span r{x.a > y.a ? x.a : y.a, x.b < y.b ? x.b : y.b}; if (r.empty()) r = Span{}; return r; }
+static inline long long floor_div(long long a, long long b) { return a >= 0 ? a / b : -((-a + b - 1) / b); }
+static inline long long ceil_div(long long a, long long b) { return -floor_div(-a, b); }
+
+int dmx_conv_dead_rows_impl(int k, int dil, int pad, int stride, int transposed, int t_in, int t_out, int a, int b, int* lo, int* hi) {
+  *lo = *hi = 0;
+  if (k < 1 || dil < 1 || stride < 1 || pad < 0 || t_in < 1 || t_out < 1) return DMX_ERR_SHAPE;
+  if (!transposed && stride != 1) return DMX_ERR_SHAPE;
+  if (a < 0) a = 0;
+  if (b > t_out) b = t_out;
+  if (b <= a) return DMX_OK;
+  const long long INF = 1ll << 40;
+  const long long ea = a == 0 ? -INF : a, eb = b == t_out ? INF : b;
+  long long l, h;
+  if (!transposed) {
+    l = ea - pad + (long long)(k - 1) * dil;
+    h = eb - pad;
+  } else {
+    l = ceil_div(ea + pad, stride);
+    h = ceil_div(eb - (k - 1) + pad, stride);
+  }
+  if (l < 0) l = 0;
+  if (h > t_in) h = t_in;
+  if (h > l) { *lo = (int)l; *hi = (int)h; }
+  return DMX_OK;
+}
+static Span dead_in(const ConvLayer& L, Span d, int t_in, int t_out) {
+  Span r;
+  (void)dmx_conv_dead_rows_impl(L.kw, L.dil, L.pad_w, L.stride, L.transposed ? 1 : 0, t_in, t_out, d.a, d.b, &r.a, &r.b);
+  return r;
+}
+
+struct DeadPlan {
+  int B = 0, T = 0, s0 = 0, s1 = 0;
+  bool on = false;
+  Span wav;
+  std::vector<Span> out, xs;
+  std::vector<Span> xo, h, x;
+  std::vector<int> skipped, total;
+};
+
 struct HifiGan : Model {
   dmx_hifigan_config cfg;
+  DeadPlan plan;
+  bool use_dead = false;
   static constexpr size_t kSplitKBytes = 32u << 20;
   float* splitk_ws = nullptr;
   ConvLayer conv_pre, conv_post;
@@ -92,18 +136,107 @@
     return dmx_conv_pair_eligible(&da, db);
   }
 
+  void step_slabs(int id, int To, bool bwd, const PairDead& pd, int& skipped, int& total) const {
+    GemmDesc da, db;
+    act_t* dummy = reinterpret_cast<act_t*>(size_t(256));
+    unsigned char* dummyb = reinterpret_cast<unsigned char*>(size_t(256));
+    skipped = total = 0;
+    if (!bwd) {
+      Epi ea; ea.flags = EPI_LRELU2 | EPI_NO_C | EPI_BITS2; ea.act_slope = cfg.leaky_relu_slope; ea.B2 = dummyb;
+      Epi eb; eb.flags = EPI_RESID | EPI_RESID_INV; eb.R = dummy; eb.resid_inv_slope = 1.f / cfg.leaky_relu_slope;
+      if (conv_fwd_1d_desc(c1[id], dummy, nullptr, B, To, ea, da) != DMX_OK || conv_fwd_1d_desc(c2[id], nullptr, dummy, B, To, eb, db) != DMX_OK) return;
+    } else {
+      Epi ea; ea.flags = EPI_MASKBITS; ea.mask_slope = cfg.leaky_relu_slope; ea.XB = dummyb;
+      Epi eb; eb.flags = EPI_RESID | EPI_MASKBITS; eb.mask_slope = cfg.leaky_relu_slope; eb.R = dummy; eb.XB = dummyb;
+      if (conv_bwd_1d_desc(c2[id], dummy, dummy, B, To, ea, da) != DMX_OK || conv_bwd_1d_desc(c1[id], dummy, dummy, B, To, eb, db) != DMX_OK) return;
+    }
+    dmx_conv_pair_slabs(&da, db, &pd, &skipped, &total);
+  }
+  bool stage_all_fused(int s, int To) const {
+    bool all = nk <= 3;
+    for (int k = 0; k < nk; ++k) for (int d = 0; d < nd; ++d) all = all && step_is_fused(idx(s, k, d), To);
+    return all;
+  }
+  PairDead dead_fwd(int id) const {
+    const Span w = span_meet(plan.xo[id], plan.h[id]);
+    PairDead pd; pd.skip0 = w.a; pd.skip1 = w.b;
+    return pd;
+  }
+  PairDead dead_bwd(int s, int id, int d) const {
+    const Span w = d == 0 ? plan.xs[s] : plan.x[id];
+    PairDead pd; pd.skip0 = w.a; pd.skip1 = w.b; pd.zero0 = plan.xo[id].a; pd.zero1 = plan.xo[id].b;
+    return pd;
+  }
+
+  void make_plan(int T_, int s0, int s1) {
+    if (plan.B == B && plan.T == T_ && plan.s0 == s0 && plan.s1 == s1 && (int)plan.out.size() == ns) return;
+    plan = DeadPlan();
+    plan.B = B; plan.T = T_; plan.s0 = s0; plan.s1 = s1;
+    plan.out.assign(ns, Span{}); plan.xs.assign(ns, Span{});
+    plan.xo.assign(ns * nk * nd, Span{}); plan.h.assign(ns * nk * nd, Span{}); plan.x.assign(ns * nk * nd, Span{});
+    plan.skipped.assign(ns, 0); plan.total.assign(ns, 0);
+    std::vector<int> len(ns);
+    int t = T_;
+    for (int i = 0; i < ns; ++i) { t = conv_out_len(ups[i], t); len[i] = t; }
+    const int Tout = ns ? len[ns - 1] : T_;
+    plan.wav = span_meet(Span{s0, s1}, Span{0, Tout});
+    if (plan.wav.empty() || ns == 0) return;
+    Span cur = dead_in(conv_post, plan.wav, Tout, Tout);
+    for (int s = ns - 1; s >= 0; --s) {
+      const int To = len[s], Tin = s ? len[s - 1] : T_;
+      plan.out[s] = cur;
+      Span xs{0, To};
+      for (int k = 0; k < nk; ++k) {
+        Span o = cur;
+        for (int d = nd - 1; d >= 0; --d) {
+          const int id = idx(s, k, d);
+          plan.xo[id] = o;
+          plan.h[id] = dead_in(c2[id], o, To, To);
+          plan.x[id] = span_meet(dead_in(c1[id], plan.h[id], To, To), o);
+          o = plan.x[id];
+        }
+        xs = span_meet(xs, o);
+      }
+      plan.xs[s] = xs;
+      cur = dead_in(ups[s], xs, Tin, To);
+    }
+    if (multi_wanted()) return;
+    int any = 0;
+    for (int s = 0; s < ns; ++s) {
+      if (!stage_all_fused(s, len[s])) continue;
+      for (int k = 0; k < nk; ++k)
+        for (int d = 0; d < nd; ++d) {
+          const int id = idx(s, k, d);
+          int sk, tot;
+          step_slabs(id, len[s], false, dead_fwd(id), sk, tot);
+          plan.skipped[s] += sk; plan.total[s] += tot;
+          step_slabs(id, len[s], true, dead_bwd(s, id, d), sk, tot);
+          plan.skipped[s] += sk; plan.total[s] += tot;
+        }
+      any += plan.skipped[s];
+    }
+    plan.on = any > 0;
+    if (!plan.on) plan.skipped.assign(ns, 0);
+  }
+
   int out_len(int T_) const {
     int t = T_;
     for (int i = 0; i < ns; ++i) t = conv_out_len(ups[i], t);
     return t;
   }
 
-  int forward(const act_t* mel, float* wav, int B_, int T_, void* ws, size_t ws_bytes, hipStream_t st) {
+  int forward(const act_t* mel, float* wav, int B_, int T_, void* ws, size_t ws_bytes, hipStream_t st, int s0 = 0, int s1 = 0) {
     if (cfg.model_in_dim & 7) return DMX_ERR_SHAPE;
     dry = (ws == nullptr);
+    B = B_;
+    if (!dry) {
+      use_dead = false;
+      if (s1 > s0) { make_plan(T_, s0, s1); use_dead = plan.on; }
+    }
+    const bool dead = use_dead && !dry;
     SplitKScope sk_scope(splitk_ws, kSplitKBytes, !dry && !multi_wanted());
     arena.reset(ws, dry ? (size_t)-1 : ws_bytes);
-    B = B_; T = T_;
+    T = T_;
     Ts.assign(ns, 0);
     xs_a.assign(ns, nullptr); act_out.assign(ns, nullptr);
     ha.assign(ns * nk * nd, nullptr); xa.assign(ns * nk * nd, nullptr);
@@ -154,8 +287,10 @@
         for (int d = 0; d < nd; ++d) {
           GemmDesc da[DMX_MAX_STAGES], db[DMX_MAX_STAGES];
           const GemmDesc* pa[DMX_MAX_STAGES]; const GemmDesc* pb[DMX_MAX_STAGES];
+          PairDead pd[DMX_MAX_STAGES];
           for (int k = 0; k < nk; ++k) {
             const int id = idx(s, k, d);
+            if (dead) pd[k] = dead_fwd(id);
             {
               Epi e; e.flags = EPI_LRELU2 | EPI_NO_C | EPI_BITS2; e.act_slope = slope; e.B2 = hb[id];
               RUN(conv_fwd_1d_desc(c1[id], xa[id], ha[id], B, To, e, da[k]));
@@ -180,8 +315,8 @@
               dmx_set_error("hifigan: resblock step %d was planned as fused but the pair kernel refuses it", idx(s, k, d));
               return DMX_ERR_STATE;
             }
-          if (d < nd - 1) RUN(dmx_conv_pair_group_launch(nk, pa, pb, st));
-          else for (int k = 0; k < nk; ++k) RUN(conv_pair_run(da[k], db[k], st));
+          if (d < nd - 1) RUN(dmx_conv_pair_group_launch(nk, pa, pb, st, dead ? pd : nullptr));
+          else for (int k = 0; k < nk; ++k) RUN(conv_pair_run(da[k], db[k], st, dead ? &pd[k] : nullptr));
         }
         arena.release(mk);
         cur_act = act_out[s];
@@ -239,7 +374,8 @@
       Epi e; e.flags = EPI_F32OUT | EPI_TANH;
       RUN(conv_fwd_1d(conv_post, cur_act, wav8, B, Tout, e, st));
     }
-    RUN(dmx_gather_col_f32(wav8, wav, (long long)B * Tout, 8, 0, st));
+    if (dead) RUN(dmx_gather_col_f32_dead(wav8, wav, (long long)B * Tout, 8, 0, Tout, plan.wav.a, plan.wav.b, st));
+    else RUN(dmx_gather_col_f32(wav8, wav, (long long)B * Tout, 8, 0, st));
     have_tape = true;
     return DMX_OK;
   }
@@ -254,7 +390,9 @@
     const int Clast = ups[ns - 1].Cop;
     act_t* g = arena.bf((size_t)B * Tout * Clast);
     CHECK_WS("hifigan");
-    RUN(dmx_tanh_bwd_pad8(dwav, wav8, gz, (long long)B * Tout, st));
+    const bool dead = use_dead && !dry;
+    if (dead) RUN(dmx_tanh_bwd_pad8_dead(dwav, wav8, gz, (long long)B * Tout, Tout, plan.wav.a, plan.wav.b, st));
+    else RUN(dmx_tanh_bwd_pad8(dwav, wav8, gz, (long long)B * Tout, st));
     {
       Epi e; e.flags = EPI_MASK; e.X = act_out[ns - 1]; e.mask_slope = 0.01f; e.alpha = 1.f / nk;
       RUN(conv_bwd_1d(conv_post, gz, g, B, Tout, e, st));
@@ -276,12 +414,20 @@
       if (all_fused && !mt) {
         const act_t* gcs[DMX_MAX_STAGES];
         for (int k = 0; k < nk; ++k) gcs[k] = g;
+        if (dead && !plan.xs[s].empty() &&
+            hipMemset2DAsync(gxs + (size_t)plan.xs[s].a * C, (size_t)To * C * sizeof(act_t), 0, (size_t)(plan.xs[s].b - plan.xs[s].a) * C * sizeof(act_t),
+                             (size_t)B, st) != hipSuccess) {
+          dmx_set_error("hifigan: clearing the dead rows of a stage gradient failed");
+          return DMX_ERR_LAUNCH;
+        }
         for (int d = nd - 1; d >= 0; --d) {
           GemmDesc da[DMX_MAX_STAGES], db[DMX_MAX_STAGES];
           const GemmDesc* pa[DMX_MAX_STAGES]; const GemmDesc* pb[DMX_MAX_STAGES];
           act_t* dsts[DMX_MAX_STAGES];
+          PairDead pd[DMX_MAX_STAGES];
           for (int k = 0; k < nk; ++k) {
             const int id = idx(s, k, d);
+            if (dead) pd[k] = dead_bwd(s, id, d);
             {
               Epi e; e.mask_slope = slope; e.flags = EPI_MASKBITS; e.XB = hb[id];
               RUN(conv_bwd_1d_desc(c2[id], gcs[k], ghk[k], B, To, e, da[k]));
@@ -293,8 +439,8 @@
             pa[k] = &da[k]; pb[k] = &db[k];
           }
           if (!dry) {
-            if (d > 0) RUN(dmx_conv_pair_group_launch(nk, pa, pb, st));
-            else for (int k = 0; k < nk; ++k) RUN(conv_pair_run(da[k], db[k], st));
+            if (d > 0) RUN(dmx_conv_pair_group_launch(nk, pa, pb, st, dead ? pd : nullptr));
+            else for (int k = 0; k < nk; ++k) RUN(conv_pair_run(da[k], db[k], st, dead ? &pd[k] : nullptr));
           }
           for (int k = 0; k < nk; ++k) gcs[k] = dsts[k];
         }
@@ -354,6 +500,20 @@
 int dmx_hifigan_fwd_impl(Model* m, const act_t* mel, float* wav, int B, int T, void* ws, size_t wsb, hipStream_t st) {
   return static_cast<HifiGan*>(m)->forward(mel, wav, B, T, ws, wsb, st);
 }
+int dmx_hifigan_fwd_dead_impl(Model* m, const act_t* mel, float* wav, int B, int T, int s0, int s1, void* ws, size_t wsb, hipStream_t st) {
+  return static_cast<HifiGan*>(m)->forward(mel, wav, B, T, ws, wsb, st, s0, s1);
+}
+int dmx_hifigan_dead_plan_impl(Model* m, int* skipped, int* total, int* lo, int* hi, int n) {
+  HifiGan* h = static_cast<HifiGan*>(m);
+  for (int s = 0; s < n && s < h->ns; ++s) {
+    const bool have = h->use_dead && s < (int)h->plan.out.size();
+    if (skipped) skipped[s] = have ? h->plan.skipped[s] : 0;
+    if (total) total[s] = have ? h->plan.total[s] : 0;
+    if (lo) lo[s] = have ? h->plan.out[s].a : 0;
+    if (hi) hi[s] = have ? h->plan.out[s].b : 0;
+  }
+  return h->ns;
+}
 int dmx_hifigan_bwd_impl(Model* m, const float* dwav, act_t* dmel, hipStream_t st) {
   return static_cast<HifiGan*>(m)->backward(dwav, dmel, st);
 }
diff --git a/diffmusic_amd/csrc/kernels.h b/diffmusic_amd/csrc/kernels.h
--- a/diffmusic_amd/csrc/kernels.h
+++ b/diffmusic_amd/csrc/kernels.h
@@ -41,6 +41,8 @@
 int dmx_extract_col(const act_t* x, float* y, long long rows, int ld, int col, hipStream_t st);
 int dmx_gather_col_f32(const float* x, float* y, long long rows, int ld, int col, hipStream_t st);
 int dmx_tanh_bwd_pad8(const float* dwav, const float* wav8, act_t* gz, long long rows, hipStream_t st);
+int dmx_gather_col_f32_dead(const float* x, float* y, long long rows, int ld, int col, int T, int s0, int s1, hipStream_t st);
+int dmx_tanh_bwd_pad8_dead(const float* dwav, const float* wav8, act_t* gz, long long rows, int T, int s0, int s1, hipStream_t st);
 int dmx_scatter_col_pad8(const float* v, act_t* y, long long rows, float scale, hipStream_t st);
 int dmx_gather_col_f32_to_act(const float* x, act_t* y, long long rows, int ld, int col, hipStream_t st);
 int dmx_pad_col8_act(const act_t* v, act_t* y, long long rows, hipStream_t st);
diff --git a/diffmusic_amd/csrc/layers.h b/diffmusic_amd/csrc/layers.h
--- a/diffmusic_amd/csrc/layers.h
+++ b/diffmusic_amd/csrc/layers.h
@@ -104,7 +104,8 @@
 int conv_bwd_1d(const ConvLayer& L, const act_t* dout, void* din, int B, int Ti, const Epi& e, hipStream_t st);
 int conv_fwd_1d_desc(const ConvLayer& L, const act_t* in, void* out, int B, int Ti, const Epi& e, GemmDesc& d);
 int conv_bwd_1d_desc(const ConvLayer& L, const act_t* dout, void* din, int B, int Ti, const Epi& e, GemmDesc& d);
-int conv_pair_run(const GemmDesc& a, const GemmDesc& b, hipStream_t st);
+struct PairDead;
+int conv_pair_run(const GemmDesc& a, const GemmDesc& b, hipStream_t st, const PairDead* dead = nullptr);
 int conv_fwd_2d(const ConvLayer& L, const act_t* in, void* out, int B, int Hi, int Wi, const Epi& e, hipStream_t st, int* gn_rows = nullptr);
 int pack_layer_up2x(ParamStore& ps, ConvLayer& L, hipStream_t st);
 int conv_up2x_fwd(const ConvLayer& L, const act_t* in, void* out, int B, int Hi, int Wi, const Epi& e, hipStream_t st,
diff --git a/diffmusic_amd/csrc/layers.hip b/diffmusic_amd/csrc/layers.hip
--- a/diffmusic_amd/csrc/layers.hip
+++ b/diffmusic_amd/csrc/layers.hip
@@ -391,8 +391,9 @@
   return rc != DMX_OK ? rc : dmx_gemm_launch(d, st);
 }
 
-int conv_pair_run(const GemmDesc& a, const GemmDesc& b, hipStream_t st) {
-  if (dmx_conv_pair_eligible(&a, b)) return dmx_conv_pair_launch(&a, b, st);
+int conv_pair_run(const GemmDesc& a, const GemmDesc& b, hipStream_t st, const PairDead* dead) {
+  if (dmx_conv_pair_eligible(&a, b)) return dmx_conv_pair_launch(&a, b, st, dead);
+  if (dead) { dmx_set_error("conv_pair_run: dead rows need the fused pair kernel"); return DMX_ERR_SHAPE; }
   const int rc = dmx_gemm_launch(a, st);
   return rc != DMX_OK ? rc : dmx_gemm_launch(b, st);
 }
diff --git a/diffmusic_amd/csrc/models.h b/diffmusic_amd/csrc/models.h
--- a/diffmusic_amd/csrc/models.h
+++ b/diffmusic_amd/csrc/models.h
@@ -22,6 +22,9 @@
 int dmx_hifigan_out_len_impl(Model* m, int T);
 int dmx_hifigan_fwd_impl(Model* m, const act_t* mel, float* wav, int B, int T, void* ws, size_t wsb, hipStream_t st);
 int dmx_hifigan_bwd_impl(Model* m, const float* dwav, act_t* dmel, hipStream_t st);
+int dmx_hifigan_fwd_dead_impl(Model* m, const act_t* mel, float* wav, int B, int T, int s0, int s1, void* ws, size_t wsb, hipStream_t st);
+int dmx_hifigan_dead_plan_impl(Model* m, int* skipped, int* total, int* lo, int* hi, int n);
+int dmx_conv_dead_rows_impl(int k, int dil, int pad, int stride, int transposed, int t_in, int t_out, int a, int b, int* lo, int* hi);
 size_t dmx_hifigan_ws_impl(Model* m, int B, int T);
 
 Model* dmx_make_vae(const dmx_vae_config* c);
diff --git a/diffmusic_amd/csrc_torch/torch_ops.cpp b/diffmusic_amd/csrc_torch/torch_ops.cpp
--- a/diffmusic_amd/csrc_torch/torch_ops.cpp
+++ b/diffmusic_amd/csrc_torch/torch_ops.cpp
@@ -17,6 +17,8 @@
 #pragma weak dmx_clip_fwd
 #pragma weak dmx_clip_bwd
 #pragma weak dmx_declip_project
+#pragma weak dmx_hifigan_fwd_dead
+#pragma weak dmx_hifigan_dead_plan
 
 namespace {
 
@@ -405,6 +407,25 @@
   ok(dmx_hifigan_fwd(m, (const uint16_t*)mel.data_ptr(), wav.data_ptr<float>(), B, T, ws.data_ptr(), ws.nbytes(), cur_stream()), "hifigan_fwd");
   return wav;
 }
+at::Tensor hifigan_fwd_dead(int64_t model, const at::Tensor& mel, int64_t s0, int64_t s1, at::Tensor ws) {
+  act_cuda(mel, "mel");
+  DMX_DEVICE_OF(mel);
+  dmx_model* m = reinterpret_cast<dmx_model*>(model);
+  const int B = (int)mel.size(0), T = (int)mel.size(1);
+  at::Tensor wav = at::empty({B, dmx_hifigan_out_len(m, T)}, mel.options().dtype(at::kFloat));
+  ok(dmx_hifigan_fwd_dead(m, (const uint16_t*)mel.data_ptr(), wav.data_ptr<float>(), B, T, (int)s0, (int)s1, ws.data_ptr(), ws.nbytes(), cur_stream()),
+     "hifigan_fwd_dead");
+  return wav;
+}
+std::vector<int64_t> hifigan_dead_plan(int64_t model, int64_t stages) {
+  const int n = (int)stages;
+  std::vector<int> a[4];
+  for (auto& v : a) v.assign(n > 0 ? n : 1, 0);
+  TORCH_CHECK(dmx_hifigan_dead_plan(reinterpret_cast<dmx_model*>(model), a[0].data(), a[1].data(), a[2].data(), a[3].data(), n) >= 0, "hifigan_dead_plan");
+  std::vector<int64_t> out;
+  for (int s = 0; s < n; ++s) for (auto& v : a) out.push_back(v[s]);
+  return out;
+}
 at::Tensor hifigan_bwd(int64_t model, const at::Tensor& dwav, int64_t frames, int64_t model_in_dim) {
   f32_cuda(dwav, "dwav");
   DMX_DEVICE_OF(dwav);
@@ -468,7 +489,9 @@
                                                          {"dmx_audio_guidance_bwd_shaped", (const void*)&dmx_audio_guidance_bwd_shaped},
                                                          {"dmx_clip_fwd", (const void*)&dmx_clip_fwd},
                                                          {"dmx_clip_bwd", (const void*)&dmx_clip_bwd},
-                                                         {"dmx_declip_project", (const void*)&dmx_declip_project}};
+                                                         {"dmx_declip_project", (const void*)&dmx_declip_project},
+                                                         {"dmx_hifigan_fwd_dead", (const void*)&dmx_hifigan_fwd_dead},
+                                                         {"dmx_hifigan_dead_plan", (const void*)&dmx_hifigan_dead_plan}};
     for (const auto& s : added)
       TORCH_CHECK(s.second != nullptr, "the loaded libdiffmusic_hip.so reports C-ABI version ", DMX_ABI_VERSION, " but does not export `", s.first,
                   "` (a build from before the VAE encoder / track-mode / declipping entry points): rebuild with `python -m diffmusic_amd.build --force`");
@@ -510,6 +533,8 @@
   m.def("grad_normalize_(Tensor(a!) dwav, float target) -> Tensor", &grad_normalize_);
   m.def("hifigan_fwd(int model, Tensor mel, Tensor(a!) ws) -> Tensor", &hifigan_fwd);
   m.def("hifigan_bwd(int model, Tensor dwav, int frames, int model_in_dim) -> Tensor", &hifigan_bwd);
+  m.def("hifigan_fwd_dead(int model, Tensor mel, int s0, int s1, Tensor(a!) ws) -> Tensor", &hifigan_fwd_dead);
+  m.def("hifigan_dead_plan(int model, int stages) -> int[]", &hifigan_dead_plan);
   m.def("htsat_fwd(int model, Tensor mel, bool keep_state, Tensor(a!) ws) -> Tensor", &htsat_fwd);
   m.def("htsat_bwd(int model, Tensor dfeat, Tensor? scale, int frames, int bins) -> Tensor", &htsat_bwd);
   m.def("gram_fwd(Tensor feat) -> Tensor", &gram_fwd);
diff --git a/diffmusic_amd/engine.py b/diffmusic_amd/engine.py
--- a/diffmusic_amd/engine.py
+++ b/diffmusic_amd/engine.py
@@ -1,4 +1,5 @@
 import ctypes as C
+import os
 import torch
 from . import _lib as L
 from . import ops
@@ -100,6 +101,7 @@
         _fill(c.resblock_dilation_sizes, [d for row in cfg["resblock_dilation_sizes"] for d in row])
         c.leaky_relu_slope = cfg["leaky_relu_slope"]
         super().__init__(L.lib().dmx_hifigan_create(C.byref(c)), cfg, device)
+        self.dead_span_enabled = os.environ.get("DMX_NO_DEAD_SPAN", "0") in ("", "0")
 
     def _stride_of(self, name):
         return self.cfg["upsample_rates"][int(name.split(".")[1])]
@@ -115,13 +117,20 @@
     def __call__(self, mel):
         return self.forward(mel.to(device=self.device, dtype=L.act_dtype()).contiguous())
 
-    def forward(self, mel):
+    def forward(self, mel, dead=None):
         assert mel.dtype == L.act_dtype() and mel.is_cuda and mel.is_contiguous()
         B, T, _ = mel.shape
         lib = L.lib()
         ws = self._workspace(("h", B, T), lib.dmx_hifigan_workspace_bytes(self._h, B, T))
         self._shape = (B, T)
+        if dead is not None and self.dead_span_enabled and int(dead[1]) > int(dead[0]):
+            return ops.hip.hifigan_fwd_dead(self._h.value, mel, int(dead[0]), int(dead[1]), ws)
         return ops.hip.hifigan_fwd(self._h.value, mel, ws)
+
+    def dead_plan(self):
+        n = len(self.cfg["upsample_rates"])
+        flat = list(ops.hip.hifigan_dead_plan(self._h.value, n))
+        return [dict(skipped=flat[4 * s], total=flat[4 * s + 1], span=(flat[4 * s + 2], flat[4 * s + 3])) for s in range(n)]
 
     def backward(self, dwav):
         _, T = self._shape
diff --git a/diffmusic_amd/inverse_problem/operator.py b/diffmusic_amd/inverse_problem/operator.py
--- a/diffmusic_amd/inverse_problem/operator.py
+++ b/diffmusic_amd/inverse_problem/operator.py
@@ -157,6 +157,9 @@
 
     def guidance(self, wav, length, measurement, supervised_space, noise=None, step=None, generator=None):
         raise NotImplementedError
+
+    def dead_span(self, length):
+        return None
 
     def _step_noise(self, shape, device, noise, step, generator):
         noiser = getattr(self, "noiser", None)
@@ -224,6 +227,16 @@
         return loss, self._a_bwd(dy, wav.shape[1])
 
 
+def longest_zero_run(mask):
+    z = np.concatenate(([0], (np.asarray(mask, dtype=np.float32).reshape(-1) == 0).astype(np.int8), [0]))
+    edges = np.flatnonzero(np.diff(z))
+    if edges.size == 0:
+        return None
+    starts, ends = edges[0::2], edges[1::2]
+    i = int(np.argmax(ends - starts))
+    return int(starts[i]), int(ends[i])
+
+
 class IdentityOperator(_MelOperator):
     fused_mask = True
 
@@ -277,6 +290,14 @@
             for start in range(0, mask.shape[1], interval):
                 mask[:, start:min(start + dur, mask.shape[1])] = 0.
         return mask
+
+    def dead_span(self, length):
+        if length != self.mask.shape[1]:
+            return None
+        cached = getattr(self, "_dead_span", None)
+        if cached is None or cached[0] is not self.mask or cached[1] != self.mask._version:
+            cached = self._dead_span = (self.mask, self.mask._version, longest_zero_run(self.mask[0]))
+        return cached[2]
 
     def _mask_on(self, device):
         if self._mask_dev is None or self._mask_dev.device != device:
diff --git a/diffmusic_amd/inverse_problem/track.py b/diffmusic_amd/inverse_problem/track.py
--- a/diffmusic_amd/inverse_problem/track.py
+++ b/diffmusic_amd/inverse_problem/track.py
@@ -67,6 +67,9 @@
     def cache_reference(self):
         return self.inner.cache_reference
 
+    def dead_span(self, length):
+        return None
+
     def forward(self, data, **kwargs):
         return self.inner.forward(data, **kwargs)
 
diff --git a/diffmusic_amd/schedulers/scheduling_guided.py b/diffmusic_amd/schedulers/scheduling_guided.py
--- a/diffmusic_amd/schedulers/scheduling_guided.py
+++ b/diffmusic_amd/schedulers/scheduling_guided.py
@@ -145,7 +145,9 @@
         with stage("vae_fwd"):
             mel = vae.decode_hip(x0, z_scale=zs, keep_state=True)
         with stage("hifigan_fwd"):
-            wav = vocoder.forward(mel)
+            span = getattr(self.operator, "dead_span", None)
+            dead = span(length) if span is not None else None
+            wav = vocoder.forward(mel) if dead is None else vocoder.forward(mel, dead=dead)
         with stage("operator_mel_loss_fwd_bwd"):
             loss, dwav = self.operator.guidance(wav, length, measurement, supervised_space, **(op_kwargs or {}))
             if not self.per_clip_norm and loss.numel() > 1:
diff --git a/include/diffmusic_hip.h b/include/diffmusic_hip.h
--- a/include/diffmusic_hip.h
+++ b/include/diffmusic_hip.h
@@ -70,6 +70,10 @@
 int dmx_hifigan_fwd(dmx_model* m, const uint16_t* mel, float* wav, int batch, int frames, void* ws, size_t ws_bytes,
                     void* stream);
 int dmx_hifigan_bwd(dmx_model* m, const float* dwav, uint16_t* dmel, void* stream);
+int dmx_hifigan_fwd_dead(dmx_model* m, const uint16_t* mel, float* wav, int batch, int frames, int s0, int s1, void* ws,
+                         size_t ws_bytes, void* stream);
+int dmx_hifigan_dead_plan(dmx_model* m, int* skipped, int* total, int* lo, int* hi, int n);
+int dmx_conv_dead_rows(int k, int dil, int pad, int stride, int transposed, int t_in, int t_out, int a, int b, int* lo, int* hi);
 
 size_t dmx_vae_workspace_bytes(dmx_model* m, int batch, int h, int w);
 int dmx_vae_decode_fwd(dmx_model* m, const float* z, float z_scale, uint16_t* mel, float* mel_f32, int batch, int h, int w,
```

Measured after the change: 26.96 steps/s (weak scaling: one step advances a batch of 8 clips on one GPU; value = K / wall x 1 GPU(s)), median of 6. 1.01x the previous value.
